# mageky/time-series-spark

Hardware: AMD Instinct MI355X
Metric: series_fitted_per_sec (higher is better)
Workload: dtype f64

## Files before the change

### include/tsf_dev.h

```cpp
#ifndef TSF_DEV_H
#define TSF_DEV_H

#include "tsf.h"

#ifdef __cplusplus
extern "C" {
#endif

enum {
    TSF_OPT_HARM = 0,
    TSF_OPT_LATTICE,
    TSF_OPT_SPARSE_EXTRA,
    TSF_OPT_FIT_GROUPED,
    TSF_OPT_GRAM_SHARE,
    TSF_OPT_GRID_ORDER,
    TSF_OPT_GRID_SHARE,
    TSF_OPT_RAGGED_SPLIT,
    TSF_OPT_QUAD_REG,
    TSF_OPT_QUAD_M2_LDS,
    TSF_OPT_QUAD_W4,
    TSF_OPT_QUAD_RREG,
    TSF_OPT_NEWTON_BATCH,
    TSF_OPT_NEWTON_FLAGS, TSF_OPT_NEWTON_NS, TSF_OPT_NEWTON_LCAP, TSF_OPT_NEWTON_FILL,
    TSF_OPT_QUAD_RAW_Y,
    TSF_OPT_DEBUG_ASYNC_SCRATCH,
    TSF_OPT_COOP_TAIL,
    TSF_OPT_MAP_DIRECT,
    TSF_OPT_COUNT
};
int tsf_set_option(tsf_ctx *ctx, int option, int value);
int tsf_get_option(const tsf_ctx *ctx, int option);

int tsf_eval(tsf_ctx *ctx, const tsf_spec *spec, int64_t N, int32_t T, const int64_t *ds,
             const void *y, int32_t y_dtype, const double *floor, const double *cap,
             const double *extra, const double *theta, double *f_out, double *grad_out);
int tsf_eval_quadratic(tsf_ctx *ctx, const tsf_spec *spec, int64_t N, int32_t T, const int64_t *ds,
                       const void *y, int32_t y_dtype, const double *extra, const double *theta_ref,
                       const double *theta, double *f_out, double *grad_out);
int tsf_design(tsf_ctx *ctx, const tsf_spec *spec, int32_t T, const int64_t *ds,
               const double *extra, double *X_out, double *t_out, tsf_grid_info *grid_out);
int tsf_selftest_math(tsf_ctx *ctx, int32_t op, int64_t n, const double *a, const double *b,
                      double *out);

#define TSF_PROFILE_RING 64
int tsf_set_profiling(tsf_ctx *ctx, int32_t enable);
int tsf_profile_read(tsf_ctx *ctx, float *ms_out, int32_t max_n, int32_t *n_out);
int tsf_last_fit_kernel_ms(tsf_ctx *ctx, float *ms_out);
int tsf_last_fit_route(tsf_ctx *ctx, int32_t *sparse_columns);
int tsf_last_cv_grids(const tsf_ctx *ctx, int64_t *n_grids, int32_t *n_launches);
int tsf_last_tune_counts(const tsf_ctx *ctx, int32_t *expand_launches, int32_t *fit_launches);

#ifdef __cplusplus
}
#endif
#endif
```

### time_series_spark_amd/_lib.py

```python
import contextlib
import ctypes
import os

import numpy as np

_HERE = os.path.dirname(os.path.abspath(__file__))
LIB_PATH = os.environ.get('TSF_LIB_PATH') or os.path.join(_HERE, 'libtsf_amd.so')

MAX_SEAS = 8
MAX_EXTRA = 64
MAX_S = 60
MAX_K = 64
MAX_P = 128
MAX_COMP = 128

GROWTH_LINEAR, GROWTH_LOGISTIC = 0, 1
MODE_ADDITIVE, MODE_MULTIPLICATIVE = 0, 1
Y_F64, Y_F32, Y_I32 = 0, 1, 2
EVAL_AUTO, EVAL_RESIDUAL, EVAL_QUADRATIC = 0, 1, 2
ALGO_LBFGS, ALGO_NEWTON, ALGO_AUTO = 0, 1, 2
RK_AUTO, RK_WAVE, RK_MFMA, RK_COOP = 0, 1, 2, 3
CONVERGE_STAN, CONVERGE_MAP = 0, 1

ST_ABSX, ST_ABSF, ST_RELF, ST_ABSGRAD, ST_RELGRAD, ST_MAXIT = 10, 20, 21, 30, 31, 40
ST_CONSTANT, ST_LSFAIL, ST_INIT_NONFINITE, ST_TOO_FEW, ST_CAP = 50, -1, -2, -10, -11
ST_EVAL_LIMIT = -3
ST_CHANGEPOINT = -12
ST_NEWTON_CONVERGED, ST_NEWTON_FAIL = 60, -4
ST_MAP_KKT, ST_MAP_FTOL, ST_MAP_MAXIT, ST_MAP_LS = 70, 71, 72, 73
STATUS_NAMES = {10: 'ABSX', 20: 'ABSF', 21: 'RELF', 30: 'ABSGRAD', 31: 'RELGRAD', 40: 'MAXIT',
                50: 'CONSTANT', -1: 'LSFAIL', -2: 'INIT_NONFINITE', -3: 'EVAL_LIMIT', -10: 'TOO_FEW',
                -11: 'CAP', -12: 'CHANGEPOINT', 60: 'NEWTON_CONVERGED', -4: 'NEWTON_FAIL', 70: 'MAP_KKT', 71: 'MAP_FTOL', 72: 'MAP_MAXIT',
                73: 'MAP_LS'}


class TsfSpec(ctypes.Structure):
    _fields_ = [('growth', ctypes.c_int32), ('n_changepoints', ctypes.c_int32),
                ('changepoint_range', ctypes.c_double),
                ('changepoint_prior_scale', ctypes.c_double),
                ('n_seas', ctypes.c_int32), ('n_extra', ctypes.c_int32),
                ('seas_period', ctypes.c_double * MAX_SEAS),
                ('seas_prior_scale', ctypes.c_double * MAX_SEAS),
                ('seas_order', ctypes.c_int32 * MAX_SEAS),
                ('seas_mode', ctypes.c_int32 * MAX_SEAS),
                ('extra_prior_scale', ctypes.c_double * MAX_EXTRA),
                ('extra_mode', ctypes.c_int32 * MAX_EXTRA),
                ('max_iter', ctypes.c_int32), ('history', ctypes.c_int32),
                ('init_alpha', ctypes.c_double), ('tol_obj', ctypes.c_double),
                ('tol_rel_obj', ctypes.c_double), ('tol_grad', ctypes.c_double),
                ('tol_rel_grad', ctypes.c_double), ('tol_param', ctypes.c_double),
                ('eval_form', ctypes.c_int32), ('recenter_every', ctypes.c_int32),
                ('recenter_ratio', ctypes.c_double),
                ('algorithm', ctypes.c_int32), ('residual_kernel', ctypes.c_int32),
                ('coop_after', ctypes.c_int32), ('converge', ctypes.c_int32), ('map_max_iter', ctypes.c_int32),
                ('map_tol', ctypes.c_double),
                ('changepoints_specified', ctypes.c_int32), ('changepoint_ns', ctypes.c_int64 * MAX_S)]


class TsfCvArgs(ctypes.Structure):
    _fields_ = [('horizon_ns', ctypes.c_int64), ('period_ns', ctypes.c_int64), ('initial_ns', ctypes.c_int64),
                ('rolling_window', ctypes.c_double)]


class TsfGridInfo(ctypes.Structure):
    _fields_ = [('start_ns', ctypes.c_int64), ('t_scale_ns', ctypes.c_int64),
                ('T', ctypes.c_int32), ('S', ctypes.c_int32), ('i1', ctypes.c_int32),
                ('NT', ctypes.c_int32), ('t_change', ctypes.c_double * (MAX_S + 4))]


GRID_DTYPE = np.dtype([('start_ns', '<i8'), ('t_scale_ns', '<i8'), ('T', '<i4'), ('S', '<i4'),
                       ('i1', '<i4'), ('NT', '<i4'), ('t_change', '<f8', (MAX_S + 4,))])


class TsfFitOut(ctypes.Structure):
    _fields_ = [('theta', ctypes.c_void_p), ('y_scale', ctypes.c_void_p),
                ('fval', ctypes.c_void_p), ('status', ctypes.c_void_p),
                ('n_iter', ctypes.c_void_p), ('n_eval', ctypes.c_void_p),
                ('grid', ctypes.c_void_p)]


class TsfCvOut(ctypes.Structure):
    _fields_ = [('fit', TsfFitOut), ('yhat', ctypes.c_void_p), ('yhat_lower', ctypes.c_void_p),
                ('yhat_upper', ctypes.c_void_p), ('horizon_ns', ctypes.c_void_p), ('mse', ctypes.c_void_p),
                ('rmse', ctypes.c_void_p), ('mae', ctypes.c_void_p), ('mape', ctypes.c_void_p),
                ('coverage', ctypes.c_void_p), ('series_status', ctypes.c_void_p)]


class TsfTuneOut(ctypes.Structure):
    _fields_ = [('score', ctypes.c_void_p), ('cand_status', ctypes.c_void_p), ('best', ctypes.c_void_p),
                ('series_status', ctypes.c_void_p), ('fit', TsfFitOut)]


EXPORTS = ['tsf_create', 'tsf_destroy', 'tsf_last_error', 'tsf_device_count', 'tsf_spec_default',
           'tsf_spec_size', 'tsf_grid_info_size', 'tsf_spec_K', 'tsf_theta_stride',
           'tsf_fit_aligned', 'tsf_fit_aligned_dev', 'tsf_fit_ragged', 'tsf_fit_ragged_dev',
           'tsf_predict', 'tsf_predict_dev', 'tsf_predict_intervals', 'tsf_predict_intervals_dev', 'tsf_predict_components', 'tsf_predict_components_dev', 'tsf_eval', 'tsf_eval_quadratic', 'tsf_design', 'tsf_selftest_math',
           'tsf_set_option', 'tsf_get_option', 'tsf_set_cost_hints', 'tsf_set_profiling', 'tsf_profile_read', 'tsf_last_fit_kernel_ms', 'tsf_last_fit_route',
           'tsf_cv_plan', 'tsf_cross_validate', 'tsf_last_cv_grids', 'tsf_tune', 'tsf_last_tune_counts',
           'tsf_pack_rows', 'tsf_pack_rows_typed', 'tsf_pack_fetch', 'tsf_pack_flags', 'tsf_pack_free', 'tsf_model_blobs',
           'tsf_csv_read', 'tsf_csv_fetch', 'tsf_csv_columns', 'tsf_csv_malformed', 'tsf_csv_free', 'tsf_csv_write_forecasts', 'tsf_csv_write_forecasts_i32',
           'tsf_csv_discover', 'tsf_csv_discover_load', 'tsf_csv_root_open', 'tsf_csv_root_load', 'tsf_csv_root_free', 'tsf_csv_read_loaded', 'tsf_csv_dir_paths', 'tsf_csv_dir_series_id', 'tsf_csv_dir_error_path', 'tsf_csv_dir_free']

CSV_E_OPEN, CSV_E_PARSE, CSV_E_CODEC = -10, -11, -12
CV_OK, CV_LESS_THAN_HORIZON, CV_NO_CUTOFF, CV_TOO_FEW, CV_FIT_FAILED = 0, -20, -21, -22, -23
TUNE_MSE, TUNE_RMSE, TUNE_MAE, TUNE_MAPE = 0, 1, 2, 3
TUNE_METRICS = {'mse': TUNE_MSE, 'rmse': TUNE_RMSE, 'mae': TUNE_MAE, 'mape': TUNE_MAPE}
TUNE_NO_SCORE = -24
TUNE_MAX_CAND = 256

OPTIONS = ['harm', 'lattice', 'sparse_extra', 'fit_grouped', 'gram_share', 'grid_order', 'grid_share', 'ragged_split',
           'quad_reg', 'quad_m2_lds', 'quad_w4', 'quad_rreg', 'newton_batch', 'newton_flags', 'newton_ns', 'newton_lcap',
           'newton_fill', 'quad_raw_y', 'debug_async_scratch', 'coop_tail', 'map_direct']

_lib = None


class TsfError(RuntimeError):
    pass


def load():
    global _lib
    if _lib is not None:
        return _lib
    if not os.path.exists(LIB_PATH):
        raise TsfError('libtsf_amd.so not built: run `python -m time_series_spark_amd.build` '
                       '(or __graft_entry__.build()).  There is no CPU fallback.')
    L = ctypes.CDLL(LIB_PATH)
    vp, i32, i64 = ctypes.c_void_p, ctypes.c_int32, ctypes.c_int64
    psp = ctypes.POINTER(TsfSpec)
    L.tsf_create.argtypes = [ctypes.c_int, ctypes.POINTER(vp)]
    L.tsf_destroy.argtypes = [vp]
    L.tsf_destroy.restype = None
    L.tsf_last_error.argtypes = [vp]
    L.tsf_last_error.restype = ctypes.c_char_p
    L.tsf_device_count.argtypes = []
    L.tsf_spec_default.argtypes = [psp]
    L.tsf_spec_default.restype = None
    L.tsf_spec_K.argtypes = [psp]
    L.tsf_theta_stride.argtypes = [psp]
    L.tsf_fit_aligned.argtypes = [vp, psp, i64, i32, vp, vp, i32, vp, vp, vp,
                                  ctypes.POINTER(TsfFitOut)]
    L.tsf_fit_aligned_dev.argtypes = [vp, psp, i64, i32, vp, vp, i32, vp, vp, vp,
                                      ctypes.POINTER(TsfFitOut), vp]
    L.tsf_fit_ragged.argtypes = [vp, psp, i64, vp, vp, vp, i32, vp, vp, vp,
                                 ctypes.POINTER(TsfFitOut)]
    L.tsf_fit_ragged_dev.argtypes = [vp, psp, i64, vp, i64, i32, vp, vp, i32, vp, vp, vp,
                                     ctypes.POINTER(TsfFitOut), vp]
    L.tsf_predict.argtypes = [vp, psp, i64, i32, vp, vp, vp, i32, vp, i32, vp, vp, vp, vp, vp]
    L.tsf_predict_dev.argtypes = [vp, psp, i64, i32, vp, vp, vp, i32, vp, i32, vp, vp, vp, vp, vp,
                                  vp]
    f64, u64 = ctypes.c_double, ctypes.c_uint64
    L.tsf_predict_intervals.argtypes = [vp, psp, i64, i32, vp, vp, vp, i32, vp, i32, vp, vp, vp, vp, i32, f64,
                                        u64, vp, vp, vp]
    L.tsf_predict_intervals_dev.argtypes = L.tsf_predict_intervals.argtypes + [vp]
    L.tsf_predict_components.argtypes = [vp, psp, i64, i32, vp, vp, vp, i32, vp, i32, vp, vp, vp, i32, vp, vp, vp, i32,
                                         f64, u64, vp, vp, vp, vp, vp, vp, vp]
    L.tsf_predict_components_dev.argtypes = L.tsf_predict_components.argtypes + [vp]
    L.tsf_eval.argtypes = [vp, psp, i64, i32, vp, vp, i32, vp, vp, vp, vp, vp, vp]
    L.tsf_eval_quadratic.argtypes = [vp, psp, i64, i32, vp, vp, i32, vp, vp, vp, vp, vp]
    L.tsf_design.argtypes = [vp, psp, i32, vp, vp, vp, vp, vp]
    L.tsf_selftest_math.argtypes = [vp, i32, i64, vp, vp, vp]
    L.tsf_set_cost_hints.argtypes = [vp, vp, i64]
    L.tsf_set_option.argtypes = [vp, i32, i32]
    L.tsf_get_option.argtypes = [vp, i32]
    L.tsf_set_profiling.argtypes = [vp, i32]
    L.tsf_profile_read.argtypes = [vp, ctypes.POINTER(ctypes.c_float), i32, ctypes.POINTER(i32)]
    L.tsf_last_fit_kernel_ms.argtypes = [vp, ctypes.POINTER(ctypes.c_float)]
    L.tsf_last_fit_route.argtypes = [vp, ctypes.POINTER(ctypes.c_int32)]
    L.tsf_cv_plan.argtypes = [i64, i32, vp, vp, ctypes.POINTER(TsfCvArgs), vp, vp, vp, vp, vp, vp, vp]
    L.tsf_cross_validate.argtypes = [vp, psp, i64, i32, vp, vp, vp, i32, vp, vp, vp, ctypes.POINTER(TsfCvArgs), vp, i32,
                                     ctypes.c_double, ctypes.c_uint64, ctypes.POINTER(TsfCvOut)]
    L.tsf_last_cv_grids.argtypes = [vp, ctypes.POINTER(i64), ctypes.POINTER(i32)]
    L.tsf_tune.argtypes = [vp, psp, psp, i32, i64, i32, vp, vp, vp, i32, vp, vp, vp, ctypes.POINTER(TsfCvArgs), i32, i32,
                           ctypes.POINTER(TsfTuneOut)]
    L.tsf_last_tune_counts.argtypes = [vp, ctypes.POINTER(i32), ctypes.POINTER(i32)]
    L.tsf_pack_rows.argtypes = [i64, vp, vp, vp, vp, i32, ctypes.POINTER(vp), ctypes.POINTER(i64),
                                ctypes.POINTER(i64), ctypes.POINTER(i32)]
    L.tsf_pack_fetch.argtypes = [vp, vp, vp, vp, vp, vp, vp, vp, vp]
    L.tsf_pack_rows_typed.argtypes = [i64, vp, vp, i32, vp, vp, i32, i32, ctypes.POINTER(vp), ctypes.POINTER(i64),
                                      ctypes.POINTER(i64), ctypes.POINTER(i32)]
    L.tsf_pack_flags.argtypes = [vp, ctypes.POINTER(i32), ctypes.POINTER(i32), ctypes.POINTER(i32), ctypes.POINTER(i32)]
    L.tsf_pack_free.argtypes = [vp]
    L.tsf_pack_free.restype = None
    L.tsf_model_blobs.argtypes = [i64, vp, i32, i32, vp, vp, vp, i32, vp, vp, vp, i32, vp, i32]
    L.tsf_csv_read.argtypes = [i32, vp, vp, ctypes.c_char_p, i32,
                               ctypes.POINTER(vp), ctypes.POINTER(i64), ctypes.POINTER(i32),
                               ctypes.POINTER(i64)]
    L.tsf_csv_fetch.argtypes = [vp, vp, vp, vp, vp]
    L.tsf_csv_columns.argtypes = [vp, ctypes.POINTER(vp), ctypes.POINTER(vp), ctypes.POINTER(vp), ctypes.POINTER(vp)]
    L.tsf_csv_discover.argtypes = [ctypes.c_char_p, i32, ctypes.POINTER(vp), ctypes.POINTER(i32), ctypes.POINTER(i32)]
    L.tsf_csv_discover_load.argtypes = L.tsf_csv_discover.argtypes
    L.tsf_csv_read_loaded.argtypes = [vp, i32, i32, ctypes.c_char_p, i32, ctypes.POINTER(vp), ctypes.POINTER(i64),
                                      ctypes.POINTER(i32), ctypes.POINTER(i64)]
    L.tsf_csv_root_open.argtypes = [ctypes.c_char_p, ctypes.POINTER(vp), ctypes.POINTER(i32), ctypes.POINTER(i32)]
    L.tsf_csv_root_load.argtypes = [vp, i32, i32, i32, ctypes.POINTER(vp), ctypes.POINTER(i32), ctypes.POINTER(i32),
                                    ctypes.POINTER(i32)]
    L.tsf_csv_root_free.argtypes = [vp]
    L.tsf_csv_root_free.restype = None
    L.tsf_csv_dir_paths.argtypes = [vp]
    L.tsf_csv_dir_paths.restype = vp
    L.tsf_csv_dir_series_id.argtypes = [vp]
    L.tsf_csv_dir_series_id.restype = vp
    L.tsf_csv_dir_error_path.argtypes = [vp]
    L.tsf_csv_dir_error_path.restype = ctypes.c_char_p
    L.tsf_csv_dir_free.argtypes = [vp]
    L.tsf_csv_dir_free.restype = None
    L.tsf_csv_malformed.argtypes = [vp]
    L.tsf_csv_malformed.restype = ctypes.c_int64
    L.tsf_csv_free.argtypes = [vp]
    L.tsf_csv_free.restype = None
    L.tsf_csv_write_forecasts.argtypes = [ctypes.c_char_p, ctypes.c_char_p, i64, vp, vp, vp, vp, i32]
    L.tsf_csv_write_forecasts_i32.argtypes = [ctypes.c_char_p, ctypes.c_char_p, i64, vp, vp, vp, vp, i32]
    if L.tsf_spec_size() != ctypes.sizeof(TsfSpec):
        raise TsfError('tsf_spec layout mismatch between _lib.py and libtsf_amd.so')
    if L.tsf_grid_info_size() != ctypes.sizeof(TsfGridInfo) or GRID_DTYPE.itemsize != ctypes.sizeof(TsfGridInfo):
        raise TsfError('tsf_grid_info layout mismatch between _lib.py and libtsf_amd.so')
    _lib = L
    return L


class Context(object):

    def __init__(self, device=0):
        L = load()
        h = ctypes.c_void_p()
        rc = L.tsf_create(int(device), ctypes.byref(h))
        if rc != 0:
            raise TsfError('tsf_create(device=%d) failed (rc=%d): no usable MI355X visible. '
                           'This library has no CPU fallback.' % (device, rc))
        self._h = h
        self.device = int(device)
        for item in filter(None, os.environ.get('TSF_OPTIONS', '').split(',')):
            k, v = item.split('=')
            self.set_option(k.strip(), int(v))

    def close(self):
        if getattr(self, '_h', None):
            load().tsf_destroy(self._h)
            self._h = None

    def __del__(self):
        try:
            self.close()
        except Exception:
            pass

    def check(self, rc):
        if rc != 0:
            msg = load().tsf_last_error(self._h)
            raise TsfError('libtsf_amd: rc=%d: %s' % (rc, msg.decode() if msg else '?'))

    @property
    def handle(self):
        return self._h

    def set_option(self, name, value=-1):
        self.check(load().tsf_set_option(self._h, OPTIONS.index(name), -1 if value is None else int(value)))

    def get_option(self, name):
        return int(load().tsf_get_option(self._h, OPTIONS.index(name)))

    @contextlib.contextmanager
    def options(self, **kw):
        old = {k: self.get_option(k) for k in kw}
        try:
            for k, v in kw.items():
                self.set_option(k, v)
            yield self
        finally:
            for k, v in old.items():
                self.set_option(k, v)


def default_spec():
    s = TsfSpec()
    load().tsf_spec_default(ctypes.byref(s))
    return s


def _ptr(a):
    return None if a is None else a.ctypes.data


def y_dtype_code(y):
    if y.dtype == np.float64:
        return Y_F64
    if y.dtype == np.float32:
        return Y_F32
    if y.dtype == np.int32:
        return Y_I32
    raise TypeError('y must be float64, float32 or int32')
```

### time_series_spark_amd/csrc/tsf_api.hip

```cpp
#include <hip/hip_runtime.h>

#include <cmath>
#include <cstdio>
#include <algorithm>
#include <chrono>
#include <cstdlib>
#include <cstring>
#include <map>
#include <mutex>
#include <string>
#include <thread>
#include <utility>
#include <atomic>
#include <vector>

#include "tsf_aux_kernels.h"
#include "tsf_interval_kernels.h"
#include "tsf_component_kernels.h"
#include "tsf_fit_kernels.h"
#include "tsf_quad_kernels.h"
#include "tsf_mfma_tabs.h"
#include "tsf_launch.h"
#include "tsf_cv_kernels.h"
#include "tsf_tune_kernels.h"
#include "tsf_cv_plan.h"

using namespace tsf;

struct tsf_ctx {
    int device;
    std::string err;
    void *ws;
    size_t ws_bytes;
    DevSpec *d_spec;
    void *nb_ws;
    size_t nb_ws_bytes;
    double *fut_tab;
    size_t fut_tab_bytes;
    void *iv_ws;
    size_t iv_ws_bytes;
    void *comp_tab;
    int32_t *order_dev[2];
    size_t order_cap[2];
    int order_next;
    int64_t order_n;
    std::vector<int32_t> cost_host;
    hipEvent_t order_ev[2];
    int order_busy[2];
    int n_cu;
    const int *last_sp_flag;
    int opt[TSF_OPT_COUNT];
    int profiling;
    hipEvent_t ev0[TSF_PROFILE_RING], ev1[TSF_PROFILE_RING];
    int ev_created;
    long ev_count;
    int64_t last_n_grids;
    int64_t cv_grids;
    int32_t cv_launches;
    int32_t tune_expand;
    int32_t tune_fits;
};

#define HIP_TRY(ctx, expr)                                                                   \
    do {                                                                                     \
        hipError_t e_ = (expr);                                                              \
        if (e_ != hipSuccess) {                                                              \
            (ctx)->err = std::string(#expr) + ": " + hipGetErrorString(e_);                  \
            return -2;                                                                       \
        }                                                                                    \
    } while (0)

static int fail(tsf_ctx *ctx, const char *msg)
{
    if (ctx) ctx->err = msg;
    return -1;
}

extern "C" int tsf_device_count(void)
{
    int n = 0;
    if (hipGetDeviceCount(&n) != hipSuccess) return 0;
    return n;
}

extern "C" int tsf_create(int device_id, tsf_ctx **out)
{
    if (!out) return -1;
    *out = nullptr;
    int n = 0;
    if (hipGetDeviceCount(&n) != hipSuccess || device_id < 0 || device_id >= n) return -2;
    if (hipSetDevice(device_id) != hipSuccess) return -2;
    tsf_ctx *c = new tsf_ctx();
    c->device = device_id; c->ws = nullptr; c->ws_bytes = 0; c->d_spec = nullptr;
    c->fut_tab = nullptr; c->fut_tab_bytes = 0;
    c->nb_ws = nullptr; c->nb_ws_bytes = 0;
    c->iv_ws = nullptr; c->iv_ws_bytes = 0;
    c->comp_tab = nullptr;
    c->order_dev[0] = c->order_dev[1] = nullptr; c->order_cap[0] = c->order_cap[1] = 0; c->order_next = 0; c->order_n = 0;
    c->order_ev[0] = c->order_ev[1] = nullptr; c->order_busy[0] = c->order_busy[1] = 0;
    c->profiling = 0; c->ev_created = 0; c->ev_count = 0;
    c->last_sp_flag = nullptr;
    c->last_n_grids = 0; c->cv_grids = 0; c->cv_launches = 0; c->tune_expand = 0; c->tune_fits = 0;
    for (int i = 0; i < TSF_OPT_COUNT; ++i) c->opt[i] = -1;
    if (hipMalloc((void **)&c->d_spec, sizeof(DevSpec)) != hipSuccess) { delete c; return -2; }
    {
        hipDeviceProp_t prop;
        c->n_cu = (hipGetDeviceProperties(&prop, device_id) == hipSuccess) ? prop.multiProcessorCount : 256;
    }
    *out = c;
    return 0;
}

namespace { void pool_trim(int device); }

extern "C" void tsf_destroy(tsf_ctx *ctx)
{
    if (!ctx) return;
    hipSetDevice(ctx->device);
    pool_trim(ctx->device);
    if (ctx->ws) hipFree(ctx->ws);
    if (ctx->d_spec) hipFree(ctx->d_spec);
    if (ctx->fut_tab) hipFree(ctx->fut_tab);
    if (ctx->nb_ws) hipFree(ctx->nb_ws);
    if (ctx->iv_ws) hipFree(ctx->iv_ws);
    if (ctx->comp_tab) hipFree(ctx->comp_tab);
    for (int b = 0; b < 2; ++b) { if (ctx->order_dev[b]) hipFree(ctx->order_dev[b]); if (ctx->order_ev[b]) hipEventDestroy(ctx->order_ev[b]); }
    if (ctx->ev_created)
        for (int i = 0; i < TSF_PROFILE_RING; ++i) { hipEventDestroy(ctx->ev0[i]); hipEventDestroy(ctx->ev1[i]); }
    delete ctx;
}

extern "C" const char *tsf_last_error(const tsf_ctx *ctx) { return ctx ? ctx->err.c_str() : "null context"; }

extern "C" int tsf_set_option(tsf_ctx *ctx, int option, int value)
{
    if (!ctx) return -1;
    if (option < 0 || option >= TSF_OPT_COUNT) return fail(ctx, "unknown option");
    ctx->opt[option] = value;
    return 0;
}

extern "C" int tsf_get_option(const tsf_ctx *ctx, int option)
{
    if (!ctx || option < 0 || option >= TSF_OPT_COUNT) return -1;
    return ctx->opt[option];
}

extern "C" void tsf_spec_default(tsf_spec *s)
{
    memset(s, 0, sizeof(*s));
    s->growth = TSF_GROWTH_LINEAR; s->n_changepoints = 25; s->changepoint_range = 0.8;
    s->changepoint_prior_scale = 0.05;
    s->max_iter = 10000; s->history = 5; s->init_alpha = 1e-3; s->tol_obj = 1e-12;
    s->tol_rel_obj = 1e4; s->tol_grad = 1e-8; s->tol_rel_grad = 1e7; s->tol_param = 1e-8;
    s->eval_form = TSF_EVAL_AUTO;
    s->algorithm = TSF_ALGO_LBFGS;
    s->residual_kernel = TSF_RK_AUTO; s->recenter_every = 128; s->recenter_ratio = 1.0;
    s->coop_after = -1;
    s->converge = TSF_CONVERGE_STAN; s->map_max_iter = 10000; s->map_tol = 1e-7;
}

extern "C" int tsf_spec_size(void) { return (int)sizeof(tsf_spec); }
extern "C" int tsf_grid_info_size(void) { return (int)sizeof(tsf_grid_info); }

extern "C" int tsf_spec_K(const tsf_spec *s)
{
    int K = s->n_extra;
    for (int i = 0; i < s->n_seas; ++i) K += 2 * s->seas_order[i];
    return K;
}

extern "C" int tsf_theta_stride(const tsf_spec *s) { return 3 + s->n_changepoints + tsf_spec_K(s); }


static int fit_P(int n_cp, int K) { return 3 + (n_cp > 0 ? n_cp : 1) + K; }

static int pick_KP(int K, int n_cp, int mixed)
{
    const int P = fit_P(n_cp, K);
    if (mixed || P > 64) return 64;
    if (K <= 8) return 8;
    if (K <= 16) return 16;
    if (K <= 28) return 28;
    return 64;
}

static int build_devspec(tsf_ctx *ctx, const tsf_spec *s, DevSpec *d, int *mode_out)
{
    if (!s) return fail(ctx, "spec is NULL");
    if (s->growth != TSF_GROWTH_LINEAR && s->growth != TSF_GROWTH_LOGISTIC) return fail(ctx, "bad growth");
    if (s->n_seas < 0 || s->n_seas > TSF_MAX_SEAS || s->n_extra < 0 || s->n_extra > TSF_MAX_EXTRA)
        return fail(ctx, "too many seasonalities / extra columns");
    if (s->n_changepoints < 0 || s->n_changepoints > TSF_MAX_S) return fail(ctx, "n_changepoints out of range");
    if (s->changepoints_specified != 0 && s->changepoints_specified != 1) return fail(ctx, "changepoints_specified must be 0 or 1");
    if (!s->changepoints_specified && !(s->changepoint_range >= 0.0 && s->changepoint_range <= 1.0)) return fail(ctx, "changepoint_range must be in [0,1]");
    if (s->changepoints_specified)
        for (int j = 1; j < s->n_changepoints; ++j)
            if (s->changepoint_ns[j] <= s->changepoint_ns[j - 1]) return fail(ctx, "changepoint_ns must be strictly ascending");
    if (!(s->changepoint_prior_scale > 0.0)) return fail(ctx, "changepoint_prior_scale must be > 0");
    if (s->history < 1 || s->history > MAXH) return fail(ctx, "history must be in [1,8]");
    if (s->eval_form < TSF_EVAL_AUTO || s->eval_form > TSF_EVAL_QUADRATIC) return fail(ctx, "bad eval_form");
    if (s->algorithm < TSF_ALGO_LBFGS || s->algorithm > TSF_ALGO_AUTO) return fail(ctx, "bad algorithm");
    if (s->residual_kernel < TSF_RK_AUTO || s->residual_kernel > TSF_RK_COOP) return fail(ctx, "bad residual_kernel");
    if (s->converge != TSF_CONVERGE_STAN && s->converge != TSF_CONVERGE_MAP) return fail(ctx, "bad converge");
    if (s->converge == TSF_CONVERGE_MAP && (s->map_max_iter < 1 || !(s->map_tol > 0.0))) return fail(ctx, "map_max_iter must be >= 1 and map_tol > 0");
    if (s->eval_form != TSF_EVAL_RESIDUAL && (s->recenter_every < 1 || !(s->recenter_ratio > 0.0)))
        return fail(ctx, "recenter_every must be >= 1 and recenter_ratio > 0");
    const int K = tsf_spec_K(s);
    if (K < 1) return fail(ctx, "model needs at least one design column (fbprophet adds a zero column; pass one extra column of zeros)");
    if (K > TSF_MAX_K || fit_P(s->n_changepoints, K) > TSF_MAX_P) return fail(ctx, "too many parameters (3+S+K must be <= 128, K <= 64)");
    memset(d, 0, sizeof(*d));
    int mode[TSF_MAX_P];
    double pr[TSF_MAX_P];
    int col = 0, np = 0;
    for (int i = 0; i < s->n_seas; ++i) {
        if (s->seas_order[i] < 1) return fail(ctx, "fourier order must be >= 1");
        if (!(s->seas_prior_scale[i] > 0.0) || !(s->seas_period[i] > 0.0)) return fail(ctx, "bad seasonality prior scale / period");
        d->seas_period[i] = s->seas_period[i]; d->seas_order[i] = s->seas_order[i]; d->seas_col[i] = col;
        for (int h = 0; h < s->seas_order[i]; ++h) {
            np++;
            mode[col] = s->seas_mode[i]; pr[col] = s->seas_prior_scale[i]; col++;
            mode[col] = s->seas_mode[i]; pr[col] = s->seas_prior_scale[i]; col++;
        }
    }
    for (int e = 0; e < s->n_extra; ++e) {
        if (!(s->extra_prior_scale[e] > 0.0)) return fail(ctx, "bad extra prior scale");
        mode[col] = s->extra_mode[e]; pr[col] = s->extra_prior_scale[e]; col++;
    }
    int n = 0;
    for (int j = 0; j < K; ++j) if (mode[j] == TSF_MODE_ADDITIVE) { d->perm[n] = j; d->inv_perm[j] = n; d->prior[n] = pr[j]; n++; }
    const int Ka = n;
    for (int j = 0; j < K; ++j) if (mode[j] != TSF_MODE_ADDITIVE) { d->perm[n] = j; d->inv_perm[j] = n; d->prior[n] = pr[j]; n++; }
    for (int j = K; j < TSF_MAX_P; ++j) d->prior[j] = 1.0;
    const int m = (Ka == K) ? 0 : (Ka == 0 ? 1 : 2);
    d->growth = s->growth; d->n_cp = s->n_changepoints; d->K = K; d->Ka = Ka;
    d->KP = pick_KP(K, s->n_changepoints, m == 2);
    d->n_seas = s->n_seas; d->n_extra = s->n_extra; d->n_pairs = np;
    d->max_iter = s->max_iter; d->history = s->history;
    d->harm = 0;
    if (m != 2 && s->n_seas >= 1 && s->n_seas <= 3) {
        bool ok = true;
        for (int i = 0; i < s->n_seas; ++i) ok = ok && s->seas_order[i] <= 255;
        if (ok) d->harm = harm_code(s->seas_order[0], s->n_seas > 1 ? s->seas_order[1] : 0, s->n_seas > 2 ? s->seas_order[2] : 0);
    }
    d->cp_range = s->changepoint_range; d->tau = s->changepoint_prior_scale;
    d->cp_spec = s->changepoints_specified;
    if (d->cp_spec) {
        d->cp_range = 0.0;
        for (int j = 0; j < s->n_changepoints; ++j) d->cp_ns[j] = s->changepoint_ns[j];
    }
    d->init_alpha = s->init_alpha; d->tol_obj = s->tol_obj; d->tol_rel_obj = s->tol_rel_obj;
    d->tol_grad = s->tol_grad; d->tol_rel_grad = s->tol_rel_grad; d->tol_param = s->tol_param;
    *mode_out = m;
    return 0;
}


struct WsLayout {
    size_t gtab, stab, tw, cw, Xw, yw, Mg, Mslot, rbuf, counter, uw, Xu, spm, spp, Bw;
    size_t mXF, mXB, mXT, mtq, mcq, mcpof, myq, mhist;
    size_t clist, cslots;
    size_t total;
};

constexpr size_t TSF_NB_KEEP = (size_t)1 << 30;

static int coop_slots_for(int64_t N, int after, int n_cu)
{
    if (after == COOP_DIRECT) return 0;
    const int64_t cap = after >= 0 ? 8192 : 8 * (int64_t)n_cu;
    return (int)(N < cap ? N : cap);
}

struct MfmaPlan { int on, NG, KF, NCB, rr0, blocks; };

static size_t align_up(size_t x) { return (x + 255) & ~(size_t)255; }

static WsLayout ws_layout(int64_t N, int64_t n_grids, int NTmax, int KP, int quad_P4 = 0,
                          int quad_slots = 0, int quad_ragged = 0, int64_t lat_U = 0,
                          const MfmaPlan *mp = nullptr, int coop_slots = 0, int coop_stride = 0, int64_t quad_pre = 0,
                          bool sparse = false, int bw_ns = 0, bool no_yw = false)
{
    WsLayout l;
    size_t off = 0;
    l.gtab = off; off = align_up(off + sizeof(GridTab) * (size_t)n_grids);
    l.stab = off; off = align_up(off + sizeof(SeriesTab) * (size_t)N);
    l.tw = off; off = align_up(off + sizeof(double) * (size_t)n_grids * NTmax * W);
    l.cw = off; off = align_up(off + sizeof(uint16_t) * (size_t)n_grids * NTmax * W);
    l.Xw = off; off = align_up(off + (lat_U > 0 ? 0 : sizeof(double) * (size_t)n_grids * NTmax * KP * W));
    l.yw = off; off = align_up(off + (no_yw ? 0 : sizeof(double) * (size_t)N * NTmax * W));
    l.Mg = off; off = align_up(off + sizeof(double) * (size_t)quad_P4 * 2 * W * (size_t)(quad_pre > 0 ? quad_pre : 1));
    l.Mslot = off; off = align_up(off + (quad_ragged ? sizeof(double) * (size_t)quad_slots * quad_P4 * 2 * W : 0));
    l.rbuf = off; off = align_up(off + sizeof(double) * (size_t)quad_slots * NTmax * W);
    l.counter = off; off = align_up(off + 256);
    l.spm = off; off = align_up(off + (sparse ? sizeof(uint32_t) * (size_t)n_grids * SP_M * W : 0));
    l.spp = off; off = align_up(off + (sparse ? sizeof(unsigned long long) * (size_t)n_grids * SP_MAXC : 0));
    l.Bw = off; off = align_up(off + sizeof(double) * (lat_U > 0 ? (size_t)lat_U * bw_ns * 2 : (size_t)n_grids * NTmax * bw_ns * 2 * W));
    l.uw = off; off = align_up(off + (lat_U > 0 ? sizeof(int32_t) * (size_t)n_grids * NTmax * W : 0));
    l.Xu = off; off = align_up(off + (lat_U > 0 ? sizeof(double) * (size_t)lat_U * KP : 0));
    const bool mf = mp && mp->on;
    const size_t tiles = mf ? (size_t)W * mp->NG : 0;
    l.mXF = off; off = align_up(off + (mf ? sizeof(double) * tiles * mp->KF * W : 0));
    l.mXB = off; off = align_up(off + (mf ? sizeof(double) * tiles * 4 * mp->NCB * W : 0));
    l.mXT = off; off = align_up(off + (mf ? sizeof(double) * tiles * 4 * W : 0));
    l.mtq = off; off = align_up(off + (mf ? sizeof(double) * tiles * 16 : 0));
    l.mcq = off; off = align_up(off + (mf ? sizeof(uint16_t) * tiles * 16 : 0));
    l.mcpof = off; off = align_up(off + (mf ? (size_t)W * 8 : 0));
    l.myq = off; off = align_up(off + (mf ? sizeof(double) * (size_t)N * tiles * 16 : 0));
    l.mhist = off; off = align_up(off + (mf ? sizeof(double) * (size_t)mp->blocks * MT_NS * 2 * MAXH * W : 0));
    l.clist = off; off = align_up(off + sizeof(int32_t) * (size_t)coop_slots);
    l.cslots = off; off = align_up(off + sizeof(double) * (size_t)coop_slots * coop_stride);
    l.total = off;
    return l;
}

static int ensure_ws(tsf_ctx *ctx, size_t bytes, int64_t N = 0, int NTmax = 0, int ragged = 0)
{
    if (ctx->ws_bytes >= bytes) return 0;
    {
        size_t free_b = 0, total_b = 0;
        if (hipMemGetInfo(&free_b, &total_b) == hipSuccess && bytes > free_b + ctx->ws_bytes && (ctx->nb_ws || ctx->iv_ws)) {
            if (ctx->nb_ws) { (void)hipFree(ctx->nb_ws); ctx->nb_ws = nullptr; ctx->nb_ws_bytes = 0; }
            if (ctx->iv_ws) { (void)hipFree(ctx->iv_ws); ctx->iv_ws = nullptr; ctx->iv_ws_bytes = 0; }
            (void)hipMemGetInfo(&free_b, &total_b);
        }
        if (free_b + total_b > 0 && bytes > free_b + ctx->ws_bytes) {
            char msg[384];
            snprintf(msg, sizeof(msg), "workspace of %.1f GB does not fit the device (%.1f GB free): %lld series, the longest has "
                     "%d rows%s", bytes / 1e9, (free_b + ctx->ws_bytes) / 1e9, (long long)N, NTmax * W,
                     ragged ? " and every series of a ragged call is padded to it -- split the call by series length" : "");
            ctx->err = msg;
            return -2;
        }
        (void)hipGetLastError();
    }
    ctx->last_sp_flag = nullptr;
    if (ctx->ws) { HIP_TRY(ctx, hipFree(ctx->ws)); ctx->ws = nullptr; ctx->ws_bytes = 0; }
    HIP_TRY(ctx, hipMalloc(&ctx->ws, bytes));
    ctx->ws_bytes = bytes;
    return 0;
}

static int quad_plan(tsf_ctx *ctx, const DevSpec &hs, int64_t N, QuadPlan *qp)
{
    const int P = fit_P(hs.n_cp, hs.K);
    qp->PPL = (hs.KP == 64) ? 2 : 1;
    qp->P4 = (qp->PPL == 2) ? ((P + 3) & ~3) : (P <= 40 ? 40 : (P <= 56 ? 56 : 64));
    qp->NW = quad_waves_per_block(qp->PPL);
    qp->n_cu = ctx->n_cu;
    qp->opt = ctx->opt;
    int64_t blocks = ctx->n_cu;
    const int64_t need = (N + qp->NW - 1) / qp->NW;
    if (blocks > need) blocks = need;
    if (blocks < 1) blocks = 1;
    qp->blocks = (int)blocks;
    int64_t slots = (int64_t)ctx->n_cu * qp->NW;
    if (slots > N + qp->NW) slots = N + qp->NW;
    qp->slots = (int)slots;
    if (qp->slots < qp->P4) qp->slots = qp->P4;
    return 0;
}

typedef int (*launch_t)(int, const FitArgs &, int, hipStream_t);
typedef int (*launch_newton_t)(int, const FitArgs &, int, hipStream_t);
static launch_newton_t pick_newton_launch(int growth, int mode)
{
    static const launch_newton_t tab[2][3] = {{launch_newton_g0m0, launch_newton_g0m1, launch_newton_g0m2},
                                              {launch_newton_g1m0, launch_newton_g1m1, launch_newton_g1m2}};
    return tab[growth][mode];
}

typedef int (*launch_map_t)(int, const FitArgs &, hipStream_t);
static launch_map_t pick_map_launch(int growth, int mode)
{
    static const launch_map_t tab[2][3] = {{launch_map_g0m0, launch_map_g0m1, launch_map_g0m2},
                                           {launch_map_g1m0, launch_map_g1m1, launch_map_g1m2}};
    return tab[growth][mode];
}

static launch_t pick_launch(int growth, int mode)
{
    static const launch_t tab[2][3] = {{launch_g0m0, launch_g0m1, launch_g0m2},
                                       {launch_g1m0, launch_g1m1, launch_g1m2}};
    return tab[growth][mode];
}

static int run_fit(tsf_ctx *ctx, const tsf_spec *spec, int64_t N, int aligned, int32_t T,
                   const int64_t *offsets, int64_t total_rows, int32_t max_T, const int64_t *ds,
                   const void *y, int32_t y_dtype, const double *floor_, const double *cap,
                   const double *extra, tsf_fit_out *out, const double *theta_in,
                   double *grad_out, hipStream_t st, int64_t lat_base = 0, int64_t lat_step = 0,
                   int64_t lat_U = 0, const double *theta_ref = nullptr,
                   const int32_t *grid_of = nullptr, const int64_t *grid_rows = nullptr, int64_t n_distinct = 0,
                   const int32_t *grid_order = nullptr, const int32_t *grid_keep = nullptr)
{
    if (!ctx) return -1;
    HIP_TRY(ctx, hipSetDevice(ctx->device));
    if (N <= 0) return fail(ctx, "N must be > 0");
    if (!ds || !y || !out) return fail(ctx, "NULL input");
    if (y_dtype < TSF_Y_F64 || y_dtype > TSF_Y_I32) return fail(ctx, "bad y_dtype");
    DevSpec hs;
    int mode = 0;
    int rc = build_devspec(ctx, spec, &hs, &mode);
    if (rc) return rc;
    if (hs.n_extra > 0 && !extra) return fail(ctx, "extra columns declared but extra is NULL");
    if (hs.growth == TSF_GROWTH_LOGISTIC && !cap) return fail(ctx, "logistic growth needs cap");
    const int Tm = aligned ? T : max_T;
    if (Tm < 1) return fail(ctx, "no rows");
    if (Tm > TSF_MAX_T) return fail(ctx, "series too long (TSF_MAX_T rows per series)");
    const int NTmax = (Tm + W - 1) / W;
    if (aligned || !grid_of || !grid_rows || n_distinct <= 0 || n_distinct >= N) { grid_of = nullptr; grid_rows = nullptr; n_distinct = 0; }
    const int64_t n_grids = aligned ? 1 : (grid_of ? n_distinct : N);
    ctx->last_n_grids = n_grids;
    const bool newton = theta_in == nullptr &&
                        (spec->algorithm == TSF_ALGO_NEWTON ||
                         (spec->algorithm == TSF_ALGO_AUTO && Tm < TSF_NEWTON_BELOW_T));
    if (newton && fit_P(hs.n_cp, hs.K) > 2 * W)
        return fail(ctx, "Newton needs 3 + n_changepoints + K <= 128");
    const bool quad_ok = hs.growth == TSF_GROWTH_LINEAR && mode == 0 && hs.history == QH &&
                         theta_in == nullptr && !newton;
    if (spec->eval_form == TSF_EVAL_QUADRATIC && !quad_ok && theta_in == nullptr)
        return fail(ctx, "eval_form QUADRATIC needs linear growth, additive columns only and history == 5");
    const bool quad = quad_ok && spec->eval_form != TSF_EVAL_RESIDUAL;
    const bool newton_quad = newton && hs.growth == TSF_GROWTH_LINEAR && mode == 0 && hs.KP <= 28 &&
                             spec->eval_form != TSF_EVAL_RESIDUAL && NTmax <= 16;
    const bool quad_eval = theta_in != nullptr && theta_ref != nullptr;
    if (quad_eval && !(aligned && hs.growth == TSF_GROWTH_LINEAR && mode == 0 && hs.KP != 64))
        return fail(ctx, "the quadratic form needs an aligned panel, linear growth, additive columns only and 3 + n_changepoints + K <= 64");
    if (!(newton_quad && aligned) && ctx->nb_ws_bytes > TSF_NB_KEEP) {
        HIP_TRY(ctx, hipFree(ctx->nb_ws));
        ctx->nb_ws = nullptr; ctx->nb_ws_bytes = 0;
    }
    QuadPlan qp;
    memset(&qp, 0, sizeof(qp));
    if (quad || newton_quad || quad_eval) {
        rc = quad_plan(ctx, hs, N, &qp);
        if (rc) return rc;
        if (newton_quad) {
            qp.slots = ctx->n_cu * 16;
            if (qp.slots < qp.P4) qp.slots = qp.P4;
        }
    }
    if (aligned || quad || newton || theta_in != nullptr || hs.n_extra > 0 || lat_step <= 0) lat_U = 0;
    {
        const int el = ctx->opt[TSF_OPT_LATTICE];
        const size_t tab = sizeof(double) * (size_t)n_grids * (size_t)NTmax * hs.KP * W;
        const bool harm_model = ctx->opt[TSF_OPT_HARM] != 0 && mode != 2 &&
                                ((hs.harm == HARM_Y10_W3 && hs.KP == 28) || (hs.harm == HARM_W3_D4 && hs.KP == 16) || (hs.harm == HARM_W3 && hs.KP == 8));
        const bool lat_harm = harm_model && hs.K == harm_kf(hs.harm);
        size_t harm_cap = (size_t)32 << 30;
        if (lat_U > 0 && el < 0 && harm_model && !lat_harm && tab > ((size_t)256 << 20)) {
            size_t free_b = 0, total_b = 0;
            if (hipMemGetInfo(&free_b, &total_b) == hipSuccess) {
                const size_t mine = (free_b + ctx->ws_bytes) / 5 * 2;
                if (mine < harm_cap) harm_cap = mine;
            } else {
                (void)hipGetLastError();
            }
        }
        if (el >= 0 ? el == 0 : ((grid_of != nullptr && tab <= ((size_t)64 << 20)) || (harm_model && !lat_harm && tab <= harm_cap))) lat_U = 0;
    }
    MfmaPlan mp;
    memset(&mp, 0, sizeof(mp));
    if (spec->residual_kernel == TSF_RK_MFMA && hs.cp_spec && theta_in == nullptr)
        return fail(ctx, "residual_kernel MFMA does not take specified changepoints (changepoints_specified = 1)");
    const bool want_mfma = spec->residual_kernel == TSF_RK_MFMA;
    if (aligned && !quad && !newton && theta_in == nullptr && hs.KP <= 28 && want_mfma) {
        const int hist_rows = (int)floor((double)Tm * hs.cp_range);
        int S = hs.n_cp;
        if (S + 1 > hist_rows) S = hist_rows - 1;
        if (S < 1) S = 1;
        const double step = (hs.n_cp > 0 && S > 0) ? (double)(hist_rows - 1) / (double)S : 1e30;
        const int per_chunk = (int)ceil((double)NTmax / (step > 1.0 ? step : 1.0)) + 2;
        if (S <= MT_SP && per_chunk <= MT_MAXCP && mfma_lds_bytes(hs.KP) <= 160 * 1024) {
            mp.on = 1;
            mp.NG = (NTmax + 15) / 16;
            mp.KF = hs.KP / 4;
            mp.NCB = (hs.KP + 15) / 16;
            mp.rr0 = (16 * mp.NG - NTmax) / 4;
            int64_t blocks = (N + MT_NS - 1) / MT_NS;
            if (blocks > ctx->n_cu) blocks = ctx->n_cu;
            mp.blocks = (int)blocks;
        }
    }
    if (spec->residual_kernel == TSF_RK_MFMA && !mp.on && theta_in == nullptr && !quad && !newton)
        return fail(ctx, "residual_kernel MFMA needs an aligned panel, K <= 28 columns of one mode, 3+S+K <= 64 and S <= 28");
    const bool coop_ok = !quad && !newton && theta_in == nullptr && !mp.on && NTmax <= COOP_MAX_NT;
    if (spec->residual_kernel == TSF_RK_COOP && !coop_ok && theta_in == nullptr)
        return fail(ctx, "residual_kernel COOP needs a residual-form L-BFGS fit of series of at most 4096 rows");
    const bool coop = coop_ok && spec->residual_kernel != TSF_RK_WAVE;
    const bool sparse_try = !quad && !newton && !mp.on && theta_in == nullptr && lat_U == 0 && hs.KP == 64 && mode != 2 &&
                            spec->residual_kernel == TSF_RK_AUTO && hs.K > SP_DENSE && hs.K <= SP_DENSE + SP_MAXC &&
                            hs.K - hs.n_extra <= SP_DENSE && NTmax <= SP_MAX_NT && ctx->opt[TSF_OPT_SPARSE_EXTRA] != 0;
    int coop_after = spec->residual_kernel == TSF_RK_COOP ? COOP_DIRECT : spec->coop_after;
    if (coop) {
        const bool grouped = NTmax <= 12 && ctx->opt[TSF_OPT_FIT_GROUPED] != 0 && lat_U == 0;
        if (spec->residual_kernel == TSF_RK_AUTO && spec->coop_after < 0 && hs.KP == 64 && !grouped && !sparse_try) coop_after = COOP_DIRECT;
    }
    const int coop_slots = coop ? coop_slots_for(N, coop_after, ctx->n_cu) : 0;
    const int coop_stride = coop ? coop_slot_doubles(hs.KP == 64 ? 2 : 1) : 0;
    const int64_t quad_pre = (quad && !aligned && grid_of && n_grids * 2 <= N && ctx->opt[TSF_OPT_GRAM_SHARE] != 0) ? n_grids : 0;
    int harm = 0;
    if (!quad && !newton && !mp.on && theta_in == nullptr && lat_U == 0 && ctx->opt[TSF_OPT_HARM] != 0) {
        if ((hs.harm == HARM_Y10_W3 && (hs.KP == 28 || sparse_try)) || (hs.harm == HARM_W3_D4 && hs.KP == 16) ||
            (hs.harm == HARM_W3 && hs.KP == 8))
            harm = hs.harm;
    } else if (!quad && !newton && !mp.on && theta_in == nullptr && lat_U > 0 && ctx->opt[TSF_OPT_HARM] != 0 && mode != 2 &&
               hs.K == harm_kf(hs.harm) &&
               ((hs.harm == HARM_Y10_W3 && hs.KP == 28) || (hs.harm == HARM_W3_D4 && hs.KP == 16) || (hs.harm == HARM_W3 && hs.KP == 8))) {
        harm = hs.harm;
    }
    int gram_harm = 0;
    if (quad && !aligned && !quad_pre && lat_U == 0 && hs.harm == HARM_Y10_W3 && hs.KP == 28 && ctx->opt[TSF_OPT_HARM] != 0)
        gram_harm = hs.harm;
    int map_harm = 0;
    if (spec->converge == TSF_CONVERGE_MAP && theta_in == nullptr && mode != 2 && ctx->opt[TSF_OPT_HARM] != 0 &&
        hs.K == harm_kf(hs.harm) &&
        ((hs.harm == HARM_Y10_W3 && hs.KP == 28) || (hs.harm == HARM_W3_D4 && hs.KP == 16) || (hs.harm == HARM_W3 && hs.KP == 8)))
        map_harm = hs.harm;
    const int bw_ns = (harm || gram_harm || map_harm) ? hs.n_seas : 0;
    const bool raw_y = quad && spec->converge != TSF_CONVERGE_MAP && ctx->opt[TSF_OPT_QUAD_RAW_Y] != 0;
    const WsLayout l = ws_layout(N, n_grids, NTmax, hs.KP, qp.P4, qp.slots, (quad || newton_quad) && !aligned, lat_U, &mp,
                                 coop_slots, coop_stride, quad_pre, sparse_try, bw_ns, raw_y);
    rc = ensure_ws(ctx, l.total, N, NTmax, !aligned);
    if (rc) return rc;
    char *ws = (char *)ctx->ws;
    GridTab *gtab = (GridTab *)(ws + l.gtab);
    SeriesTab *stab = (SeriesTab *)(ws + l.stab);
    double *tw = (double *)(ws + l.tw);
    uint16_t *cw = (uint16_t *)(ws + l.cw);
    double *Xw = (double *)(ws + l.Xw);
    double *yw = raw_y ? (double *)nullptr : (double *)(ws + l.yw);
    HIP_TRY(ctx, hipMemcpyAsync(ctx->d_spec, &hs, sizeof(hs), hipMemcpyHostToDevice, st));
    if (lat_U > 0) {
        double *Xu = (double *)(ws + l.Xu);
        HIP_TRY(ctx, hipMemsetAsync(Xu, 0, sizeof(double) * (size_t)lat_U * hs.KP, st));
        HIP_TRY(ctx, hipMemsetAsync(ws + l.uw, 0, sizeof(int32_t) * (size_t)n_grids * NTmax * W, st));
        const int64_t work = lat_U * (hs.n_seas > 0 ? hs.n_seas : 1);
        hipLaunchKernelGGL(setup_lattice_kernel, dim3((unsigned)((work + 255) / 256 > 65535 ? 65535 : (work + 255) / 256)),
                           dim3(256), 0, st, ctx->d_spec, lat_U, lat_base, lat_step, Xu, bw_ns ? (double *)(ws + l.Bw) : (double *)nullptr);
        HIP_TRY(ctx, hipGetLastError());
    } else {
        HIP_TRY(ctx, hipMemsetAsync(Xw, 0, sizeof(double) * (size_t)n_grids * NTmax * hs.KP * W, st));
        if (bw_ns) HIP_TRY(ctx, hipMemsetAsync(ws + l.Bw, 0, sizeof(double) * (size_t)n_grids * NTmax * bw_ns * 2 * W, st));
    }
    HIP_TRY(ctx, hipMemsetAsync(gtab, 0, sizeof(GridTab) * (size_t)n_grids, st));
    hipLaunchKernelGGL(setup_grid_kernel, dim3((unsigned)n_grids), dim3(256), 0, st, ctx->d_spec,
                       (int)n_grids, aligned ? nullptr : offsets, T, ds, extra,
                       aligned ? (int64_t)T : total_rows, NTmax, gtab, tw, cw, Xw,
                       (int32_t *)(ws + l.uw), lat_base, lat_U > 0 ? lat_step : (int64_t)0, grid_rows,
                       (bw_ns && lat_U == 0) ? (double *)(ws + l.Bw) : (double *)nullptr, grid_keep);
    HIP_TRY(ctx, hipGetLastError());
    if (sparse_try) {
        int *sp_bad = (int *)(ws + l.counter) + 8;
        HIP_TRY(ctx, hipMemsetAsync(sp_bad, 0, sizeof(int), st));
        hipLaunchKernelGGL(sparse_extra_kernel, dim3((unsigned)n_grids), dim3(64), 0, st, ctx->d_spec, gtab, Xw, NTmax,
                           (uint32_t *)(ws + l.spm), (unsigned long long *)(ws + l.spp), sp_bad);
        HIP_TRY(ctx, hipGetLastError());
    }
    if (!raw_y) {
        hipLaunchKernelGGL(setup_series_kernel, dim3((unsigned)N), dim3(64), 0, st, ctx->d_spec, N,
                           aligned ? nullptr : offsets, T, ds, y, y_dtype, floor_, cap, NTmax, gtab,
                           aligned, stab, yw, grid_of);
        HIP_TRY(ctx, hipGetLastError());
    }
    FitArgs a;
    memset(&a, 0, sizeof(a));
    a.sp = ctx->d_spec; a.N = N; a.aligned = aligned; a.NTmax = NTmax;
    a.theta_stride = tsf_theta_stride(spec);
    {
        const double eps = 2.220446049250313e-16;
        a.opt.init_alpha = hs.init_alpha; a.opt.tol_obj = hs.tol_obj;
        a.opt.tol_rel_obj_eps = hs.tol_rel_obj * eps; a.opt.tol_grad = hs.tol_grad;
        a.opt.tol_rel_grad_eps = hs.tol_rel_grad * eps; a.opt.tol_param = hs.tol_param;
        a.opt.max_iter = hs.max_iter; a.opt.history = hs.history;
    }
    a.gtab = gtab; a.stab = stab; a.tw = tw; a.yw = yw; a.Xw = Xw; a.cw = cw;
    a.theta = out->theta; a.y_scale = out->y_scale; a.fval = out->fval; a.status = out->status;
    a.n_iter = out->n_iter; a.n_eval = out->n_eval; a.grid_out = out->grid;
    a.theta_in = theta_in; a.grad_out = grad_out;
    if (raw_y) { a.y_raw = y; a.y_raw_dtype = y_dtype; a.y_offsets = aligned ? nullptr : offsets; a.y_T = T; }
    a.uw = (const int32_t *)(ws + l.uw); a.Xu = (const double *)(ws + l.Xu); a.xidx = lat_U > 0 ? 1 : 0;
    a.grid_of = grid_of;
    a.Bw = (bw_ns && lat_U == 0) ? (const double *)(ws + l.Bw) : nullptr; a.bw_ns = bw_ns; a.harm = harm;
    a.Bu = (bw_ns && lat_U > 0) ? (const double *)(ws + l.Bw) : nullptr;
    a.coop_harm = (harm != 0 && hs.K == harm_kf(harm) && mode != 2) ? 1 : 0;
    {
        const size_t row_tabs = (size_t)n_grids * NTmax * W * (sizeof(double) + sizeof(uint16_t) + sizeof(double) * 2 * (size_t)bw_ns) +
                                (size_t)N * NTmax * W * sizeof(double);
        const int oh = ctx->opt[TSF_OPT_HARM];
        a.harm_pf = (harm != 0 && (oh == 2 || (oh != 1 && !aligned && row_tabs > ((size_t)256 << 20)))) ? 1 : 0;
        if (harm != 0 && lat_U > 0) a.harm_pf = 1;
    }
    a.opt_coop_sparse = ctx->opt[TSF_OPT_SPARSE_EXTRA] != 2 ? 1 : 0;
    ctx->last_sp_flag = nullptr;
    if (sparse_try) {
        a.sp_meta = (const uint32_t *)(ws + l.spm); a.sp_prog = (const unsigned long long *)(ws + l.spp);
        a.sp_flag = (int *)(ws + l.counter) + 8;
        ctx->last_sp_flag = a.sp_flag;
    }
    const int order_buf = (ctx->order_n == N && !theta_in) ? (ctx->order_next ^ 1) : -1;
    if (order_buf >= 0) a.order = ctx->order_dev[order_buf];
    else if (grid_order && ctx->opt[TSF_OPT_GRID_ORDER] != 0) a.order = grid_order;
    ctx->order_n = 0;
    const int slot = (int)(ctx->ev_count % TSF_PROFILE_RING);
    if (ctx->profiling) HIP_TRY(ctx, hipEventRecord(ctx->ev0[slot], st));
    int lrc;
    bool map_done = false;
    if (newton_quad) {
        QuadArgs qa;
        memset(&qa, 0, sizeof(qa));
        qa.f = a; qa.Mg = (const double *)(ws + l.Mg); qa.Mslot = (double *)(ws + l.Mslot);
        qa.rbuf = (double *)(ws + l.rbuf);
        qa.counter = (int *)(ws + l.counter); qa.P4 = qp.P4;
        if (aligned && !(ctx->opt[TSF_OPT_DEBUG_ASYNC_SCRATCH] > 0 && (ctx->opt[TSF_OPT_DEBUG_ASYNC_SCRATCH] & 1))) {
            const size_t need = newton_batch_scratch_bytes(hs.KP, fit_P(hs.n_cp, hs.K) | 1, N, NTmax, ctx->n_cu, ctx->opt);
            if (need > ctx->nb_ws_bytes) {
                if (ctx->nb_ws) { HIP_TRY(ctx, hipFree(ctx->nb_ws)); ctx->nb_ws = nullptr; ctx->nb_ws_bytes = 0; }
                if (hipMalloc(&ctx->nb_ws, need) == hipSuccess) ctx->nb_ws_bytes = need;
                else { ctx->nb_ws = nullptr; (void)hipGetLastError(); }
            }
            qa.nb_buf = ctx->nb_ws; qa.nb_bytes = ctx->nb_ws_bytes;
        }
        HIP_TRY(ctx, hipMemsetAsync(qa.counter, 0, sizeof(int), st));
        lrc = launch_newton_quad(hs.KP, qp, qa, (double *)(ws + l.Mg), fit_P(hs.n_cp, hs.K) | 1, ctx->n_cu, st);
        if (lrc == -1) lrc = pick_newton_launch(hs.growth, mode)(hs.KP, a, fit_P(hs.n_cp, hs.K), st);
    } else if (newton) {
        lrc = pick_newton_launch(hs.growth, mode)(hs.KP, a, fit_P(hs.n_cp, hs.K), st);
    } else if (quad_eval) {
        QuadArgs qa;
        memset(&qa, 0, sizeof(qa));
        qa.f = a; qa.Mg = (const double *)(ws + l.Mg); qa.rbuf = (double *)(ws + l.rbuf);
        qa.counter = (int *)(ws + l.counter); qa.P4 = qp.P4;
        lrc = launch_eval_quad(hs.KP, qp, qa, (double *)(ws + l.Mg), theta_ref, st);
    } else if (quad) {
        QuadArgs qa;
        memset(&qa, 0, sizeof(qa));
        qa.f = a; qa.Mg = (const double *)(ws + l.Mg); qa.Mslot = (double *)(ws + l.Mslot);
        qa.rbuf = (double *)(ws + l.rbuf);
        qa.counter = (int *)(ws + l.counter); qa.P4 = qp.P4;
        qa.recenter_every = spec->recenter_every; qa.recenter_ratio = spec->recenter_ratio;
        qa.dbg = nullptr; qa.nb_buf = nullptr; qa.nb_bytes = 0;
        qa.Mpre = quad_pre ? qa.Mg : nullptr; qa.n_pre = quad_pre;
        qa.gram_harm = gram_harm;
        HIP_TRY(ctx, hipMemsetAsync(qa.counter, 0, sizeof(int), st));
        lrc = -1;
        if (spec->converge == TSF_CONVERGE_MAP && qp.PPL == 1 && ctx->opt[TSF_OPT_MAP_DIRECT] != 0) {
            qa.f.map_max_iter = spec->map_max_iter; qa.f.map_tol = spec->map_tol;
            lrc = launch_map_quad(hs.KP, qp, qa, (double *)(ws + l.Mg), fit_P(hs.n_cp, hs.K) | 1, st);
            if (lrc == 0) map_done = true;
        }
        if (lrc == -1) lrc = launch_quad(hs.KP, qp, qa, (double *)(ws + l.Mg), st);
    } else if (mp.on) {
        MfmaTabs mt;
        memset(&mt, 0, sizeof(mt));
        int *flags = (int *)(ws + l.counter);
        HIP_TRY(ctx, hipMemsetAsync(flags, 0, 2 * sizeof(int), st));
        mt.XF = (const double *)(ws + l.mXF); mt.XB = (const double *)(ws + l.mXB);
        mt.XT = (const double *)(ws + l.mXT); mt.tq = (const double *)(ws + l.mtq);
        mt.cq = (const uint16_t *)(ws + l.mcq); mt.cpof = (const int8_t *)(ws + l.mcpof);
        mt.yq = (const double *)(ws + l.myq); mt.hist = (double *)(ws + l.mhist);
        mt.counter = flags; mt.overflow = flags + 1;
        mt.NG = mp.NG; mt.KF = mp.KF; mt.NCB = mp.NCB; mt.rr0 = mp.rr0; mt.run_if_overflow = 0;
        lrc = launch_mfma_layout(a, hs.KP, mt, (double *)(ws + l.mXF), (double *)(ws + l.mXB),
                                 (double *)(ws + l.mXT), (double *)(ws + l.mtq), (uint16_t *)(ws + l.mcq),
                                 (int8_t *)(ws + l.mcpof), (double *)(ws + l.myq), flags + 1, st);
        if (lrc == 0) {
            if (ctx->profiling) HIP_TRY(ctx, hipEventRecord(ctx->ev0[slot], st));
            lrc = launch_mfma(hs.KP, hs.growth, mode, a, mt, mp.blocks, st);
        }
        if (lrc == 0) {
            FitArgs fb = a;
            fb.run_flag = flags + 1; fb.run_if = 1;
            lrc = pick_launch(hs.growth, mode)(hs.KP, fb, 0, st);
        }
    } else {
        if (coop) {
            a.coop_ctl = (int *)(ws + l.counter);
            a.coop_list = (int32_t *)(ws + l.clist);
            a.coop_slots = (double *)(ws + l.cslots);
            a.coop_max = coop_slots; a.coop_stride = coop_stride;
            a.coop_after = coop_after;
            a.coop_blocks = ctx->n_cu;
            {
                const int pct = ctx->opt[TSF_OPT_COOP_TAIL] > 0 ? ctx->opt[TSF_OPT_COOP_TAIL] : 200;
                a.coop_tail_at = (int)((int64_t)ctx->n_cu * (pct > 400 ? 400 : pct) / 100);
                if (a.coop_tail_at < 1) a.coop_tail_at = 1;
            }
            HIP_TRY(ctx, hipMemsetAsync(a.coop_ctl, 0, 4 * sizeof(int), st));
        }
        lrc = pick_launch(hs.growth, mode)(hs.KP, a, theta_in != nullptr, st);
    }
    if (lrc == 0 && spec->converge == TSF_CONVERGE_MAP && theta_in == nullptr && !map_done) {
        a.map_max_iter = spec->map_max_iter; a.map_tol = spec->map_tol; a.map_harm = map_harm;
        if (map_harm && lat_U == 0) a.Bw = (const double *)(ws + l.Bw);
        if (map_harm && lat_U > 0) a.Bu = (const double *)(ws + l.Bw);
        a.order = nullptr; a.run_flag = nullptr;
        lrc = pick_map_launch(hs.growth, mode)(hs.KP, a, st);
    }
    if (ctx->profiling) { HIP_TRY(ctx, hipEventRecord(ctx->ev1[slot], st)); ctx->ev_count++; }
    if (order_buf >= 0) {
        if (!ctx->order_ev[order_buf]) HIP_TRY(ctx, hipEventCreateWithFlags(&ctx->order_ev[order_buf], hipEventDisableTiming));
        HIP_TRY(ctx, hipEventRecord(ctx->order_ev[order_buf], st));
        ctx->order_busy[order_buf] = 1;
    }
    if (lrc != 0) {
        ctx->err = std::string("kernel launch failed: ") + (lrc > 0 ? hipGetErrorString((hipError_t)lrc) : "no kernel for this shape");
        return -2;
    }
    return 0;
}

extern "C" int tsf_fit_aligned_dev(tsf_ctx *ctx, const tsf_spec *spec, int64_t N, int32_t T,
                                   const int64_t *ds, const void *y, int32_t y_dtype,
                                   const double *floor_, const double *cap, const double *extra,
                                   tsf_fit_out *out, void *stream)
{
    if (!ctx) return -1;
    if (!out || !out->theta || !out->y_scale || !out->fval || !out->status || !out->n_iter ||
        !out->n_eval || !out->grid)
        return fail(ctx, "tsf_fit_out has NULL members");
    return run_fit(ctx, spec, N, 1, T, nullptr, 0, T, ds, y, y_dtype, floor_, cap, extra, out,
                   nullptr, nullptr, (hipStream_t)stream);
}

extern "C" int tsf_fit_ragged_dev(tsf_ctx *ctx, const tsf_spec *spec, int64_t N,
                                  const int64_t *offsets, int64_t total_rows, int32_t max_T,
                                  const int64_t *ds, const void *y, int32_t y_dtype,
                                  const double *floor_, const double *cap, const double *extra,
                                  tsf_fit_out *out, void *stream)
{
    if (!ctx) return -1;
    if (!offsets) return fail(ctx, "offsets is NULL");
    if (!out || !out->theta || !out->y_scale || !out->fval || !out->status || !out->n_iter ||
        !out->n_eval || !out->grid)
        return fail(ctx, "tsf_fit_out has NULL members");
    return run_fit(ctx, spec, N, 0, 0, offsets, total_rows, max_T, ds, y, y_dtype, floor_, cap,
                   extra, out, nullptr, nullptr, (hipStream_t)stream);
}


namespace {
struct PoolEntry { void *p; size_t bytes; int device; };
std::mutex g_pool_mu;
std::vector<PoolEntry> g_pool;
size_t g_pool_bytes = 0;
constexpr size_t POOL_LIMIT = (size_t)2 << 30;

size_t pool_class(size_t n)
{
    size_t c = 256;
    while (c < n) c <<= 1;
    return c;
}

void pool_trim(int device)
{
    std::lock_guard<std::mutex> lk(g_pool_mu);
    for (size_t i = 0; i < g_pool.size();) {
        if (g_pool[i].device == device) {
            hipFree(g_pool[i].p);
            g_pool_bytes -= g_pool[i].bytes;
            g_pool[i] = g_pool.back();
            g_pool.pop_back();
        } else {
            ++i;
        }
    }
}

struct DevBuf {
    void *p = nullptr;
    size_t bytes = 0;
    int device = 0;
    ~DevBuf()
    {
        if (!p) return;
        std::lock_guard<std::mutex> lk(g_pool_mu);
        if (g_pool_bytes + bytes <= POOL_LIMIT) { g_pool.push_back({p, bytes, device}); g_pool_bytes += bytes; }
        else hipFree(p);
    }
    hipError_t alloc(size_t n)
    {
        bytes = pool_class(n ? n : 8);
        hipGetDevice(&device);
        {
            std::lock_guard<std::mutex> lk(g_pool_mu);
            for (size_t i = 0; i < g_pool.size(); ++i) {
                if (g_pool[i].device == device && g_pool[i].bytes == bytes) {
                    p = g_pool[i].p;
                    g_pool_bytes -= bytes;
                    g_pool[i] = g_pool.back();
                    g_pool.pop_back();
                    return hipSuccess;
                }
            }
        }
        return hipMalloc(&p, bytes);
// ... 803 lines not shown
    HIP_TRY(ctx, hipDeviceSynchronize());
    HIP_TRY(ctx, hipMemcpy(yhat, d_yh.p, nh, hipMemcpyDeviceToHost));
    HIP_TRY(ctx, hipMemcpy(trend, d_tr.p, nh, hipMemcpyDeviceToHost));
    if (n_comp > 0) HIP_TRY(ctx, hipMemcpy(comp, d_co.p, nh * n_comp, hipMemcpyDeviceToHost));
    if (iv) {
        HIP_TRY(ctx, hipMemcpy(yhat_lower, d_lo.p, nh, hipMemcpyDeviceToHost));
        HIP_TRY(ctx, hipMemcpy(yhat_upper, d_hi.p, nh, hipMemcpyDeviceToHost));
        HIP_TRY(ctx, hipMemcpy(trend_lower, d_tlo.p, nh, hipMemcpyDeviceToHost));
        HIP_TRY(ctx, hipMemcpy(trend_upper, d_thi.p, nh, hipMemcpyDeviceToHost));
    }
    return 0;
}


extern "C" int tsf_design(tsf_ctx *ctx, const tsf_spec *spec, int32_t T, const int64_t *ds,
                          const double *extra, double *X_out, double *t_out,
                          tsf_grid_info *grid_out)
{
    if (!ctx) return -1;
    HIP_TRY(ctx, hipSetDevice(ctx->device));
    if (!spec || !ds || T < 2) return fail(ctx, "bad input");
    DevSpec hs;
    int mode = 0;
    int rc = build_devspec(ctx, spec, &hs, &mode);
    if (rc) return rc;
    if (hs.n_extra > 0 && !extra) return fail(ctx, "extra is NULL");
    const int NT = (T + W - 1) / W;
    const WsLayout l = ws_layout(1, 1, NT, hs.KP);
    rc = ensure_ws(ctx, l.total);
    if (rc) return rc;
    char *ws = (char *)ctx->ws;
    DevBuf d_ds, d_ex;
    HIP_TRY(ctx, d_ds.alloc(8 * (size_t)T));
    HIP_TRY(ctx, hipMemcpy(d_ds.p, ds, 8 * (size_t)T, hipMemcpyHostToDevice));
    if (hs.n_extra > 0) {
        HIP_TRY(ctx, d_ex.alloc(8 * (size_t)hs.n_extra * T));
        HIP_TRY(ctx, hipMemcpy(d_ex.p, extra, 8 * (size_t)hs.n_extra * T, hipMemcpyHostToDevice));
    }
    HIP_TRY(ctx, hipMemcpy(ctx->d_spec, &hs, sizeof(hs), hipMemcpyHostToDevice));
    HIP_TRY(ctx, hipMemset(ws + l.Xw, 0, sizeof(double) * (size_t)NT * hs.KP * W));
    HIP_TRY(ctx, hipMemset(ws + l.gtab, 0, sizeof(GridTab)));
    hipLaunchKernelGGL(setup_grid_kernel, dim3(1), dim3(256), 0, nullptr, ctx->d_spec, 1, nullptr, T,
                       d_ds.as<int64_t>(), d_ex.as<double>(), (int64_t)T, NT, (GridTab *)(ws + l.gtab),
                       (double *)(ws + l.tw), (uint16_t *)(ws + l.cw), (double *)(ws + l.Xw), nullptr,
                       (int64_t)0, (int64_t)0);
    HIP_TRY(ctx, hipGetLastError());
    HIP_TRY(ctx, hipDeviceSynchronize());
    std::vector<double> Xw((size_t)NT * hs.KP * W), tw((size_t)NT * W);
    GridTab gt;
    HIP_TRY(ctx, hipMemcpy(Xw.data(), ws + l.Xw, Xw.size() * 8, hipMemcpyDeviceToHost));
    HIP_TRY(ctx, hipMemcpy(tw.data(), ws + l.tw, tw.size() * 8, hipMemcpyDeviceToHost));
    HIP_TRY(ctx, hipMemcpy(&gt, ws + l.gtab, sizeof(gt), hipMemcpyDeviceToHost));
    for (int i = 0; i < T; ++i) {
        const int L = i / NT, q = i - L * NT;
        if (t_out) t_out[i] = tw[(size_t)q * W + L];
        if (X_out)
            for (int j = 0; j < hs.K; ++j)
                X_out[(size_t)i * hs.K + hs.perm[j]] = Xw[((size_t)q * hs.KP + j) * W + L];
    }
    if (grid_out) *grid_out = gt.info;
    return 0;
}

extern "C" int tsf_selftest_math(tsf_ctx *ctx, int32_t op, int64_t n, const double *a,
                                 const double *b, double *out)
{
    if (!ctx) return -1;
    HIP_TRY(ctx, hipSetDevice(ctx->device));
    if (n <= 0 || !a || !out) return fail(ctx, "bad input");
    DevBuf da, db, dout;
    HIP_TRY(ctx, da.alloc(8 * n)); HIP_TRY(ctx, dout.alloc(8 * n));
    HIP_TRY(ctx, hipMemcpy(da.p, a, 8 * n, hipMemcpyHostToDevice));
    if (b) { HIP_TRY(ctx, db.alloc(8 * n)); HIP_TRY(ctx, hipMemcpy(db.p, b, 8 * n, hipMemcpyHostToDevice)); }
    hipLaunchKernelGGL(selftest_kernel, dim3((unsigned)((n + 255) / 256)), dim3(256), 0, nullptr, op, n,
                       da.as<double>(), b ? db.as<double>() : nullptr, dout.as<double>());
    HIP_TRY(ctx, hipGetLastError());
    HIP_TRY(ctx, hipDeviceSynchronize());
    HIP_TRY(ctx, hipMemcpy(out, dout.p, 8 * n, hipMemcpyDeviceToHost));
    return 0;
}


extern "C" int tsf_set_cost_hints(tsf_ctx *ctx, const int32_t *cost, int64_t n)
{
    if (!ctx) return -1;
    ctx->order_n = 0;
    if (!cost || n <= 0) return 0;
    if (n > (int64_t)INT32_MAX) return fail(ctx, "tsf_set_cost_hints: too many series");
    HIP_TRY(ctx, hipSetDevice(ctx->device));
    std::vector<int32_t> order((size_t)n);
    for (int64_t i = 0; i < n; ++i) order[(size_t)i] = (int32_t)i;
    std::stable_sort(order.begin(), order.end(), [cost](int32_t x, int32_t y) { return cost[x] > cost[y]; });
    const int b = ctx->order_next;
    if (ctx->order_busy[b]) {
        HIP_TRY(ctx, hipEventSynchronize(ctx->order_ev[b]));
        ctx->order_busy[b] = 0;
    }
    const size_t need = sizeof(int32_t) * (size_t)n;
    if (ctx->order_cap[b] < need) {
        if (ctx->order_dev[b]) { HIP_TRY(ctx, hipFree(ctx->order_dev[b])); ctx->order_dev[b] = nullptr; ctx->order_cap[b] = 0; }
        HIP_TRY(ctx, hipMalloc((void **)&ctx->order_dev[b], need));
        ctx->order_cap[b] = need;
    }
    HIP_TRY(ctx, hipMemcpy(ctx->order_dev[b], order.data(), need, hipMemcpyHostToDevice));
    ctx->order_next = b ^ 1;
    ctx->order_n = n;
    if (cost != ctx->cost_host.data()) ctx->cost_host.assign(cost, cost + n);
    return 0;
}

extern "C" int tsf_set_profiling(tsf_ctx *ctx, int32_t enable)
{
    if (!ctx) return -1;
    HIP_TRY(ctx, hipSetDevice(ctx->device));
    if (enable && !ctx->ev_created) {
        for (int i = 0; i < TSF_PROFILE_RING; ++i) {
            HIP_TRY(ctx, hipEventCreate(&ctx->ev0[i]));
            HIP_TRY(ctx, hipEventCreate(&ctx->ev1[i]));
        }
        ctx->ev_created = 1;
    }
    ctx->profiling = enable ? 1 : 0;
    ctx->ev_count = 0;
    return 0;
}

extern "C" int tsf_profile_read(tsf_ctx *ctx, float *ms_out, int32_t max_n, int32_t *n_out)
{
    if (!ctx) return -1;
    if (!ms_out || !n_out) return fail(ctx, "NULL output");
    HIP_TRY(ctx, hipSetDevice(ctx->device));
    long n = ctx->ev_count < TSF_PROFILE_RING ? ctx->ev_count : TSF_PROFILE_RING;
    if (n > max_n) n = max_n;
    const long first = ctx->ev_count - n;
    for (long i = 0; i < n; ++i) {
        const int slot = (int)((first + i) % TSF_PROFILE_RING);
        HIP_TRY(ctx, hipEventSynchronize(ctx->ev1[slot]));
        HIP_TRY(ctx, hipEventElapsedTime(&ms_out[i], ctx->ev0[slot], ctx->ev1[slot]));
    }
    *n_out = (int32_t)n;
    return 0;
}

extern "C" int tsf_last_fit_route(tsf_ctx *ctx, int32_t *sparse_columns)
{
    if (!ctx || !sparse_columns) return -1;
    *sparse_columns = 0;
    if (!ctx->last_sp_flag) return 0;
    int bad = 1;
    HIP_TRY(ctx, hipSetDevice(ctx->device));
    HIP_TRY(ctx, hipDeviceSynchronize());
    HIP_TRY(ctx, hipMemcpy(&bad, ctx->last_sp_flag, sizeof(int), hipMemcpyDeviceToHost));
    *sparse_columns = bad ? 0 : 1;
    return 0;
}

extern "C" int tsf_last_fit_kernel_ms(tsf_ctx *ctx, float *ms_out)
{
    if (!ctx) return -1;
    if (!ms_out || ctx->ev_count == 0) return fail(ctx, "no profiled fit call recorded");
    int32_t n = 0;
    float tmp[TSF_PROFILE_RING];
    int rc = tsf_profile_read(ctx, tmp, TSF_PROFILE_RING, &n);
    if (rc) return rc;
    *ms_out = tmp[n - 1];
    return 0;
}


extern "C" int tsf_last_cv_grids(const tsf_ctx *ctx, int64_t *n_grids, int32_t *n_launches)
{
    if (!ctx || !n_grids || !n_launches) return -1;
    *n_grids = ctx->cv_grids;
    *n_launches = ctx->cv_launches;
    return 0;
}

namespace {
struct CvCall {
    bool aligned = false;
    int64_t N = 0;
    int32_t T = 0;
    const int64_t *offsets = nullptr, *ds = nullptr;
    int32_t y_dtype = 0;
    size_t ysz = 8;
    int n_extra = 0, stride = 0;
    bool has_floor = false, has_cap = false;
    std::vector<std::vector<tsf_cv::Fold>> plan;
    std::vector<int32_t> pst;
    std::vector<int64_t> pnh, pnm, fold_off, rows_off, m_off;
    int64_t F = 0, R = 0, M = 0;
    std::vector<int32_t> f_series, f_c;
    std::vector<int64_t> f_cut, f_hist, f_hold, f_row0;
    std::vector<double> f_floor, f_cap;
    std::vector<int32_t> f_keep;
    int32_t Hmax = 1, C = 0;
    DevBuf d_ds, d_y, d_off, d_ex, d_fl, d_cap, d_key, d_fser, d_fc, d_fhist, d_fhold;
    CvPanel pn;
    DevBuf d_th, d_ys, d_fv, d_st, d_it, d_ev, d_gr;
    tsf_fit_out dfo;
};

struct CvViews {
    const int32_t *d_series;
    const int32_t *series;
    const int64_t *hist;
    const int32_t *cls;
    int32_t n_cls;
    const int32_t *keep;
};

struct CvGroup {
    std::vector<int32_t> gf;
    int64_t G = 0, rows = 0, n_distinct = 0;
    int32_t maxT = 0;
    DevBuf d_gf, d_goff, d_gds, d_gy, d_gex, d_gfl, d_gcap, d_gof, d_grows, d_gord;
    DevBuf d_gkeep;
};

struct CvHoldout {
    DevBuf d_fds, d_fex, d_fkey, d_ffl, d_fcap;
};

struct CvMetrics {
    DevBuf d_foff, d_roff, d_moff, d_fcut, d_frow0, d_hs, d_ts, d_pre, d_yo, d_loo, d_hio, d_mh, d_mm, d_sst;
    CvMetricArgs ma;
};
}

static void cv_plan_call(int64_t N, int32_t T, const int64_t *offsets, const int64_t *ds, const tsf_cv_args &a,
                         const tsf_spec *spec, int32_t y_dtype, const double *floor_, const double *cap, CvCall *S)
{
    S->aligned = offsets == nullptr;
    S->N = N; S->T = T; S->offsets = offsets; S->ds = ds; S->y_dtype = y_dtype; S->ysz = ysize(y_dtype);
    S->n_extra = spec->n_extra; S->stride = tsf_theta_stride(spec);
    S->has_floor = floor_ != nullptr; S->has_cap = cap != nullptr;
    tsf_cv::panel_plan(N, T, offsets, ds, a, &S->plan, &S->pst, &S->pnh, &S->pnm);
    S->fold_off.assign((size_t)N + 1, 0); S->rows_off.assign((size_t)N + 1, 0); S->m_off.assign((size_t)N + 1, 0);
    for (int64_t n = 0; n < N; ++n) {
        S->fold_off[(size_t)n + 1] = S->fold_off[(size_t)n] + (int64_t)S->plan[(size_t)n].size();
        S->rows_off[(size_t)n + 1] = S->rows_off[(size_t)n] + S->pnh[(size_t)n];
        S->m_off[(size_t)n + 1] = S->m_off[(size_t)n] + S->pnm[(size_t)n];
    }
    const int64_t F = S->F = S->fold_off[(size_t)N];
    S->R = S->rows_off[(size_t)N]; S->M = S->m_off[(size_t)N];
    S->f_series.resize((size_t)F); S->f_c.resize((size_t)F);
    S->f_cut.resize((size_t)F); S->f_hist.resize((size_t)F); S->f_hold.resize((size_t)F); S->f_row0.resize((size_t)F);
    S->f_floor.resize(floor_ ? (size_t)F : 0); S->f_cap.resize(cap ? (size_t)F : 0);
    const bool cp_spec = spec->changepoints_specified == 1 && spec->n_changepoints >= 0 && spec->n_changepoints <= TSF_MAX_S;
    S->f_keep.resize(cp_spec ? (size_t)F : 0);
    for (int64_t n = 0; n < N; ++n) {
        int64_t r = S->rows_off[(size_t)n];
        for (size_t c = 0; c < S->plan[(size_t)n].size(); ++c) {
            const int64_t f = S->fold_off[(size_t)n] + (int64_t)c;
            const tsf_cv::Fold &x = S->plan[(size_t)n][c];
            S->f_series[(size_t)f] = (int32_t)n; S->f_c[(size_t)f] = (int32_t)c;
            S->f_cut[(size_t)f] = x.cutoff; S->f_hist[(size_t)f] = x.hist; S->f_hold[(size_t)f] = x.hold; S->f_row0[(size_t)f] = r;
            if (floor_) S->f_floor[(size_t)f] = floor_[n];
            if (cap) S->f_cap[(size_t)f] = cap[n];
            if (cp_spec) {
                int32_t k = 0;
                while (k < spec->n_changepoints && spec->changepoint_ns[k] <= x.cutoff) ++k;
                S->f_keep[(size_t)f] = k;
            }
            r += x.hold;
            if (x.hold > S->Hmax) S->Hmax = (int32_t)x.hold;
        }
        if ((int32_t)S->plan[(size_t)n].size() > S->C) S->C = (int32_t)S->plan[(size_t)n].size();
    }
}

static int cv_upload(tsf_ctx *ctx, const void *y, const double *floor_, const double *cap, const double *extra,
                     const int64_t *series_key, CvCall *S)
{
    const int64_t N = S->N, F = S->F, T = S->T;
    const int64_t n_ds = S->aligned ? T : S->offsets[N];
    const int64_t n_y = S->aligned ? N * T : S->offsets[N];
    HIP_TRY(ctx, S->d_ds.alloc(8 * (size_t)n_ds));
    HIP_TRY(ctx, hipMemcpy(S->d_ds.p, S->ds, 8 * (size_t)n_ds, hipMemcpyHostToDevice));
    HIP_TRY(ctx, S->d_y.alloc(S->ysz * (size_t)n_y));
    HIP_TRY(ctx, hipMemcpy(S->d_y.p, y, S->ysz * (size_t)n_y, hipMemcpyHostToDevice));
    if (!S->aligned) {
        HIP_TRY(ctx, S->d_off.alloc(8 * ((size_t)N + 1)));
        HIP_TRY(ctx, hipMemcpy(S->d_off.p, S->offsets, 8 * ((size_t)N + 1), hipMemcpyHostToDevice));
    }
    if (S->n_extra > 0) {
        HIP_TRY(ctx, S->d_ex.alloc(8 * (size_t)S->n_extra * n_ds));
        HIP_TRY(ctx, hipMemcpy(S->d_ex.p, extra, 8 * (size_t)S->n_extra * n_ds, hipMemcpyHostToDevice));
    }
    if (floor_) { HIP_TRY(ctx, S->d_fl.alloc(8 * (size_t)N)); HIP_TRY(ctx, hipMemcpy(S->d_fl.p, floor_, 8 * (size_t)N, hipMemcpyHostToDevice)); }
    if (cap) { HIP_TRY(ctx, S->d_cap.alloc(8 * (size_t)N)); HIP_TRY(ctx, hipMemcpy(S->d_cap.p, cap, 8 * (size_t)N, hipMemcpyHostToDevice)); }
    if (series_key) { HIP_TRY(ctx, S->d_key.alloc(8 * (size_t)N)); HIP_TRY(ctx, hipMemcpy(S->d_key.p, series_key, 8 * (size_t)N, hipMemcpyHostToDevice)); }
    if (F > 0) {
        HIP_TRY(ctx, S->d_fser.alloc(4 * (size_t)F)); HIP_TRY(ctx, hipMemcpy(S->d_fser.p, S->f_series.data(), 4 * (size_t)F, hipMemcpyHostToDevice));
        HIP_TRY(ctx, S->d_fc.alloc(4 * (size_t)F)); HIP_TRY(ctx, hipMemcpy(S->d_fc.p, S->f_c.data(), 4 * (size_t)F, hipMemcpyHostToDevice));
        HIP_TRY(ctx, S->d_fhist.alloc(8 * (size_t)F)); HIP_TRY(ctx, hipMemcpy(S->d_fhist.p, S->f_hist.data(), 8 * (size_t)F, hipMemcpyHostToDevice));
        HIP_TRY(ctx, S->d_fhold.alloc(8 * (size_t)F)); HIP_TRY(ctx, hipMemcpy(S->d_fhold.p, S->f_hold.data(), 8 * (size_t)F, hipMemcpyHostToDevice));
    }
    CvPanel &pn = S->pn;
    pn.ds = S->d_ds.as<int64_t>(); pn.y = S->d_y.p; pn.extra = S->n_extra > 0 ? S->d_ex.as<double>() : nullptr;
    pn.src_off = S->aligned ? nullptr : S->d_off.as<int64_t>(); pn.T = S->aligned ? T : 0;
    pn.src_total = S->aligned ? 0 : S->offsets[N];
    pn.ysz = (int)S->ysz; pn.n_extra = S->n_extra;
    const int stride = S->stride;
    HIP_TRY(ctx, S->d_th.alloc(8 * (size_t)F * stride)); HIP_TRY(ctx, S->d_ys.alloc(8 * (size_t)F));
    HIP_TRY(ctx, S->d_fv.alloc(8 * (size_t)F)); HIP_TRY(ctx, S->d_st.alloc(4 * (size_t)F));
// ... 539 lines not shown
```

### time_series_spark_amd/csrc/tsf_inst_quad4.hip

```cpp
#include "tsf_quad_launch.h"

namespace tsf {

int launch_quad_aligned_reg(int KP, const QuadPlan &qp, const QuadArgs &qa, double *Mg, hipStream_t st)
{
    switch (KP * 100 + qp.P4) {
    case 840: return launch_quad_mm<8, 1, QM_GLOBAL_REG, 40>(qp, qa, Mg, st);
    case 856: return launch_quad_mm<8, 1, QM_GLOBAL_REG, 56>(qp, qa, Mg, st);
    case 1640: return launch_quad_mm<16, 1, QM_GLOBAL_REG, 40>(qp, qa, Mg, st);
    case 1656: return launch_quad_mm<16, 1, QM_GLOBAL_REG, 56>(qp, qa, Mg, st);
    case 2840: return launch_quad_mm<28, 1, QM_GLOBAL_REG, 40>(qp, qa, Mg, st);
    case 2856: return launch_quad_mm<28, 1, QM_GLOBAL_REG, 56>(qp, qa, Mg, st);
    default: return -2;
    }
}

}
```

### time_series_spark_amd/csrc/tsf_launch.h

```cpp
#pragma once
#include <hip/hip_runtime.h>
#include <stddef.h>
#include <stdint.h>
namespace tsf {
struct FitArgs;
struct QuadArgs;
struct MfmaTabs;
struct QuadPlan { int P4, PPL, NW, blocks, slots, n_cu; const int *opt; };
int quad_waves_per_block(int PPL);
int launch_quad(int KP, const QuadPlan &qp, const QuadArgs &qa, double *Mg, hipStream_t st);
int launch_quad_aligned1(int KP, const QuadPlan &qp, const QuadArgs &qa, double *Mg, hipStream_t st);
int launch_eval_quad(int KP, const QuadPlan &qp, const QuadArgs &qa, double *Mg, const double *theta_ref, hipStream_t st);
int launch_map_quad(int KP, const QuadPlan &qp, const QuadArgs &qa, double *Mg, int PM, hipStream_t st);
int launch_quad_aligned_reg(int KP, const QuadPlan &qp, const QuadArgs &qa, double *Mg, hipStream_t st);
int launch_newton_quad(int KP, const QuadPlan &qp, const QuadArgs &qa, double *Mg, int PM, int n_cu, hipStream_t st);
size_t newton_batch_scratch_bytes(int KP, int PM, int64_t N, int NTmax, int n_cu, const int *opt);
int launch_g0m0(int KP, const FitArgs &a, int eval_only, hipStream_t st);
int launch_g0m1(int KP, const FitArgs &a, int eval_only, hipStream_t st);
int launch_g0m2(int KP, const FitArgs &a, int eval_only, hipStream_t st);
int launch_g1m0(int KP, const FitArgs &a, int eval_only, hipStream_t st);
int launch_g1m1(int KP, const FitArgs &a, int eval_only, hipStream_t st);
int launch_g1m2(int KP, const FitArgs &a, int eval_only, hipStream_t st);
int launch_map_g0m0(int KP, const FitArgs &a, hipStream_t st);
int launch_map_g0m1(int KP, const FitArgs &a, hipStream_t st);
int launch_map_g0m2(int KP, const FitArgs &a, hipStream_t st);
int launch_map_g1m0(int KP, const FitArgs &a, hipStream_t st);
int launch_map_g1m1(int KP, const FitArgs &a, hipStream_t st);
int launch_map_g1m2(int KP, const FitArgs &a, hipStream_t st);
size_t mfma_lds_bytes(int KP);
int launch_mfma_layout(const FitArgs &a, int KP, const MfmaTabs &mt, double *XF, double *XB, double *XT,
                       double *tq, uint16_t *cq, int8_t *cpof, double *yq, int *overflow, hipStream_t st);
int launch_mfma(int KP, int growth, int mode, const FitArgs &a, const MfmaTabs &mt, int blocks, hipStream_t st);
int launch_newton_g0m0(int KP, const FitArgs &a, int P, hipStream_t st);
int launch_newton_g0m1(int KP, const FitArgs &a, int P, hipStream_t st);
int launch_newton_g0m2(int KP, const FitArgs &a, int P, hipStream_t st);
int launch_newton_g1m0(int KP, const FitArgs &a, int P, hipStream_t st);
int launch_newton_g1m1(int KP, const FitArgs &a, int P, hipStream_t st);
int launch_newton_g1m2(int KP, const FitArgs &a, int P, hipStream_t st);
}
```

### time_series_spark_amd/csrc/tsf_quad_kernels.h

```cpp
#pragma once
#include "tsf_fit_kernels.h"

namespace tsf {

#define UQ(x) uniform_f64(x)
#ifndef TSF_QUAD_EXPSC
#define TSF_QUAD_EXPSC 0
#endif

constexpr int QH = 5;
constexpr int quad_waves_per_simd(bool w3, int nw = 0) { return nw == 16 ? 4 : (w3 ? 3 : 2); }
constexpr bool quad_three_waves(int mmode, int ppl, bool hlds) { return hlds && mmode == 0 && ppl == 1; }

struct QuadArgs {
    FitArgs f;
    const double *Mg;
    double *Mslot;
    const double *Mpre;
    int64_t n_pre;
    double *rbuf;
    int *counter;
    int P4;
    int recenter_every;
    double recenter_ratio;
    long long *dbg;
    void *nb_buf;
    size_t nb_bytes;
    int gram_harm;
};

template <int KP, int PPL>
struct QuadLds {
    double th[PPL * W + W];
    double ks[NTAB + 1], mc[NTAB + 1];
    double tp1[NTAB], tp2[NTAB];
    double tot1[W + 1], tot2[W + 1];
    double accR[KP];
    double ref[PPL * W], cvec[PPL * W];
};

constexpr int QC_N = 32;
enum { QC_LOG2E = 0, QC_LN2HI = 1, QC_LN2LO = 2, QC_EXP_P = 3 , QC_EXP_HI = 14, QC_EXP_LO = 15,
       QC_TOL_OBJ = 16, QC_TOL_REL_OBJ = 17, QC_TOL_GRAD = 18, QC_TOL_REL_GRAD = 19, QC_TOL_PARAM = 20,
       QC_INIT_ALPHA = 21, QC_RC_RATIO = 22,
       QC_GRAD2_LO = 23, QC_GRAD2_HI = 24, QC_PARAM2_LO = 25, QC_PARAM2_HI = 26, QC_RELGRAD_LO = 27, QC_RELGRAD_HI = 28 };
template <int PPL>
constexpr size_t quad_lanec_bytes() { return sizeof(double) * (3 * PPL * W + QC_N); }

typedef const volatile __attribute__((address_space(3))) double *qc_lds_ptr;
__device__ __forceinline__ double qc(const double *ct, int k) { return *((qc_lds_ptr)ct + k); }

template <int PPL>
struct QuadWave { double dl[PPL * W], ref[PPL * W], cvec[PPL * W]; };

struct QuadPool {
    int *locks;
    unsigned char *slots;
    int ns, first;
    unsigned slot_bytes;
};
constexpr size_t QUAD_POOL_LOCK_BYTES = 64;

__device__ __forceinline__ int pool_acquire(const QuadPool &pl)
{
    int i = pl.first;
    for (;;) {
        const int old = atomicCAS(pl.locks + i, 0, 1);
        if (__any(old == 0)) break;
        i = (i + 1 == pl.ns) ? 0 : i + 1;
        if (i == pl.first) __builtin_amdgcn_s_sleep(8);
    }
    __builtin_amdgcn_fence(__ATOMIC_ACQUIRE, "workgroup");
    return __builtin_amdgcn_readfirstlane(i);
}

__device__ __forceinline__ void pool_release(const QuadPool &pl, int i)
{
    __builtin_amdgcn_fence(__ATOMIC_RELEASE, "workgroup");
    __hip_atomic_store(pl.locks + i, 0, __ATOMIC_RELAXED, __HIP_MEMORY_SCOPE_WORKGROUP);
}


template <int KP, int G, int NTR = 0>
__device__ __forceinline__ void column_group(const SeriesView &sv, const double *rb, int g0,
                                             double *accR, const double (&rr)[NTR > 0 ? NTR : 1])
{
    const int lane = lane_id();
    double acc[G];
#pragma unroll
    for (int j = 0; j < G; ++j) acc[j] = 0.0;
    auto step = [&](int q, double r) {
        const double *xp = sv.Xw + ((size_t)q * KP + g0) * W + lane;
        double x[G];
#pragma unroll
        for (int j = 0; j < G; ++j) x[j] = xp[j * W];
#pragma unroll
        for (int j = 0; j < G; ++j) acc[j] = __builtin_fma(x[j], r, acc[j]);
    };
    if (NTR > 0) {
#pragma unroll 2
        for (int q = sv.NT - 1; q >= NTR; --q) step(q, rb[q * W + lane]);
        const int q1 = sv.NT < NTR ? sv.NT : NTR;
#pragma unroll 4
        for (int q = q1 - 1; q >= 0; --q) step(q, rr[NTR > 0 ? q : 0]);
    } else {
#pragma unroll 4
        for (int q = sv.NT - 1; q >= 0; --q) step(q, rb[q * W + lane]);
    }
    column_sums_g<G>(acc, accR + g0);
}

template <int KP, int HARM, int G0, int G>
__device__ __forceinline__ void column_group_harm(const SeriesView &sv, const double *rb, double *accR, bool has_xd)
{
    constexpr int KF = harm_kf(HARM), NS = harm_ns(HARM);
    const int lane = lane_id();
    double acc[G];
#pragma unroll
    for (int j = 0; j < G; ++j) acc[j] = 0.0;
#pragma unroll 2
    for (int q = sv.NT - 1; q >= 0; --q) {
        const double r = rb[q * W + lane];
        const bool valid = q < sv.cnt;
        const double2 *bq = reinterpret_cast<const double2 *>(sv.Bw) + (size_t)q * NS * W + lane;
        double2 bp[NS];
#pragma unroll
        for (int se = 0; se < NS; ++se) {
            const double2 b = bq[se * W];
            bp[se].x = valid ? b.x : 0.0; bp[se].y = valid ? b.y : 0.0;
        }
        harm_row<HARM>(bp, [&](int j, double v) {
            if (j >= G0 && j < G0 + G) acc[j - G0 < 0 ? 0 : (j - G0 < G ? j - G0 : 0)] = __builtin_fma(v, r, acc[j - G0 < 0 ? 0 : (j - G0 < G ? j - G0 : 0)]);
        });
        if (G0 + G > KF && has_xd) {
#pragma unroll
            for (int j = (G0 > KF ? G0 : KF); j < G0 + G; ++j)
                acc[j - G0] = __builtin_fma(sv.Xw[((size_t)q * KP + j) * W + lane], r, acc[j - G0]);
        }
    }
    column_sums_g<G>(acc, accR + G0);
}

template <int KP, int PPL, int NTR = 0, int HARM = 0, class RGen>
__device__ __forceinline__ void ztr_pass(const SeriesView &sv, QuadLds<KP, PPL> &wl, double *rb,
                                         RGen gen, double &sse_out, double (&ztr)[PPL])
{
    const int lane = lane_id();
    const int S = sv.S;
    double sse = 0.0, rt1 = 0.0, rt2 = 0.0;
    double rr[NTR > 0 ? NTR : 1];
    if (NTR > 0) {
#pragma unroll
        for (int q = 0; q < (NTR > 0 ? NTR : 1); ++q) rr[q] = 0.0;
    }
    auto row_step = [&](int q) -> double {
        const bool valid = q < sv.cnt;
        const int idx = q * W + lane;
        const unsigned cwv = valid ? (unsigned)sv.cw[idx] : 0u;
        const int c = (int)(cwv & 0xffu), cprev = (int)(cwv >> 8);
        const double ti = valid ? sv.tw[idx] : 0.0;
        double r = gen(q, idx, c, ti);
        if (!valid) r = 0.0;
        sse = __builtin_fma(r, r, sse);
        rt1 = __builtin_fma(r, ti, rt1);
        rt2 = rt2 + r;
        for (int j = cprev; j < c; ++j) { wl.tp1[j] = rt1; wl.tp2[j] = rt2; }
        return r;
    };
    if (NTR > 0) {
#pragma unroll 1
        for (int q = sv.NT - 1; q >= NTR; --q) rb[q * W + lane] = row_step(q);
        const int q1 = sv.NT < NTR ? sv.NT : NTR;
#pragma unroll 1
        for (int q = q1 - 1; q >= 0; --q) rr[NTR > 0 ? q : 0] = row_step(q);
    } else {
#pragma unroll 1
        for (int q = sv.NT - 1; q >= 0; --q) rb[q * W + lane] = row_step(q);
    }
    sse_out = bfly_sum(sse);
    const double s1 = suffix_scan(rt1), s2v = suffix_scan(rt2);
    wl.tot1[lane] = s1; wl.tot2[lane] = s2v;
    if (lane == 0) { wl.tot1[W] = 0.0; wl.tot2[W] = 0.0; }
// ... 560 lines not shown
            else rv = cur.w[c];
            r[c] = (valid && qq >= 0) ? rv : 0.0;
            rt1[c] = __builtin_fma(r[c], ti, rt1[c]); rt2[c] = rt2[c] + r[c];
        }
        for (int j = cprev; j < cseg; ++j) {
#pragma unroll
            for (int c = 0; c < NC; ++c) { tp1[c][j] = rt1[c]; tp2[c][j] = rt2[c]; }
        }
        harm_row<HARM>(bp, [&](int j, double v) {
#pragma unroll
            for (int c = 0; c < NC; ++c) acc[c][j] = __builtin_fma(v, r[c], acc[c][j]);
        });
        if (has_xd) {
            const double *xp = sv.Xw + (size_t)q * KP * W + lane;
#pragma unroll
            for (int j = KF; j < KP; ++j) {
                const double xv = xp[j * W];
#pragma unroll
                for (int c = 0; c < NC; ++c) acc[c][j] = __builtin_fma(xv, r[c], acc[c][j]);
            }
        }
        cur = nxt;
    }
#pragma unroll
    for (int c = 0; c < NC; ++c) {
        const double s1 = suffix_scan(rt1[c]), s2v = suffix_scan(rt2[c]);
        tot1[c][lane] = s1; tot2[c][lane] = s2v;
        if (lane == 0) { tot1[c][W] = 0.0; tot2[c][W] = 0.0; }
    }
    constexpr int G8 = (KP / 8) * 8;
#pragma unroll
    for (int c = 0; c < NC; ++c) {
#pragma unroll
        for (int g0 = 0; g0 < G8; g0 += 8) {
            double ta[8];
#pragma unroll
            for (int u = 0; u < 8; ++u) ta[u] = acc[c][g0 + u];
            column_sums_g<8>(ta, accR[c] + g0);
        }
        if (KP % 8 != 0) {
            double ta[4];
#pragma unroll
            for (int u = 0; u < 4; ++u) ta[u] = acc[c][(G8 + u) < KP ? G8 + u : 0];
            column_sums_g<4>(ta, accR[c] + G8);
        }
    }
    wave_sync();
    {
        const int p = lane;
#pragma unroll
        for (int c = 0; c < NC; ++c) {
            double v = 0.0;
            if (p == 0) v = tot1[c][0];
            else if (p == 1) v = tot2[c][0];
            else if (p >= 3 && p < 3 + S) {
                const int j = p - 3, Lj = sv.Ljp_l[0];
                v = (tp1[c][j] + tot1[c][Lj + 1]) - sv.tcp_l[0] * (tp2[c][j] + tot2[c][Lj + 1]);
            } else if (p >= 3 + S && p < sv.P) {
                v = accR[c][p - 3 - S];
            }
            z[c] = v;
        }
    }
    wave_sync();
}

template <int KP, int PPL>
__global__ __launch_bounds__(64) void gram_build_kernel(QuadArgs qa, double *Mout)
{
    __shared__ QuadLds<KP, PPL> wl;
    const int q = blockIdx.x, lane = threadIdx.x;
    SeriesView sv;
    make_view_q<KP, PPL>(qa.f, 0, sv);
    double *out = Mout + (size_t)q * PPL * W;
    if (q == 2 || q >= sv.P) {
#pragma unroll
        for (int s = 0; s < PPL; ++s) out[s * W + lane] = 0.0;
        return;
    }
    double *rb = qa.rbuf + (size_t)q * qa.f.NTmax * W;
    double ztr[PPL];
    gram_column<KP, PPL>(sv, wl, rb, q, ztr);
#pragma unroll
    for (int s = 0; s < PPL; ++s) out[s * W + lane] = ztr[s];
}

template <int KP, int PPL>
__global__ __launch_bounds__(64) void gram_grids_kernel(QuadArgs qa, double *Mpre, int64_t g0)
{
    __shared__ QuadLds<KP, PPL> wl;
    const int q = blockIdx.x, lane = threadIdx.x;
    const int64_t g = g0 + blockIdx.y;
    SeriesView sv;
    make_view_grid<KP, PPL>(qa.f, g, 0, sv);
    double *out = Mpre + ((size_t)g * qa.P4 + q) * PPL * W;
    if (q == 2 || q >= sv.P) {
#pragma unroll
        for (int s = 0; s < PPL; ++s) out[s * W + lane] = 0.0;
        return;
    }
    double *rb = qa.rbuf + ((size_t)blockIdx.y * qa.P4 + q) * qa.f.NTmax * W;
    double ztr[PPL];
    gram_column<KP, PPL>(sv, wl, rb, q, ztr);
#pragma unroll
    for (int s = 0; s < PPL; ++s) out[s * W + lane] = ztr[s];
}

#ifdef TSF_QUAD_TIMING
#define QT_DECL long long qt_acc[8] = {0, 0, 0, 0, 0, 0, 0, 0}; long long qt_t0 = __builtin_readcyclecounter(), qt_start = qt_t0
#define QT_LAP(k) do { const long long t_ = __builtin_readcyclecounter(); qt_acc[k] += t_ - qt_t0; qt_t0 = t_; } while (0)
#define QT_FLUSH() do { if (qa.dbg && lane == 0) { qt_acc[7] = __builtin_readcyclecounter() - qt_start; for (int k_ = 0; k_ < 8; ++k_) qa.dbg[(size_t)n * 8 + k_] = qt_acc[k_]; } } while (0)
#else
#define QT_DECL do { } while (0)
#define QT_LAP(k) do { } while (0)
#define QT_FLUSH() do { } while (0)
#endif

__device__ __forceinline__ SeriesTab series_tab_wave(const SeriesView &sv, const GridTab &gt)
{
    SeriesTab st;
    st.cap = 0.0; st.floor_ = 0.0; st.k0 = 0.0; st.m0 = 0.0; st.y_scale = 1.0; st.status0 = 0; st.pad_ = 0;
    const int T = sv.T, NT = sv.NT;
    if (T < 2) { st.status0 = TSF_ST_TOO_FEW; return st; }
    const int lane = lane_id();
    double amax = 0.0, ymin = __builtin_huge_val(), ymax = -__builtin_huge_val();
    for (int i = lane; i < T; i += W) {
        const double v = load_y(sv.y_raw, sv.y_dtype, sv.y_base + i);
        amax = __builtin_fmax(amax, __builtin_fabs(v - 0.0));
        ymin = __builtin_fmin(ymin, v);
        ymax = __builtin_fmax(ymax, v);
    }
#pragma unroll
    for (int off = 1; off < W; off <<= 1) {
        amax = __builtin_fmax(amax, __shfl_xor(amax, off, W));
        ymin = __builtin_fmin(ymin, __shfl_xor(ymin, off, W));
        ymax = __builtin_fmax(ymax, __shfl_xor(ymax, off, W));
    }
    const double ys = (amax == 0.0) ? 1.0 : amax;
    const int i1 = gt.info.i1;
    const double t0 = sv.tw[0];
    const double t1 = sv.tw[(i1 - (i1 / NT) * NT) * W + i1 / NT];
    const double y0 = (load_y(sv.y_raw, sv.y_dtype, sv.y_base) - 0.0) / ys;
    const double y1 = (load_y(sv.y_raw, sv.y_dtype, sv.y_base + i1) - 0.0) / ys;
    const double Td = t1 - t0;
    st.k0 = (y1 - y0) / Td;
    st.m0 = y0 - st.k0 * t0;
    if (ymin == ymax) st.status0 = TSF_ST_CONSTANT;
    if (gt.cp_bad) st.status0 = TSF_ST_CHANGEPOINT;
    st.y_scale = ys;
    return st;
}

template <int KP, int PPL, int PQ, bool RAGGED, int MRS = W, bool HLDS = false, int MBATCH = 16, bool MREG = false, int NTR = 0, bool POOL = false,
          bool MPIPE = (TSF_QUAD_MPIPE != 0) && !POOL>
__device__ __forceinline__ bool fit_one_quad(const QuadArgs &qa, QuadLds<KP, PPL> *wlp, double *rb,
                                          const double *Mp, double *Mown, int64_t n, double *lanec,
                                          double *hist = nullptr, GramX *gx = nullptr,
                                          QuadWave<PPL> *qw = nullptr, const QuadPool *pool = nullptr)
{
    static_assert(!POOL || (!RAGGED && PQ > 0 && PPL == 1), "pooled trend tables: the shared-M one-slot kernel");
    double *const dl_w = POOL ? qw->dl : wlp->th;
    double *const ref_w = POOL ? qw->ref : wlp->ref;
    double *const cvec_w = POOL ? qw->cvec : wlp->cvec;
    const FitArgs &a = qa.f;
    const DevSpec *sp = a.sp;
    const int lane = lane_id();
    const int P4 = qa.P4;
    const double eps = 2.220446049250313e-16;
    const double c1 = 1e-4, c2 = 0.9, minAlpha = 1e-12, min_range = 1e-16;
    const int maxLSIts = 20, maxLSRestarts = 10;
    SeriesView sv;
    make_view_q<KP, PPL>(a, n, sv);
    const SeriesTab st = a.y_raw ? series_tab_wave(sv, a.gtab[grid_index(a, n)]) : a.stab[n];
    sv.y_scl = st.y_scale;
    if (lane == 0) {
        a.y_scale[n] = st.y_scale;
        if (!a.aligned || n == 0) a.grid_out[a.aligned ? 0 : n] = a.gtab[grid_index(a, n)].info;
    }
    double xk[PPL], gk[PPL], pk[PPL], xk1[PPL], gk1[PPL];
#pragma unroll
    for (int s = 0; s < PPL; ++s) {
        const int p = lane + s * W;
        xk[s] = (p == 0) ? st.k0 : (p == 1 ? st.m0 : 0.0);
        gk[s] = 0.0; pk[s] = 0.0; xk1[s] = xk[s]; gk1[s] = 0.0;
    }
    if (st.status0 != 0) {
        if (st.status0 == TSF_ST_CONSTANT) {
#pragma unroll
            for (int s = 0; s < PPL; ++s) if (lane + s * W == 2) xk[s] = -20.72326583694641;
        }
        store_theta<PPL>(a, sv, n, xk, a.theta);
        if (lane == 0) { a.status[n] = st.status0; a.n_iter[n] = 0; a.n_eval[n] = 0; a.fval[n] = 0.0; }
        return false;
    }
    LaneConst<PPL> lk;
    quad_const_table(lanec + 3 * PPL * W, a.opt, qa.recenter_ratio);
    lane_consts<PPL>(sp, sv, lanec, lk);
    lk.ct = lanec + 3 * PPL * W;
    constexpr bool CT = HLDS && !RAGGED && !MREG && PQ > 0 && PPL == 1;
    const double *const ct = lk.ct;
    QT_DECL;
    if (RAGGED && MRS == W && qa.Mpre) {
        Mp = qa.Mpre + (size_t)grid_index(a, n) * P4 * PPL * W;
    } else if (RAGGED) {
        bool built = false;
        if constexpr (MREG && PPL == 1 && KP == 28) {
            if (qa.gram_harm == HARM_Y10_W3) {
                int qs[3] = {-1, -1, -1}, nq = 0;
#pragma unroll 1
                for (int q = 0; q <= P4; ++q) {
                    if (q < P4) {
                        const bool real = q != 2 && q < sv.P;
                        if (!real) { Mown[(size_t)q * W + lane] = 0.0; continue; }
                        qs[nq++] = q;
                        if (nq < 3) continue;
                    } else if (nq == 0) break;
                    double z[3];
                    gram_columns_harm<KP, HARM_Y10_W3, 3>(sv, *wlp, gx, qs, z);
#pragma unroll
                    for (int c = 0; c < 3; ++c) if (qs[c] >= 0) Mown[(size_t)qs[c] * W + lane] = z[c];
                    qs[0] = -1; qs[1] = -1; qs[2] = -1; nq = 0;
                }
                built = true;
            }
        }
        if (built) {
        } else if constexpr (MREG && PPL == 1) {
            int qprev = -1;
#pragma unroll 1
            for (int q = 0; q < P4; ++q) {
                const bool real = q != 2 && q < sv.P;
                if (!real) { Mown[(size_t)q * W + lane] = 0.0; continue; }
                if (qprev < 0) { qprev = q; continue; }
                double za, zb;
                gram_columns2<KP>(sv, *wlp, *gx, qprev, q, za, zb);
                Mown[(size_t)qprev * W + lane] = za;
                Mown[(size_t)q * W + lane] = zb;
                qprev = -1;
            }
            if (qprev >= 0) {
                double za, zb;
                gram_columns2<KP>(sv, *wlp, *gx, qprev, qprev, za, zb);
                Mown[(size_t)qprev * W + lane] = za;
            }
        } else {
#pragma unroll 1
        for (int q = 0; q < P4; ++q) {
            double col[PPL];
#pragma unroll
            for (int s = 0; s < PPL; ++s) col[s] = 0.0;
            if (q != 2 && q < sv.P) gram_column<KP, PPL>(sv, *wlp, rb, q, col);
            if (MRS == W) {
#pragma unroll
                for (int s = 0; s < PPL; ++s) Mown[((size_t)q * PPL + s) * W + lane] = col[s];
            } else if (lane < MRS) {
                Mown[(size_t)q * MRS + lane] = col[0];
            }
        }
        }
        Mp = Mown;
        QT_LAP(5);
    }
    double mreg[(MREG && PQ > 0) ? PQ : 1];
    if constexpr (MREG && PQ > 0) {
        static_assert(!MREG || (MRS == W && PPL == 1), "register M: one-slot kernels");
        const double *Msrc = Mp;
#pragma unroll
        for (int q = 0; q < PQ; ++q) mreg[q] = Msrc[(size_t)q * W + lane];
    } else {
        mreg[0] = 0.0;
    }

    double s0 = 0.0, q2 = 0.0;
    constexpr int QHR = HLDS ? 1 : QH;
    double ShR[QHR][PPL], YhR[QHR][PPL], rh[QH];
#pragma unroll
    for (int h = 0; h < QH; ++h) rh[h] = 0.0;
#pragma unroll
    for (int h = 0; h < QHR; ++h) {
#pragma unroll
        for (int s = 0; s < PPL; ++s) { ShR[h][s] = 0.0; YhR[h][s] = 0.0; }
    }
    int h0 = 0;
    double *const histS = hist, *const histY = hist + QH * PPL * W;
    double *const histR = hist + 2 * QH * PPL * W;

    double fk = 0.0, fk1 = 0.0, alpha = a.opt.init_alpha, gammak = 1.0;
    int itNum = 0, ret = 0, resetB = 0, hist_len = 0, since_rc = 0;
    double dfp = 0, c1dfp = 0, c2dfp = 0, alpha0 = 0, prevF = 0, prevDFp = 0;
    double alo = 0, aloF = 0, aloDFp = 0, ahi = 0, ahiF = 0, ahiDFp = 0;
    int nits = 0, lsRestarts = 0, zoom = 0, zit = 0;
    double gp = 0.0;
    bool gp_valid = false, pk1_scaled = false;
    double gp1s = 0.0;

    const int eval_limit = 64 * a.opt.max_iter + 1024;
    auto recenter = [&](double &fe_out) -> bool {
        double xe[PPL], ge[PPL], fe, sse_e, ztr_e[PPL];
#pragma unroll
        for (int s = 0; s < PPL; ++s) xe[s] = xk[s];
        sv.n_eval++;
        QT_LAP(2);
        bool bad;
        if constexpr (POOL) {
            const int slot = pool_acquire(*pool);
            unsigned char *sl = pool->slots + (size_t)slot * pool->slot_bytes;
            double *rbs = pool->slot_bytes > sizeof(QuadLds<KP, PPL>) ? reinterpret_cast<double *>(sl + sizeof(QuadLds<KP, PPL>)) : rb;
            bad = resid_eval_q<KP, PPL, NTR>(sv, *reinterpret_cast<QuadLds<KP, PPL> *>(sl), lk, rbs, xe, fe, ge, sse_e, ztr_e);
            pool_release(*pool, slot);
        } else if constexpr (RAGGED && MREG && PPL == 1 && KP == 28 && NTR == 0) {
            if (qa.gram_harm == HARM_Y10_W3) bad = resid_eval_q<KP, PPL, NTR, HARM_Y10_W3>(sv, *wlp, lk, rb, xe, fe, ge, sse_e, ztr_e);
            else bad = resid_eval_q<KP, PPL, NTR>(sv, *wlp, lk, rb, xe, fe, ge, sse_e, ztr_e);
        } else {
            bad = resid_eval_q<KP, PPL, NTR>(sv, *wlp, lk, rb, xe, fe, ge, sse_e, ztr_e);
        }
        QT_LAP(3);
        if (!bad) {
#pragma unroll
            for (int s = 0; s < PPL; ++s) {
                const int p = lane + s * W;
                ref_w[p] = (p == 2) ? 0.0 : xe[s];
                cvec_w[p] = ztr_e[s];
                gk[s] = ge[s];
            }
            s0 = sse_e; since_rc = 0; fk = UQ(fe);
            wave_sync();
        }
        fe_out = fe;
        return bad;
    };
    bool first = true, do_resid = true;
    for (;;) {
        QT_LAP(0);
        if (do_resid) {
            double fe0;
            const bool bad0 = recenter(fe0);
            if (first && bad0) { ret = TSF_ST_INIT_NONFINITE; fk = UQ(fe0); break; }
        }
        if (first) {
            first = false;
#pragma unroll
            for (int s = 0; s < PPL; ++s) { pk[s] = -gk[s]; gk1[s] = 0.0; xk1[s] = 0.0; }
        } else {
            double sk[PPL], yk[PPL];
#pragma unroll
            for (int s = 0; s < PPL; ++s) { sk[s] = xk[s] - xk1[s]; yk[s] = gk[s] - gk1[s]; }
            const double dots = bfly_sum4_lanes(pdot_part<PPL>(gk, gk), pdot_part<PPL>(sk, sk),
                                                pdot_part<PPL>(yk, sk), pdot_part<PPL>(yk, yk));
            const double g2sum = readlane_f64(dots, 0), s2sum = readlane_f64(dots, 2);
            auto norm_below = [&](double x2, int k_lo, int k_tol) -> bool {
                if (x2 < qc(ct, k_lo)) return true;
                if (x2 >= qc(ct, k_lo + 1)) return false;
                return __builtin_sqrt(x2) < qc(ct, k_tol);
            };
            double qnum = dpp_mov<0x07>(dots);
            if ((lane & 3) >= 2) qnum = 1.0;
            const double qden = dpp_mov<0x5D>(dots);
            const double qv = qnum / qden;
            if (resetB) {
                const double B0fact = readlane_f64(qv, 0);
                hist_len = 0;
                double ps[PPL];
#pragma unroll
                for (int s = 0; s < PPL; ++s) ps[s] = pk[s] / B0fact;
                gp1s = pdot<PPL>(gk1, ps);
                alpha = UQ(alpha * B0fact);
                pk1_scaled = true;
            } else {
                pk1_scaled = false;
            }
            gammak = readlane_f64(qv, 1);
            const double rho_new = readlane_f64(qv, 2);
            double Sh[QH][PPL], Yh[QH][PPL];
            if (HLDS) {
                if (resetB) h0 = 0;
                int slot;
                if (hist_len < QH) {
                    slot = h0 + hist_len; if (slot >= QH) slot -= QH;
                    hist_len++;
                } else {
                    slot = h0; h0 = (h0 + 1 == QH) ? 0 : h0 + 1;
                }
#pragma unroll
                for (int s = 0; s < PPL; ++s) {
                    histS[(slot * PPL + s) * W + lane] = sk[s];
                    histY[(slot * PPL + s) * W + lane] = yk[s];
                }
                histR[slot] = rho_new;
                wave_sync();
#pragma unroll
                for (int h = 0; h < QH; ++h) {
                    int sl = h0 + h; if (sl >= QH) sl -= QH;
#pragma unroll
                    for (int s = 0; s < PPL; ++s) {
                        Sh[h][s] = histS[(sl * PPL + s) * W + lane];
                        Yh[h][s] = histY[(sl * PPL + s) * W + lane];
                    }
                    rh[h] = histR[sl];
                }
            } else {
            if (hist_len < QH) {
#pragma unroll
                for (int h = 0; h < QH; ++h) {
                    if (h == hist_len) {
                        rh[h] = rho_new;
#pragma unroll
                        for (int s = 0; s < PPL; ++s) { ShR[h][s] = sk[s]; YhR[h][s] = yk[s]; }
                    }
                }
                hist_len++;
            } else {
#pragma unroll
                for (int h = 0; h + 1 < QH; ++h) {
                    rh[h] = rh[h + 1];
#pragma unroll
                    for (int s = 0; s < PPL; ++s) { ShR[h][s] = ShR[h + 1][s]; YhR[h][s] = YhR[h + 1][s]; }
                }
                rh[QH - 1] = rho_new;
#pragma unroll
                for (int s = 0; s < PPL; ++s) { ShR[QH - 1][s] = sk[s]; YhR[QH - 1][s] = yk[s]; }
            }
#pragma unroll
            for (int h = 0; h < QH; ++h) {
#pragma unroll
                for (int s = 0; s < PPL; ++s) { Sh[h][s] = ShR[HLDS ? 0 : h][s]; Yh[h][s] = YhR[HLDS ? 0 : h][s]; }
            }
            }
            double alphas[QH];
            QT_LAP(1);
#pragma unroll
            for (int s = 0; s < PPL; ++s) pk[s] = -gk[s];
#pragma unroll
            for (int h = QH - 1; h >= 0; --h) {
                if (h < hist_len) {
                    const double aa = lane63(rh[h] * pdot_l63<PPL>(Sh[h], pk));
#pragma unroll
                    for (int s = 0; s < PPL; ++s) pk[s] = __builtin_fma(-aa, Yh[h][s], pk[s]);
                    alphas[h] = aa;
                }
            }
#pragma unroll
            for (int s = 0; s < PPL; ++s) pk[s] = pk[s] * gammak;
#pragma unroll
            for (int h = 0; h < QH; ++h) {
                if (h < hist_len) {
                    const double cc = lane63(alphas[h] - rh[h] * pdot_l63<PPL>(Yh[h], pk));
#pragma unroll
                    for (int s = 0; s < PPL; ++s) pk[s] = __builtin_fma(cc, Sh[h][s], pk[s]);
                }
            }
            QT_LAP(6);
            const double dF = __builtin_fabs(fk1 - fk);
            const double fmaxv = __builtin_fmax(__builtin_fabs(fk1),
                                                __builtin_fmax(__builtin_fabs(fk), 1.0));
            gp = pdot<PPL>(gk, pk);
            gp_valid = true;
            auto relgrad_below = [&]() -> bool {
                const double m = __builtin_fmax(__builtin_fabs(fk), 1.0), ngp = -gp;
                if (ngp < qc(ct, QC_RELGRAD_LO) * m) return true;
                if (ngp > qc(ct, QC_RELGRAD_HI) * m) return false;
                return ngp / m < qc(ct, QC_TOL_REL_GRAD);
            };
            if constexpr (CT) {
                if (dF < qc(ct, QC_TOL_OBJ)) ret = TSF_ST_ABSF;
                else if (dF < qc(ct, QC_TOL_REL_OBJ) * fmaxv) ret = TSF_ST_RELF;
                else if (norm_below(g2sum, QC_GRAD2_LO, QC_TOL_GRAD)) ret = TSF_ST_ABSGRAD;
                else if (relgrad_below()) ret = TSF_ST_RELGRAD;
                else if (norm_below(s2sum, QC_PARAM2_LO, QC_TOL_PARAM)) ret = TSF_ST_ABSX;
                else if (itNum >= a.opt.max_iter) ret = TSF_ST_MAXIT;
                else ret = 0;
            } else {
                if (dF < a.opt.tol_obj) ret = TSF_ST_ABSF;
                else if (dF < a.opt.tol_rel_obj_eps * fmaxv) ret = TSF_ST_RELF;
                else if (__builtin_sqrt(g2sum) < a.opt.tol_grad) ret = TSF_ST_ABSGRAD;
                else if (-gp / __builtin_fmax(__builtin_fabs(fk), 1.0) < a.opt.tol_rel_grad_eps) ret = TSF_ST_RELGRAD;
                else if (__builtin_sqrt(s2sum) < a.opt.tol_param) ret = TSF_ST_ABSX;
                else if (itNum >= a.opt.max_iter) ret = TSF_ST_MAXIT;
                else ret = 0;
            }

            QT_LAP(1);
            if (ret != 0) break;
        }
        itNum++;
        resetB = (itNum == 1) ? 1 : 0;
        bool accepted = false;
        for (;;) {
            if (resetB) {
#pragma unroll
                for (int s = 0; s < PPL; ++s) pk[s] = -gk[s];
                gp_valid = false;
            }
            if (!gp_valid) gp = pdot<PPL>(gk, pk);
            gp_valid = false;
            if (itNum > 1 && resetB != 2) {
                const double gp1 = pk1_scaled ? gp1s : dfp;
                const double ci = cubic_interp6(gp1, alpha, fk - fk1, gp, minAlpha, 1.0);
                alpha = UQ(__builtin_fmin(1.0, 1.01 * ci));
            } else {
                alpha = CT ? qc(ct, QC_INIT_ALPHA) : a.opt.init_alpha;
            }
            dfp = gp;
            c1dfp = UQ(c1 * dfp); c2dfp = UQ(c2 * dfp);
            alpha0 = minAlpha; prevF = fk; prevDFp = dfp;
            nits = 0; lsRestarts = 0; zoom = 0; zit = 0;

            bool ls_fail = false, pre = true;
            for (;;) {
                if (pre) {
                    if (!zoom) {
                        if (nits >= maxLSIts) ls_fail = true;
                    } else {
                        zit++;
                        if (__builtin_fabs(alo - ahi) < min_range) {
                            ls_fail = true;
                        } else if (zit % 5 == 0) {
                            alpha = UQ(0.5 * (alo + ahi));
                        } else {
                            const double d1 = aloDFp + ahiDFp - 3.0 * (aloF - ahiF) / (alo - ahi);
                            double d2 = __builtin_sqrt(d1 * d1 - aloDFp * ahiDFp);
                            if (ahi < alo) d2 = -d2;
                            alpha = ahi - (ahi - alo) * (ahiDFp + d2 - d1) / (ahiDFp - aloDFp + 2.0 * d2);
                            const double lo = __builtin_fmin(alo, ahi), hi = __builtin_fmax(alo, ahi),
                                         w = __builtin_fabs(alo - ahi);
                            if (!finite_f64(alpha) || alpha < lo + 0.01 * w || alpha > hi - 0.01 * w)
                                alpha = 0.5 * (alo + ahi);
                            alpha = UQ(alpha);
                        }
                    }

                    if (ls_fail) break;
                }
                pre = true;
                if (sv.n_eval >= eval_limit) { ret = TSF_ST_EVAL_LIMIT; break; }
                double xe[PPL], ge[PPL], fe;
#pragma unroll
                for (int s = 0; s < PPL; ++s) { xk1[s] = __builtin_fma(alpha, pk[s], xk[s]); xe[s] = xk1[s]; }
                sv.n_eval++;
                QT_LAP(2);
                const bool bad = gram_eval_q<PPL, PQ, MRS, MBATCH, MREG, MPIPE, (TSF_QUAD_EXPTAB != 0)>(sv, lk, Mp, P4, xe, ref_w, cvec_w, s0, fe, ge, q2, dl_w, mreg);
                QT_LAP(4);
#pragma unroll
                for (int s = 0; s < PPL; ++s) gk1[s] = ge[s];
                const double f1 = UQ(fe);
                if (bad) {
                    if (!zoom) {
                        if (lsRestarts >= maxLSRestarts) ls_fail = true;
                        else { alpha = UQ(0.5 * (alpha0 + alpha)); lsRestarts++; }
                    } else {
                        alpha = UQ(0.5 * (alpha + __builtin_fmin(alo, ahi)));
                        if (__builtin_fabs(__builtin_fmin(alo, ahi) - alpha) < min_range) ls_fail = true;
                    }
                    if (ls_fail) break;
                    pre = false;
                    continue;
                }
                const double newDFp = pdot<PPL>(gk1, pk);
                QT_LAP(5);
                bool ls_ok = false;
                if (!zoom) {
                    lsRestarts = 0;
                    if (f1 > fk + alpha * c1dfp || (f1 >= prevF && nits > 0)) {
                        zoom = 1; alo = alpha0; aloF = prevF; aloDFp = prevDFp;
                        ahi = alpha; ahiF = f1; ahiDFp = newDFp;
                    } else if (__builtin_fabs(newDFp) <= -c2dfp) {
                        ls_ok = true;
                    } else if (newDFp >= 0) {
                        zoom = 1; alo = alpha; aloF = f1; aloDFp = newDFp;
                        ahi = alpha0; ahiF = prevF; ahiDFp = prevDFp;
                    } else {
                        alpha0 = alpha; prevF = f1; prevDFp = newDFp;
                        alpha = UQ(alpha * 10.0);
                        nits++;
                    }
                } else {
                    if (f1 > (fk + alpha * c1dfp) || f1 >= aloF) {
                        ahi = alpha; ahiF = f1; ahiDFp = newDFp;
                    } else if (__builtin_fabs(newDFp) <= -c2dfp) {
                        ls_ok = true;
                    } else {
                        if (newDFp * (ahi - alo) >= 0) { ahi = alo; ahiF = aloF; ahiDFp = aloDFp; }
                        alo = alpha; aloF = f1; aloDFp = newDFp;
                    }
                }
                if (ls_ok) { fk1 = f1; accepted = true; break; }
            }
            if (accepted || ret != 0) break;
            if (resetB) { ret = TSF_ST_LSFAIL; break; }
            resetB = 2;
        }
        if (!accepted) break;
        { const double tf = fk; fk = fk1; fk1 = tf; }
#pragma unroll
        for (int s = 0; s < PPL; ++s) {
            const double tx = xk[s]; xk[s] = xk1[s]; xk1[s] = tx;
            const double tg = gk[s]; gk[s] = gk1[s]; gk1[s] = tg;
        }
        since_rc++;
        do_resid = q2 > (CT ? qc(ct, QC_RC_RATIO) : qa.recenter_ratio) * s0 || since_rc >= qa.recenter_every;
    }
    store_theta<PPL>(a, sv, n, xk, a.theta);
    if (lane == 0) { a.status[n] = ret; a.n_iter[n] = itNum; a.n_eval[n] = sv.n_eval; a.fval[n] = fk; }
    QT_FLUSH();
    return false;
}

enum { QM_LDS = 0, QM_GLOBAL = 1, QM_RAGGED = 2, QM_RAGGED_LDS = 3, QM_RAGGED_REG = 4, QM_GLOBAL_REG = 5 };

template <int PPL>
constexpr size_t quad_hist_bytes(bool hlds) { return hlds ? sizeof(double) * (2 * QH * PPL * W + 8) : 0; }

template <int KP, int PPL, int NW, int MMODE, int PQ, bool RLDS, bool HLDS = false, int NTR = 0, bool RPOOL = false>
__global__ __launch_bounds__(NW * 64, quad_waves_per_simd(quad_three_waves(MMODE, PPL, HLDS), NW)) void fit_quad_kernel(QuadArgs qa, int pool_slots, int pool_slot_bytes)
{
    static_assert(NTR == 0 || (!RLDS && MMODE == QM_LDS), "register-resident weights: the shared-M kernel without LDS staging");
    static_assert(!RPOOL || (MMODE == QM_LDS && !RLDS && PPL == 1 && PQ > 0 && HLDS), "pooled trend tables: the shared-M one-slot kernel");
    extern __shared__ __align__(16) unsigned char smem[];
    const FitArgs &a = qa.f;
    const int lane = lane_id(), wid = (int)threadIdx.x >> 6;
    const int P4 = qa.P4;
    constexpr bool MLDS = MMODE == QM_LDS;
    double *Ml = reinterpret_cast<double *>(smem);
    const size_t m_bytes = MLDS ? sizeof(double) * (size_t)P4 * PPL * W : 0;
    constexpr bool RAGGED_K = MMODE == QM_RAGGED || MMODE == QM_RAGGED_LDS || MMODE == QM_RAGGED_REG;
    constexpr size_t LCB = quad_lanec_bytes<PPL>();
    double *lanec = reinterpret_cast<double *>(smem + m_bytes + (RAGGED_K ? LCB * wid : 0));
    const size_t off_wl = m_bytes + LCB * (RAGGED_K ? NW : 1);
    constexpr size_t WLB = RPOOL ? sizeof(QuadWave<PPL>) : sizeof(QuadLds<KP, PPL>);
    QuadLds<KP, PPL> *wlp = RPOOL ? nullptr : reinterpret_cast<QuadLds<KP, PPL> *>(smem + off_wl + WLB * wid);
    QuadWave<PPL> *qw = RPOOL ? reinterpret_cast<QuadWave<PPL> *>(smem + off_wl + WLB * wid) : nullptr;
    constexpr size_t HB = quad_hist_bytes<PPL>(HLDS);
    const size_t off_hist = off_wl + WLB * NW;
    double *hist = HLDS ? reinterpret_cast<double *>(smem + off_hist + HB * wid) : nullptr;
    const size_t off_rb = off_hist + HB * NW;
    QuadPool pool;
    pool.locks = reinterpret_cast<int *>(smem + off_rb);
    pool.slots = smem + off_rb + QUAD_POOL_LOCK_BYTES;
    pool.ns = pool_slots;
    pool.first = __builtin_amdgcn_readfirstlane(wid % (pool_slots > 0 ? pool_slots : 1));
    pool.slot_bytes = (unsigned)pool_slot_bytes;
    if (RPOOL) {
        for (int i = threadIdx.x; i < (int)(QUAD_POOL_LOCK_BYTES / sizeof(int)); i += NW * 64) pool.locks[i] = 0;
        for (int i = threadIdx.x; i < pool_slots * (PPL * W + W); i += NW * 64) {
            const int sl = i / (PPL * W + W), k = i - sl * (PPL * W + W);
            reinterpret_cast<QuadLds<KP, PPL> *>(pool.slots + (size_t)sl * pool.slot_bytes)->th[k] = 0.0;
        }
    }
    if (MLDS) {
        for (int i = threadIdx.x; i < P4 * PPL * W; i += NW * 64) Ml[i] = qa.Mg[i];
        __syncthreads();
    }
    const double *Mp = MLDS ? Ml : qa.Mg;
    const size_t rb_bytes = RLDS ? sizeof(double) * (size_t)NW * a.NTmax * W : 0;
    double *Mown = (MMODE == QM_RAGGED || MMODE == QM_RAGGED_REG) ? qa.Mslot + ((size_t)blockIdx.x * NW + wid) * (size_t)P4 * PPL * W
                 : (MMODE == QM_RAGGED_LDS) ? reinterpret_cast<double *>(smem + off_rb + rb_bytes) +
                                               (size_t)wid * (PQ * PQ + W)
                                            : nullptr;
    constexpr int MRS = (MMODE == QM_RAGGED_LDS) ? PQ : W;
    if (MMODE == QM_RAGGED_LDS) {
        Mown[PQ * PQ + lane] = 0.0;
        wave_sync();
    }
    double *rb = RLDS ? reinterpret_cast<double *>(smem + off_rb) + (size_t)wid * a.NTmax * W
                      : qa.rbuf + ((size_t)blockIdx.x * NW + wid) * a.NTmax * W;
    GramX *gx = (MMODE == QM_RAGGED_REG && RLDS) ? reinterpret_cast<GramX *>(rb) : nullptr;
    if (RPOOL) {
        for (int i = lane; i < PPL * W; i += W) qw->dl[i] = 0.0;
    } else {
        for (int i = lane; i < PPL * W + W; i += W) wlp->th[i] = 0.0;
    }
    wave_sync();

    for (;;) {
        int n32 = atomicAdd(qa.counter, lane == 0 ? 1 : 0);
        n32 = __builtin_amdgcn_readfirstlane(n32);
        if (n32 >= a.N) break;
        const int64_t n = a.order ? (int64_t)a.order[n32] : (int64_t)n32;
        fit_one_quad<KP, PPL, PQ, RAGGED_K, MRS, HLDS,
                     ((quad_three_waves(MMODE, PPL, HLDS) || MMODE == QM_RAGGED_REG || MMODE == QM_GLOBAL_REG) ? 8 : 16),
                     MMODE == QM_RAGGED_REG || MMODE == QM_GLOBAL_REG, NTR, RPOOL>(qa, wlp, rb, Mp, Mown, n, lanec, hist, gx, qw, &pool);
    }
}


template <int KP, int PQ, int NTR>
__global__ __launch_bounds__(64) void eval_quad_kernel(QuadArgs qa, const double *theta_ref)
{
    extern __shared__ __align__(16) unsigned char smem[];
    const FitArgs &a = qa.f;
    const int lane = lane_id();
    double *Ml = reinterpret_cast<double *>(smem);
    const size_t m_bytes = sizeof(double) * (size_t)PQ * W;
    double *lanec = reinterpret_cast<double *>(smem + m_bytes);
    QuadLds<KP, 1> &wl = *reinterpret_cast<QuadLds<KP, 1> *>(smem + m_bytes + quad_lanec_bytes<1>());
    for (int i = lane; i < PQ * W; i += W) Ml[i] = qa.Mg[i];
    for (int i = lane; i < 2 * W; i += W) wl.th[i] = 0.0;
    wave_sync();
    double *rb = qa.rbuf + (size_t)blockIdx.x * a.NTmax * W;
    for (int64_t n = blockIdx.x; n < a.N; n += gridDim.x) {
        SeriesView sv;
        make_view_q<KP, 1>(a, n, sv);
        LaneConst<1> lk;
        quad_const_table(lanec + 3 * W, a.opt, qa.recenter_ratio);
        lane_consts<1>(a.sp, sv, lanec, lk);
        lk.ct = lanec + 3 * W;
        double xr[1], gr[1], fr, s0, ztr[1];
        load_theta<1>(a, sv, n, theta_ref, xr);
        const bool bad_ref = resid_eval_q<KP, 1, NTR>(sv, wl, lk, rb, xr, fr, gr, s0, ztr);
        wl.ref[lane] = (lane == 2) ? 0.0 : xr[0];
        wl.cvec[lane] = ztr[0];
        wave_sync();
        double th[1], g[1], f, q2;
        load_theta<1>(a, sv, n, a.theta_in, th);
        const double mreg[1] = {0.0};
        const bool bad = gram_eval_q<1, PQ, W, 8, false, true, (TSF_QUAD_EXPTAB != 0)>(sv, lk, Ml, qa.P4, th, wl.ref, wl.cvec, s0, f, g, q2, wl.th, mreg);
        store_theta<1, false>(a, sv, n, g, a.grad_out);
        if (lane == 0) { a.fval[n] = f; a.status[n] = (bad || bad_ref) ? 1 : 0; }
        wave_sync();
    }
}

}
```

### time_series_spark_amd/csrc/tsf_quad_launch.h

```cpp
#pragma once
#include "tsf_quad_kernels.h"
#include "tsf_launch.h"
#include <cstdio>
#include <cstdlib>
#include <cstring>
#include <vector>

#ifndef TSF_QUAD_NW
#define TSF_QUAD_NW 8
#endif
#ifndef TSF_QUAD_NW3
#define TSF_QUAD_NW3 12
#endif
#ifndef TSF_QUAD_NTR
#define TSF_QUAD_NTR 12
#endif
#ifndef TSF_QUAD_NW4
#define TSF_QUAD_NW4 16
#endif
#ifndef TSF_QUAD_POOL_MIN
#define TSF_QUAD_POOL_MIN 3
#endif
#ifndef TSF_QUAD_POOL_RB_MIN
#define TSF_QUAD_POOL_RB_MIN 4
#endif
#ifndef TSF_QUAD_W4_MIN_PER_SLOT
#define TSF_QUAD_W4_MIN_PER_SLOT 8
#endif
#ifndef TSF_QUAD_W4_DEFAULT
#define TSF_QUAD_W4_DEFAULT -1
#endif
#ifndef TSF_QUAD_NW2G
#define TSF_QUAD_NW2G 8
#endif
#ifndef TSF_QUAD_NW2
#define TSF_QUAD_NW2 4
#endif

namespace tsf {

template <int PPL, int MMODE>
struct QuadShape {
    static constexpr bool HL = true;
    static constexpr int NW = (PPL == 2) ? (MMODE == QM_GLOBAL ? TSF_QUAD_NW2G : TSF_QUAD_NW2) : (quad_three_waves(MMODE, PPL, HL) ? TSF_QUAD_NW3 : TSF_QUAD_NW);
};

template <int PPL>
static size_t quad_pool_base_bytes(int P4, int nw)
{
    return sizeof(double) * (size_t)P4 * PPL * W + quad_lanec_bytes<PPL>() +
           (sizeof(QuadWave<PPL>) + quad_hist_bytes<PPL>(true)) * (size_t)nw + QUAD_POOL_LOCK_BYTES;
}

template <int KP, int PPL, int MMODE, int PQ, bool RLDS, int NTR = 0, bool RPOOL = false>
static int launch_quad_rl(const QuadPlan &qp, const QuadArgs &qa_in, double *Mg, hipStream_t st, int pool_slots = 0, int pool_slot_bytes = 0)
{
    constexpr int NW = RPOOL ? TSF_QUAD_NW4 : QuadShape<PPL, MMODE>::NW;
    constexpr bool MLDS = MMODE == QM_LDS;
    constexpr bool HL = QuadShape<PPL, MMODE>::HL;
    const QuadArgs &qa = qa_in;
    int64_t blocks = qp.n_cu;
    if (blocks > (qa.f.N + NW - 1) / NW) blocks = (qa.f.N + NW - 1) / NW;
    if (blocks < 1) blocks = 1;
    if (MMODE != QM_RAGGED && MMODE != QM_RAGGED_REG) {
        hipLaunchKernelGGL((gram_build_kernel<KP, PPL>), dim3((unsigned)qp.P4), dim3(64), 0, st, qa, Mg);
        hipError_t e = hipGetLastError();
        if (e != hipSuccess) return (int)e;
    }
    const size_t lds = RPOOL ? quad_pool_base_bytes<PPL>(qp.P4, NW) + (size_t)pool_slot_bytes * (size_t)pool_slots
                     : (MLDS ? sizeof(double) * (size_t)qp.P4 * PPL * W : 0) + quad_lanec_bytes<PPL>() * ((MMODE == QM_RAGGED || MMODE == QM_RAGGED_REG) ? NW : 1) +
                       (sizeof(QuadLds<KP, PPL>) + quad_hist_bytes<PPL>(HL)) * NW +
                       (RLDS ? sizeof(double) * (size_t)NW * qa.f.NTmax * W : 0);
    hipFuncSetAttribute((const void *)fit_quad_kernel<KP, PPL, NW, MMODE, PQ, RLDS, HL, NTR, RPOOL>,
                            hipFuncAttributeMaxDynamicSharedMemorySize, 160 * 1024);
#ifdef TSF_QUAD_TIMING
    {
        QuadArgs qb = qa;
        const size_t nb = sizeof(long long) * 8 * (size_t)qa.f.N;
        hipMalloc((void **)&qb.dbg, nb);
        hipMemsetAsync(qb.dbg, 0, nb, st);
        hipLaunchKernelGGL((fit_quad_kernel<KP, PPL, NW, MMODE, PQ, RLDS, HL, NTR, RPOOL>), dim3((unsigned)blocks), dim3(NW * 64), lds, st, qb, pool_slots, pool_slot_bytes);
        hipStreamSynchronize(st);
        std::vector<long long> h(8 * (size_t)qa.f.N);
        hipMemcpy(h.data(), qb.dbg, nb, hipMemcpyDeviceToHost);
        double sum[8] = {0};
        long long mx = 0;
        for (int64_t i = 0; i < qa.f.N; ++i) { for (int k = 0; k < 8; ++k) sum[k] += (double)h[i * 8 + k]; if (h[i * 8 + 7] > mx) mx = h[i * 8 + 7]; }
        fprintf(stderr, "[quad-timing] N %lld waves/CU %d pool %d mean cycles/series: misc %.0f post %.0f (+ two-loop %.0f) ls %.0f resid %.0f gram %.0f newDFp %.0f | total %.0f max %lld\n",
                (long long)qa.f.N, NW, pool_slots, sum[0] / qa.f.N, sum[1] / qa.f.N, sum[6] / qa.f.N, sum[2] / qa.f.N, sum[3] / qa.f.N, sum[4] / qa.f.N, sum[5] / qa.f.N, sum[7] / qa.f.N, mx);
        hipFree(qb.dbg);
        return (int)hipGetLastError();
    }
#endif
    hipLaunchKernelGGL((fit_quad_kernel<KP, PPL, NW, MMODE, PQ, RLDS, HL, NTR, RPOOL>), dim3((unsigned)blocks), dim3(NW * 64), lds, st, qa, pool_slots, pool_slot_bytes);
    return (int)hipGetLastError();
}

template <int KP, int PPL, int MMODE, int PQ>
static int launch_quad_mm(const QuadPlan &qp, const QuadArgs &qa, double *Mg, hipStream_t st)
{
    constexpr int NW = QuadShape<PPL, MMODE>::NW;
    constexpr bool HL = QuadShape<PPL, MMODE>::HL;
    if constexpr (MMODE == QM_LDS && PPL == 1 && PQ > 0) {
        const int e = qp.opt ? qp.opt[TSF_OPT_QUAD_W4] : -1;
        const int forced = e >= 0 ? e : TSF_QUAD_W4_DEFAULT;
        const size_t pbase = quad_pool_base_bytes<PPL>(qp.P4, TSF_QUAD_NW4);
        const size_t avail = pbase < 160 * 1024 ? 160 * 1024 - pbase : 0;
        size_t slot = sizeof(QuadLds<KP, PPL>) + sizeof(double) * (size_t)qa.f.NTmax * W;
        if (avail / slot < TSF_QUAD_POOL_RB_MIN) slot = sizeof(QuadLds<KP, PPL>);
        int ns = (int)(avail / slot);
        if (ns > TSF_QUAD_NW4) ns = TSF_QUAD_NW4;
        if (forced > 0 && forced < ns) ns = forced;
        if (forced != 0 && ns >= (forced > 0 ? 1 : TSF_QUAD_POOL_MIN) &&
            (forced > 0 || qa.f.N >= (int64_t)TSF_QUAD_W4_MIN_PER_SLOT * TSF_QUAD_NW4 * qp.n_cu))
            return launch_quad_rl<KP, PPL, MMODE, PQ, false, 0, true>(qp, qa, Mg, st, ns, (int)slot);
    }
    const size_t base = (MMODE == QM_LDS ? sizeof(double) * (size_t)qp.P4 * PPL * W : 0) + quad_lanec_bytes<PPL>() * ((MMODE == QM_RAGGED || MMODE == QM_RAGGED_REG) ? NW : 1) +
                        (sizeof(QuadLds<KP, PPL>) + quad_hist_bytes<PPL>(HL)) * NW;
    const size_t rbytes = sizeof(double) * (size_t)NW * qa.f.NTmax * W;
    if (base + rbytes <= 160 * 1024) return launch_quad_rl<KP, PPL, MMODE, PQ, true>(qp, qa, Mg, st);
    if constexpr (MMODE == QM_LDS && PPL == 1 && PQ > 0) {
        if (!(qp.opt && qp.opt[TSF_OPT_QUAD_RREG] == 0))
            return launch_quad_rl<KP, PPL, MMODE, PQ, false, TSF_QUAD_NTR>(qp, qa, Mg, st);
    }
    return launch_quad_rl<KP, PPL, MMODE, PQ, false>(qp, qa, Mg, st);
}

}
```

### time_series_spark_amd/forecaster.py

```python
import ctypes
import os

import numpy as np

from . import _lib, parallel

DAY_NS = 86400 * 10 ** 9


class ModelSpec(object):

    def __init__(self, growth='linear', seasonality_mode='additive', n_changepoints=25,
                 changepoint_range=0.8, changepoint_prior_scale=0.05,
                 seasonality_prior_scale=10.0, holidays_prior_scale=10.0,
                 seasonalities=None, extra=None, holidays=None, changepoints=None, **lbfgs):
        if growth not in ('linear', 'logistic'):
            raise ValueError("Parameter 'growth' should be 'linear' or 'logistic'.")
        if seasonality_mode not in ('additive', 'multiplicative'):
            raise ValueError("seasonality_mode must be 'additive' or 'multiplicative'")
        if changepoint_range < 0 or changepoint_range > 1:
            raise ValueError("Parameter 'changepoint_range' must be in [0, 1]")
        self.growth = growth
        self.seasonality_mode = seasonality_mode
        self.changepoints = None if changepoints is None else changepoints_ns(changepoints)
# ... 664 lines not shown
        return np.concatenate([[0], np.cumsum(self.n_holdout)]).astype(np.int64)

    @property
    def metric_offsets(self):
        return np.concatenate([[0], np.cumsum(self.n_metric)]).astype(np.int64)


def _cv_args(horizon, period, initial, rolling_window):
    a = _lib.TsfCvArgs()
    a.horizon_ns = int(horizon)
    a.period_ns = -1 if period is None else int(period)
    a.initial_ns = -1 if initial is None else int(initial)
    a.rolling_window = float(rolling_window)
    return a


def _cv_panel(ds_ns, y, offsets):
    ds_ns = np.ascontiguousarray(ds_ns, dtype=np.int64)
    y = np.ascontiguousarray(y)
    if offsets is None:
        if y.ndim != 2 or y.shape[1] != ds_ns.shape[0]:
            raise ValueError('aligned panel: y must be [N][T] with T == len(ds)')
        return ds_ns, y, None, y.shape[0], ds_ns.shape[0]
    offsets = np.ascontiguousarray(offsets, dtype=np.int64)
    if y.ndim != 1 or y.shape[0] != ds_ns.shape[0] or offsets[-1] != y.shape[0]:
        raise ValueError('ragged panel: ds / y must be 1-D with offsets[-1] rows')
    return ds_ns, y, offsets, len(offsets) - 1, 0


def cv_plan(ds_ns, horizon, period=None, initial=None, rolling_window=0.1, offsets=None, N=1):
    L = _lib.load()
    ds_ns = np.ascontiguousarray(ds_ns, dtype=np.int64)
    if offsets is not None:
        offsets = np.ascontiguousarray(offsets, dtype=np.int64)
        N, T = len(offsets) - 1, 0
    else:
        T = len(ds_ns)
    a = _cv_args(horizon, period, initial, rolling_window)
    nf, st = np.zeros(N, np.int32), np.zeros(N, np.int32)
    nh, nm = np.zeros(N, np.int64), np.zeros(N, np.int64)
    args = (N, T, _lib._ptr(offsets), ds_ns.ctypes.data, ctypes.byref(a), nf.ctypes.data, st.ctypes.data,
            nh.ctypes.data, nm.ctypes.data)
    if L.tsf_cv_plan(*args, None, None, None) != 0:
        raise ValueError('tsf_cv_plan: bad arguments (horizon > 0, rolling_window in [0, 1], sorted panel)')
    F = int(nf.sum())
    cut, hist, hold = np.zeros(F, np.int64), np.zeros(F, np.int32), np.zeros(F, np.int32)
    if L.tsf_cv_plan(*args, cut.ctypes.data, hist.ctypes.data, hold.ctypes.data) != 0:
        raise ValueError('tsf_cv_plan failed')
    return {'n_folds': nf, 'status': st, 'n_holdout': nh, 'n_metric': nm, 'cutoff': cut, 'hist_rows': hist,
            'hold_rows': hold}


def cross_validate(spec, ds_ns, y, horizon, period=None, initial=None, offsets=None, floor=None, cap=None, extra=None,
                   rolling_window=0.1, intervals=False, uncertainty_samples=1000, interval_width=0.8, seed=0,
                   series_key=None, ctx=None, devices=None):
    ds_ns, y, offsets, N, T = _cv_panel(ds_ns, y, offsets)
    fl = _opt_f64(floor, N, 'floor')
    cp = _opt_f64(cap, N, 'cap')
    key = None if series_key is None else np.ascontiguousarray(series_key, dtype=np.int64)
    if key is not None and key.shape != (N,):
        raise ValueError('series_key must be [N]')
    devs = None if ctx is not None else resolve_devices(devices)
    kw = dict(rolling_window=rolling_window, intervals=intervals, uncertainty_samples=uncertainty_samples,
              interval_width=interval_width, seed=seed)
    if devs and N >= 2 * MIN_SERIES_PER_DEVICE:
        parts = min(len(devs), N // MIN_SERIES_PER_DEVICE)
        lens = np.full(N, T, np.int64) if offsets is None else np.diff(offsets)
        cuts = _cuts(lens, parts)
        key = np.arange(N, dtype=np.int64) if key is None else key
        ex = None if extra is None else np.asarray(extra)

        def one(c, a, b):
            if offsets is None:
                return cross_validate(spec, ds_ns, y[a:b], horizon, period, initial, None,
                                      None if fl is None else fl[a:b], None if cp is None else cp[a:b], extra,
                                      series_key=key[a:b], ctx=c, **kw)
            r0, r1 = int(offsets[a]), int(offsets[b])
            return cross_validate(spec, ds_ns[r0:r1], y[r0:r1], horizon, period, initial, offsets[a:b + 1] - r0,
                                  None if fl is None else fl[a:b], None if cp is None else cp[a:b],
                                  None if ex is None else ex[:, r0:r1], series_key=key[a:b], ctx=c, **kw)
        blocks = [(c, int(a), int(b)) for c, a, b in zip(_contexts(devs[:parts]), cuts[:-1], cuts[1:]) if b > a]
        parts_res = _run_blocks(one, blocks)
        return _merge_cv(spec, parts_res, [a for _, a, _ in blocks], intervals)
    ctx = ctx or get_context()
    L = _lib.load()
    cs = spec.to_c()
    ex = None
    if spec.extra:
        ex = np.ascontiguousarray(extra, dtype=np.float64)
        if ex.shape != (len(spec.extra), len(ds_ns)):
            raise ValueError('extra must be [n_extra][len(ds)]')
    plan = cv_plan(ds_ns, horizon, period, initial, rolling_window, offsets=offsets, N=N)
    F, R, M = int(plan['n_folds'].sum()), int(plan['n_holdout'].sum()), int(plan['n_metric'].sum())
    fout, farrs = _alloc_out(F, spec.theta_stride, F)
    yhat = np.zeros(R)
    lo = np.zeros(R) if intervals else None
    hi = np.zeros(R) if intervals else None
    hz = np.zeros(M, np.int64)
    mse, rmse, mae, mape = np.zeros(M), np.zeros(M), np.zeros(M), np.zeros(M)
    cov = np.zeros(M) if intervals else None
    sst = np.zeros(N, np.int32)
    out = _lib.TsfCvOut(fout, yhat.ctypes.data, _lib._ptr(lo), _lib._ptr(hi), hz.ctypes.data, mse.ctypes.data,
                        rmse.ctypes.data, mae.ctypes.data, mape.ctypes.data, _lib._ptr(cov), sst.ctypes.data)
    a = _cv_args(horizon, period, initial, rolling_window)
    rc = L.tsf_cross_validate(ctx.handle, ctypes.byref(cs), N, T, _lib._ptr(offsets), ds_ns.ctypes.data, y.ctypes.data,
                              _lib.y_dtype_code(y), _lib._ptr(fl), _lib._ptr(cp), _lib._ptr(ex), ctypes.byref(a),
                              _lib._ptr(key), int(uncertainty_samples) if intervals else 0, float(interval_width),
                              int(seed), ctypes.byref(out))
    ctx.check(rc)
    fold_series = np.repeat(np.arange(N, dtype=np.int64), plan['n_folds'])
    start = (np.zeros(N, np.int64) if offsets is None else offsets[:-1])[fold_series] + plan['hist_rows']
    ridx = np.repeat(start - np.concatenate([[0], np.cumsum(plan['hold_rows'])[:-1]]), plan['hold_rows']) + np.arange(R)
    row_fold = np.repeat(np.arange(F, dtype=np.int64), plan['hold_rows'])
    if offsets is None:
        y_rows = y[fold_series[row_fold], ridx].astype(np.float64)
    else:
        y_rows = y[ridx].astype(np.float64)
    return CVResult(spec=spec, status=sst, n_folds=plan['n_folds'], n_holdout=plan['n_holdout'], n_metric=plan['n_metric'],
                    fold_series=fold_series, cutoff=plan['cutoff'], hist_rows=plan['hist_rows'], hold_rows=plan['hold_rows'],
                    fit=FitResult(spec, *farrs), row_fold=row_fold, ds=ds_ns[ridx], y=y_rows, yhat=yhat,
                    yhat_lower=lo, yhat_upper=hi,
                    metric_series=np.repeat(np.arange(N, dtype=np.int64), plan['n_metric']), horizon=hz, mse=mse,
                    rmse=rmse, mae=mae, mape=mape, coverage=cov)


def _merge_cv(spec, parts, firsts, intervals):
    cat = lambda k, p=parts: np.concatenate([getattr(x, k) for x in p])
    f_first = np.cumsum([0] + [len(p.cutoff) for p in parts])
    shifted = lambda k, base: np.concatenate([getattr(p, k) + b for p, b in zip(parts, base)])
    return CVResult(spec=spec, status=cat('status'), n_folds=cat('n_folds'), n_holdout=cat('n_holdout'),
                    n_metric=cat('n_metric'), fold_series=shifted('fold_series', firsts), cutoff=cat('cutoff'),
                    hist_rows=cat('hist_rows'), hold_rows=cat('hold_rows'),
                    fit=_merge_fits(spec, [p.fit for p in parts], shared_grid=False),
                    row_fold=shifted('row_fold', f_first[:-1]), ds=cat('ds'), y=cat('y'), yhat=cat('yhat'),
                    yhat_lower=cat('yhat_lower') if intervals else None, yhat_upper=cat('yhat_upper') if intervals else None,
                    metric_series=shifted('metric_series', firsts), horizon=cat('horizon'), mse=cat('mse'),
                    rmse=cat('rmse'), mae=cat('mae'), mape=cat('mape'), coverage=cat('coverage') if intervals else None)


def performance_metrics(cv):
    import pandas as pd
    d = {'series': cv.metric_series, 'horizon': cv.horizon, 'mse': cv.mse, 'rmse': cv.rmse, 'mae': cv.mae,
         'mape': cv.mape}
    if cv.coverage is not None:
        d['coverage'] = cv.coverage
    return pd.DataFrame(d)


def last_cv_grids(ctx=None):
    ctx = ctx or get_context()
    g, n = ctypes.c_int64(), ctypes.c_int32()
    ctx.check(_lib.load().tsf_last_cv_grids(ctx.handle, ctypes.byref(g), ctypes.byref(n)))
    return int(g.value), int(n.value)



TUNE_AXES = ('changepoint_prior_scale', 'seasonality_prior_scale', 'holidays_prior_scale')


def _n_holiday_columns(spec):
    from . import features
    return len(features.holiday_columns(spec.holidays)[0]) if spec.holidays else 0


def tune_candidates(spec, grid):
    import itertools
    if not isinstance(grid, dict) or not grid:
        raise ValueError('grid must be a non-empty dict over %s' % (TUNE_AXES,))
    unknown = sorted(set(grid) - set(TUNE_AXES))
    if unknown:
        raise ValueError('unknown grid axes %s (tunable: %s)' % (unknown, TUNE_AXES))
    n_hol = _n_holiday_columns(spec)
    if 'seasonality_prior_scale' in grid and not spec.seasonalities:
        raise ValueError('grid over seasonality_prior_scale, but the model has no seasonality')
    if 'holidays_prior_scale' in grid and n_hol == 0:
        raise ValueError('grid over holidays_prior_scale, but the model has no holidays')
    axes = [k for k in TUNE_AXES if k in grid]
    values = []
    for k in axes:
        v = np.asarray(grid[k], dtype=np.float64).ravel()
        if v.size == 0:
            raise ValueError('grid axis %s is empty' % k)
        if not (np.isfinite(v).all() and (v > 0).all()):
            raise ValueError('grid axis %s: prior scales must be finite and > 0' % k)
        values.append(v)
    cands, params = [], {k: [] for k in axes}
    for combo in itertools.product(*values):
        d = spec.to_dict()
        d['seasonalities'] = [dict(s) for s in spec.seasonalities]
        d['extra'] = [dict(e) for e in spec.extra]
        for e in d['extra'][n_hol:]:
            e.setdefault('prior_scale', spec.holidays_prior_scale)
        for k, v in zip(axes, combo):
            v = float(v)
            d[k] = v
            params[k].append(v)
            if k == 'seasonality_prior_scale':
                for s in d['seasonalities']:
                    s['prior_scale'] = v
            elif k == 'holidays_prior_scale':
                for e in d['extra'][:n_hol]:
                    e['prior_scale'] = v
        cands.append(ModelSpec.from_dict(d))
    return cands, {k: np.array(v) for k, v in params.items()}


def _effective_scales(spec, cands):
    n_hol = _n_holiday_columns(spec)
    cs = [c.to_c() for c in cands]
    return {'changepoint_prior_scale': np.array([c.changepoint_prior_scale for c in cs]),
            'seasonality_prior_scale': np.array([c.seas_prior_scale[0] if c.n_seas else np.nan for c in cs]),
            'holidays_prior_scale': np.array([c.extra_prior_scale[0] if n_hol else np.nan for c in cs])}


class TuneResult(object):

    def __init__(self, **kw):
        self.__dict__.update(kw)

    def spec_of(self, n):
        b = int(self.best[n])
        return self.candidates[b] if b >= 0 else self.spec

    def frame(self):
        import pandas as pd
        N = len(self.best)
        ok = self.best >= 0
        eff = _effective_scales(self.spec, list(self.candidates) + [self.spec])
        pick = np.where(ok, self.best, len(self.candidates))
        d = {'series': np.arange(N, dtype=np.int64), 'candidate': self.best.astype(np.int64),
             'status': self.status.astype(np.int64)}
        for k in TUNE_AXES:
            d[k] = eff[k][pick]
        d['metric'] = np.full(N, self.metric, dtype=object)
        d['score'] = np.where(ok, self.score[np.arange(N), np.maximum(self.best, 0)], np.nan)
        return pd.DataFrame(d)


def tune(spec, ds_ns, y, horizon, period=None, initial=None, offsets=None, floor=None, cap=None, extra=None,
         grid=None, candidates=None, metric='rmse', refit=True, ctx=None, devices=None):
    if (grid is None) == (candidates is None):
        raise ValueError('give exactly one of grid and candidates')
    if grid is not None:
        cands, params = tune_candidates(spec, grid)
    else:
        cands = list(candidates)
        if not cands:
            raise ValueError('candidates is empty')
        params = _effective_scales(spec, cands)
    if len(cands) > _lib.TUNE_MAX_CAND:
        raise ValueError('at most %d candidates' % _lib.TUNE_MAX_CAND)
    if metric not in _lib.TUNE_METRICS:
        raise ValueError('metric must be one of %s' % sorted(_lib.TUNE_METRICS))
    ds_ns, y, offsets, N, T = _cv_panel(ds_ns, y, offsets)
    fl = _opt_f64(floor, N, 'floor')
    cp = _opt_f64(cap, N, 'cap')
    C = len(cands)

    def result(score, cst, best, sst, fit):
        return TuneResult(spec=spec, candidates=cands, params=params, metric=metric, score=score, cand_status=cst,
                          best=best, status=sst, fit=fit)
    devs = None if ctx is not None else resolve_devices(devices)
    if devs and N >= 2 * MIN_SERIES_PER_DEVICE:
        parts = min(len(devs), N // MIN_SERIES_PER_DEVICE)
        lens = np.full(N, T, np.int64) if offsets is None else np.diff(offsets)
        cuts = _cuts(lens, parts)
        ex = None if extra is None else np.asarray(extra)

        def one(c, a, b):
            kw = dict(candidates=cands, metric=metric, refit=refit, ctx=c)
            if offsets is None:
                return tune(spec, ds_ns, y[a:b], horizon, period, initial, None, None if fl is None else fl[a:b],
                            None if cp is None else cp[a:b], extra, **kw)
            r0, r1 = int(offsets[a]), int(offsets[b])
            return tune(spec, ds_ns[r0:r1], y[r0:r1], horizon, period, initial, offsets[a:b + 1] - r0,
                        None if fl is None else fl[a:b], None if cp is None else cp[a:b],
                        None if ex is None else ex[:, r0:r1], **kw)
        blocks = [(c, int(a), int(b)) for c, a, b in zip(_contexts(devs[:parts]), cuts[:-1], cuts[1:]) if b > a]
        pr = _run_blocks(one, blocks)
        cat = lambda k: np.concatenate([getattr(p, k) for p in pr])
        fit = _merge_fits(spec, [p.fit for p in pr], shared_grid=offsets is None) if refit else None
        return result(cat('score'), cat('cand_status'), cat('best'), cat('status'), fit)
    ctx = ctx or get_context()
    L = _lib.load()
    ex = None
    if spec.extra:
        ex = np.ascontiguousarray(extra, dtype=np.float64)
        if ex.shape != (len(spec.extra), len(ds_ns)):
            raise ValueError('extra must be [n_extra][len(ds)]')
    base = spec.to_c()
    carr = (_lib.TsfSpec * C)(*[c.to_c() for c in cands])
    score = np.zeros((N, C))
    cst = np.zeros((N, C), np.int32)
    best = np.zeros(N, np.int32)
    sst = np.zeros(N, np.int32)
    fout, farrs = _alloc_out(N, spec.theta_stride, 1 if offsets is None else N) if refit else (_lib.TsfFitOut(), None)
    out = _lib.TsfTuneOut(score.ctypes.data, cst.ctypes.data, best.ctypes.data, sst.ctypes.data, fout)
    a = _cv_args(horizon, period, initial, 1.0)
    rc = L.tsf_tune(ctx.handle, ctypes.byref(base), carr, C, N, T, _lib._ptr(offsets), ds_ns.ctypes.data, y.ctypes.data,
                    _lib.y_dtype_code(y), _lib._ptr(fl), _lib._ptr(cp), _lib._ptr(ex), ctypes.byref(a),
                    _lib.TUNE_METRICS[metric], int(bool(refit)), ctypes.byref(out))
    ctx.check(rc)
    return result(score, cst, best, sst, FitResult(spec, *farrs) if refit else None)


def last_tune_counts(ctx=None):
# ... 5 lines not shown
```

Before: 1.126 million.

## Hand over straggler quad fits to a register-M resume kernel at tail

New measurement: 1.108 million. 1.6% lower.

```diff
diff --git a/include/tsf_dev.h b/include/tsf_dev.h
--- a/include/tsf_dev.h
+++ b/include/tsf_dev.h
@@ -26,6 +26,7 @@
     TSF_OPT_DEBUG_ASYNC_SCRATCH,
     TSF_OPT_COOP_TAIL,
     TSF_OPT_MAP_DIRECT,
+    TSF_OPT_QUAD_TAIL,
     TSF_OPT_COUNT
 };
 int tsf_set_option(tsf_ctx *ctx, int option, int value);
@@ -47,6 +48,7 @@
 int tsf_profile_read(tsf_ctx *ctx, float *ms_out, int32_t max_n, int32_t *n_out);
 int tsf_last_fit_kernel_ms(tsf_ctx *ctx, float *ms_out);
 int tsf_last_fit_route(tsf_ctx *ctx, int32_t *sparse_columns);
+int tsf_last_quad_tail(tsf_ctx *ctx, int32_t *handed_over, int32_t *resumed, int32_t *alive_at_flag);
 int tsf_last_cv_grids(const tsf_ctx *ctx, int64_t *n_grids, int32_t *n_launches);
 int tsf_last_tune_counts(const tsf_ctx *ctx, int32_t *expand_launches, int32_t *fit_launches);
 
diff --git a/time_series_spark_amd/_lib.py b/time_series_spark_amd/_lib.py
--- a/time_series_spark_amd/_lib.py
+++ b/time_series_spark_amd/_lib.py
@@ -95,7 +95,7 @@
            'tsf_spec_size', 'tsf_grid_info_size', 'tsf_spec_K', 'tsf_theta_stride',
            'tsf_fit_aligned', 'tsf_fit_aligned_dev', 'tsf_fit_ragged', 'tsf_fit_ragged_dev',
            'tsf_predict', 'tsf_predict_dev', 'tsf_predict_intervals', 'tsf_predict_intervals_dev', 'tsf_predict_components', 'tsf_predict_components_dev', 'tsf_eval', 'tsf_eval_quadratic', 'tsf_design', 'tsf_selftest_math',
-           'tsf_set_option', 'tsf_get_option', 'tsf_set_cost_hints', 'tsf_set_profiling', 'tsf_profile_read', 'tsf_last_fit_kernel_ms', 'tsf_last_fit_route',
+           'tsf_set_option', 'tsf_get_option', 'tsf_set_cost_hints', 'tsf_set_profiling', 'tsf_profile_read', 'tsf_last_fit_kernel_ms', 'tsf_last_fit_route', 'tsf_last_quad_tail',
            'tsf_cv_plan', 'tsf_cross_validate', 'tsf_last_cv_grids', 'tsf_tune', 'tsf_last_tune_counts',
            'tsf_pack_rows', 'tsf_pack_rows_typed', 'tsf_pack_fetch', 'tsf_pack_flags', 'tsf_pack_free', 'tsf_model_blobs',
            'tsf_csv_read', 'tsf_csv_fetch', 'tsf_csv_columns', 'tsf_csv_malformed', 'tsf_csv_free', 'tsf_csv_write_forecasts', 'tsf_csv_write_forecasts_i32',
@@ -110,7 +110,7 @@
 
 OPTIONS = ['harm', 'lattice', 'sparse_extra', 'fit_grouped', 'gram_share', 'grid_order', 'grid_share', 'ragged_split',
            'quad_reg', 'quad_m2_lds', 'quad_w4', 'quad_rreg', 'newton_batch', 'newton_flags', 'newton_ns', 'newton_lcap',
-           'newton_fill', 'quad_raw_y', 'debug_async_scratch', 'coop_tail', 'map_direct']
+           'newton_fill', 'quad_raw_y', 'debug_async_scratch', 'coop_tail', 'map_direct', 'quad_tail']
 
 _lib = None
 
@@ -168,6 +168,7 @@
     L.tsf_profile_read.argtypes = [vp, ctypes.POINTER(ctypes.c_float), i32, ctypes.POINTER(i32)]
     L.tsf_last_fit_kernel_ms.argtypes = [vp, ctypes.POINTER(ctypes.c_float)]
     L.tsf_last_fit_route.argtypes = [vp, ctypes.POINTER(ctypes.c_int32)]
+    L.tsf_last_quad_tail.argtypes = [vp] + [ctypes.POINTER(ctypes.c_int32)] * 3
     L.tsf_cv_plan.argtypes = [i64, i32, vp, vp, ctypes.POINTER(TsfCvArgs), vp, vp, vp, vp, vp, vp, vp]
     L.tsf_cross_validate.argtypes = [vp, psp, i64, i32, vp, vp, vp, i32, vp, vp, vp, ctypes.POINTER(TsfCvArgs), vp, i32,
                                      ctypes.c_double, ctypes.c_uint64, ctypes.POINTER(TsfCvOut)]
diff --git a/time_series_spark_amd/csrc/tsf_api.hip b/time_series_spark_amd/csrc/tsf_api.hip
--- a/time_series_spark_amd/csrc/tsf_api.hip
+++ b/time_series_spark_amd/csrc/tsf_api.hip
@@ -49,6 +49,7 @@
     int order_busy[2];
     int n_cu;
     const int *last_sp_flag;
+    const int *last_qtail;
     int opt[TSF_OPT_COUNT];
     int profiling;
     hipEvent_t ev0[TSF_PROFILE_RING], ev1[TSF_PROFILE_RING];
@@ -100,6 +101,7 @@
     c->order_ev[0] = c->order_ev[1] = nullptr; c->order_busy[0] = c->order_busy[1] = 0;
     c->profiling = 0; c->ev_created = 0; c->ev_count = 0;
     c->last_sp_flag = nullptr;
+    c->last_qtail = nullptr;
     c->last_n_grids = 0; c->cv_grids = 0; c->cv_launches = 0; c->tune_expand = 0; c->tune_fits = 0;
     for (int i = 0; i < TSF_OPT_COUNT; ++i) c->opt[i] = -1;
     if (hipMalloc((void **)&c->d_spec, sizeof(DevSpec)) != hipSuccess) { delete c; return -2; }
@@ -335,6 +337,7 @@
         (void)hipGetLastError();
     }
     ctx->last_sp_flag = nullptr;
+    ctx->last_qtail = nullptr;
     if (ctx->ws) { HIP_TRY(ctx, hipFree(ctx->ws)); ctx->ws = nullptr; ctx->ws_bytes = 0; }
     HIP_TRY(ctx, hipMalloc(&ctx->ws, bytes));
     ctx->ws_bytes = bytes;
@@ -520,8 +523,10 @@
         map_harm = hs.harm;
     const int bw_ns = (harm || gram_harm || map_harm) ? hs.n_seas : 0;
     const bool raw_y = quad && spec->converge != TSF_CONVERGE_MAP && ctx->opt[TSF_OPT_QUAD_RAW_Y] != 0;
+    const int qtail_slots = (quad && aligned && qp.PPL == 1 && qp.P4 != 64 && ctx->opt[TSF_OPT_QUAD_TAIL] != 0)
+                                ? (int)(N < (int64_t)QT_MAIN_WAVES * ctx->n_cu ? N : (int64_t)QT_MAIN_WAVES * ctx->n_cu) : 0;
     const WsLayout l = ws_layout(N, n_grids, NTmax, hs.KP, qp.P4, qp.slots, (quad || newton_quad) && !aligned, lat_U, &mp,
-                                 coop_slots, coop_stride, quad_pre, sparse_try, bw_ns, raw_y);
+                                 qtail_slots ? qtail_slots : coop_slots, qtail_slots ? QT_REC : coop_stride, quad_pre, sparse_try, bw_ns, raw_y);
     rc = ensure_ws(ctx, l.total, N, NTmax, !aligned);
     if (rc) return rc;
     char *ws = (char *)ctx->ws;
@@ -594,6 +599,7 @@
     }
     a.opt_coop_sparse = ctx->opt[TSF_OPT_SPARSE_EXTRA] != 2 ? 1 : 0;
     ctx->last_sp_flag = nullptr;
+    ctx->last_qtail = nullptr;
     if (sparse_try) {
         a.sp_meta = (const uint32_t *)(ws + l.spm); a.sp_prog = (const unsigned long long *)(ws + l.spp);
         a.sp_flag = (int *)(ws + l.counter) + 8;
@@ -643,7 +649,9 @@
         qa.dbg = nullptr; qa.nb_buf = nullptr; qa.nb_bytes = 0;
         qa.Mpre = quad_pre ? qa.Mg : nullptr; qa.n_pre = quad_pre;
         qa.gram_harm = gram_harm;
-        HIP_TRY(ctx, hipMemsetAsync(qa.counter, 0, sizeof(int), st));
+        if (qtail_slots) { qa.tail_list = (int *)(ws + l.clist); qa.tail_rec = (double *)(ws + l.cslots); qa.tail_cap = qtail_slots; }
+        ctx->last_qtail = qtail_slots ? qa.counter : nullptr;
+        HIP_TRY(ctx, hipMemsetAsync(qa.counter, 0, sizeof(int) * QTC_N, st));
         lrc = -1;
         if (spec->converge == TSF_CONVERGE_MAP && qp.PPL == 1 && ctx->opt[TSF_OPT_MAP_DIRECT] != 0) {
             qa.f.map_max_iter = spec->map_max_iter; qa.f.map_tol = spec->map_tol;
@@ -1753,6 +1761,19 @@
     HIP_TRY(ctx, hipDeviceSynchronize());
     HIP_TRY(ctx, hipMemcpy(&bad, ctx->last_sp_flag, sizeof(int), hipMemcpyDeviceToHost));
     *sparse_columns = bad ? 0 : 1;
+    return 0;
+}
+
+extern "C" int tsf_last_quad_tail(tsf_ctx *ctx, int32_t *handed_over, int32_t *resumed, int32_t *alive_at_flag)
+{
+    if (!ctx || !handed_over || !resumed || !alive_at_flag) return -1;
+    *handed_over = 0; *resumed = 0; *alive_at_flag = -1;
+    if (!ctx->last_qtail) return 0;
+    int w[QTC_N];
+    HIP_TRY(ctx, hipSetDevice(ctx->device));
+    HIP_TRY(ctx, hipDeviceSynchronize());
+    HIP_TRY(ctx, hipMemcpy(w, ctx->last_qtail, sizeof(w), hipMemcpyDeviceToHost));
+    *handed_over = w[QTC_LEN]; *resumed = w[QTC_RESUMED]; *alive_at_flag = w[QTC_ALIVE] - 1;
     return 0;
 }
 
diff --git a/time_series_spark_amd/csrc/tsf_inst_quad4.hip b/time_series_spark_amd/csrc/tsf_inst_quad4.hip
--- a/time_series_spark_amd/csrc/tsf_inst_quad4.hip
+++ b/time_series_spark_amd/csrc/tsf_inst_quad4.hip
@@ -15,4 +15,17 @@
     }
 }
 
+int launch_quad_tail(int KP, const QuadPlan &qp, const QuadArgs &qa, hipStream_t st)
+{
+    switch (KP * 100 + qp.P4) {
+    case 840: return launch_quad_resume<8, 40>(qp, qa, st);
+    case 856: return launch_quad_resume<8, 56>(qp, qa, st);
+    case 1640: return launch_quad_resume<16, 40>(qp, qa, st);
+    case 1656: return launch_quad_resume<16, 56>(qp, qa, st);
+    case 2840: return launch_quad_resume<28, 40>(qp, qa, st);
+    case 2856: return launch_quad_resume<28, 56>(qp, qa, st);
+    default: return -1;
+    }
 }
+
+}
diff --git a/time_series_spark_amd/csrc/tsf_launch.h b/time_series_spark_amd/csrc/tsf_launch.h
--- a/time_series_spark_amd/csrc/tsf_launch.h
+++ b/time_series_spark_amd/csrc/tsf_launch.h
@@ -13,6 +13,7 @@
 int launch_eval_quad(int KP, const QuadPlan &qp, const QuadArgs &qa, double *Mg, const double *theta_ref, hipStream_t st);
 int launch_map_quad(int KP, const QuadPlan &qp, const QuadArgs &qa, double *Mg, int PM, hipStream_t st);
 int launch_quad_aligned_reg(int KP, const QuadPlan &qp, const QuadArgs &qa, double *Mg, hipStream_t st);
+int launch_quad_tail(int KP, const QuadPlan &qp, const QuadArgs &qa, hipStream_t st);
 int launch_newton_quad(int KP, const QuadPlan &qp, const QuadArgs &qa, double *Mg, int PM, int n_cu, hipStream_t st);
 size_t newton_batch_scratch_bytes(int KP, int PM, int64_t N, int NTmax, int n_cu, const int *opt);
 int launch_g0m0(int KP, const FitArgs &a, int eval_only, hipStream_t st);
diff --git a/time_series_spark_amd/csrc/tsf_quad_kernels.h b/time_series_spark_amd/csrc/tsf_quad_kernels.h
--- a/time_series_spark_amd/csrc/tsf_quad_kernels.h
+++ b/time_series_spark_amd/csrc/tsf_quad_kernels.h
@@ -27,7 +27,22 @@
     void *nb_buf;
     size_t nb_bytes;
     int gram_harm;
+    int *tail_list;
+    double *tail_rec;
+    int tail_cap, tail_at;
 };
+
+enum { QT_XK = 0, QT_GK, QT_XK1, QT_GK1, QT_PK, QT_REF, QT_CVEC, QT_S , QT_Y = QT_S + QH ,
+       QT_SCAL = QT_Y + QH, QT_ROWS };
+enum { QTS_FK = 0, QTS_FK1, QTS_ALPHA, QTS_S0, QTS_DFP, QTS_RHO ,
+       QTS_ITNUM = QTS_RHO + QH, QTS_RESETB, QTS_HIST_LEN, QTS_SINCE_RC, QTS_DO_RESID, QTS_N_EVAL, QTS_N };
+#ifndef TSF_QUAD_TAIL_POLL_EVERY
+#define TSF_QUAD_TAIL_POLL_EVERY 4
+#endif
+constexpr int QT_REC = QT_ROWS * W;
+constexpr int QT_MAIN_WAVES = 12;
+enum { QTC_HEAD = 0, QTC_DONE, QTC_FLAG, QTC_LEN, QTC_TAIL_HEAD, QTC_RESUMED, QTC_ALIVE, QTC_N };
+enum { QTAIL_NONE = 0, QTAIL_MAIN = 1, QTAIL_RESUME = 2 };
 
 template <int KP, int PPL>
 struct QuadLds {
@@ -894,13 +909,16 @@
 }
 
 template <int KP, int PPL, int PQ, bool RAGGED, int MRS = W, bool HLDS = false, int MBATCH = 16, bool MREG = false, int NTR = 0, bool POOL = false,
+          int TAIL = QTAIL_NONE,
           bool MPIPE = (TSF_QUAD_MPIPE != 0) && !POOL>
 __device__ __forceinline__ bool fit_one_quad(const QuadArgs &qa, QuadLds<KP, PPL> *wlp, double *rb,
                                           const double *Mp, double *Mown, int64_t n, double *lanec,
                                           double *hist = nullptr, GramX *gx = nullptr,
-                                          QuadWave<PPL> *qw = nullptr, const QuadPool *pool = nullptr)
+                                          QuadWave<PPL> *qw = nullptr, const QuadPool *pool = nullptr,
+                                          const double *rec = nullptr)
 {
     static_assert(!POOL || (!RAGGED && PQ > 0 && PPL == 1), "pooled trend tables: the shared-M one-slot kernel");
+    static_assert(TAIL == QTAIL_NONE || (HLDS && !RAGGED && !POOL && PQ > 0 && PPL == 1), "hand-over: aligned one-slot kernels with the history ring in LDS");
     double *const dl_w = POOL ? qw->dl : wlp->th;
     double *const ref_w = POOL ? qw->ref : wlp->ref;
     double *const cvec_w = POOL ? qw->cvec : wlp->cvec;
@@ -913,9 +931,14 @@
     const int maxLSIts = 20, maxLSRestarts = 10;
     SeriesView sv;
     make_view_q<KP, PPL>(a, n, sv);
-    const SeriesTab st = a.y_raw ? series_tab_wave(sv, a.gtab[grid_index(a, n)]) : a.stab[n];
+    SeriesTab st;
+    if constexpr (TAIL == QTAIL_RESUME) {
+        st.cap = 0.0; st.floor_ = 0.0; st.k0 = 0.0; st.m0 = 0.0; st.y_scale = UQ(a.y_scale[n]); st.status0 = 0; st.pad_ = 0;
+    } else {
+        st = a.y_raw ? series_tab_wave(sv, a.gtab[grid_index(a, n)]) : a.stab[n];
+    }
     sv.y_scl = st.y_scale;
-    if (lane == 0) {
+    if (TAIL != QTAIL_RESUME && lane == 0) {
         a.y_scale[n] = st.y_scale;
         if (!a.aligned || n == 0) a.grid_out[a.aligned ? 0 : n] = a.gtab[grid_index(a, n)].info;
     }
@@ -926,7 +949,7 @@
         xk[s] = (p == 0) ? st.k0 : (p == 1 ? st.m0 : 0.0);
         gk[s] = 0.0; pk[s] = 0.0; xk1[s] = xk[s]; gk1[s] = 0.0;
     }
-    if (st.status0 != 0) {
+    if (TAIL != QTAIL_RESUME && st.status0 != 0) {
         if (st.status0 == TSF_ST_CONSTANT) {
 #pragma unroll
             for (int s = 0; s < PPL; ++s) if (lane + s * W == 2) xk[s] = -20.72326583694641;
@@ -1072,8 +1095,34 @@
         return bad;
     };
     bool first = true, do_resid = true;
+    if constexpr (TAIL == QTAIL_RESUME) {
+        const double *r = rec + lane;
+        xk[0] = r[QT_XK * W]; gk[0] = r[QT_GK * W]; xk1[0] = r[QT_XK1 * W]; gk1[0] = r[QT_GK1 * W]; pk[0] = r[QT_PK * W];
+        ref_w[lane] = r[QT_REF * W]; cvec_w[lane] = r[QT_CVEC * W];
+#pragma unroll
+        for (int h = 0; h < QH; ++h) {
+            histS[h * W + lane] = r[(QT_S + h) * W];
+            histY[h * W + lane] = r[(QT_Y + h) * W];
+        }
+        const double sc = r[QT_SCAL * W];
+#pragma unroll
+        for (int h = 0; h < QH; ++h) histR[h] = readlane_f64(sc, QTS_RHO + h);
+        fk = readlane_f64(sc, QTS_FK); fk1 = readlane_f64(sc, QTS_FK1); alpha = readlane_f64(sc, QTS_ALPHA);
+        s0 = readlane_f64(sc, QTS_S0); dfp = readlane_f64(sc, QTS_DFP);
+        itNum = (int)readlane_f64(sc, QTS_ITNUM); resetB = (int)readlane_f64(sc, QTS_RESETB);
+        hist_len = (int)readlane_f64(sc, QTS_HIST_LEN); since_rc = (int)readlane_f64(sc, QTS_SINCE_RC);
+        do_resid = readlane_f64(sc, QTS_DO_RESID) != 0.0;
+        sv.n_eval = (int)readlane_f64(sc, QTS_N_EVAL);
+        first = false;
+        wave_sync();
+    }
     for (;;) {
         QT_LAP(0);
+        int hand_over = 0;
+        if constexpr (TAIL == QTAIL_MAIN) {
+            if ((itNum & (TSF_QUAD_TAIL_POLL_EVERY - 1)) == 0)
+                hand_over = __hip_atomic_load(qa.counter + QTC_FLAG, __ATOMIC_RELAXED, __HIP_MEMORY_SCOPE_AGENT);
+        }
         if (do_resid) {
             double fe0;
             const bool bad0 = recenter(fe0);
@@ -1340,10 +1389,45 @@
         }
         since_rc++;
         do_resid = q2 > (CT ? qc(ct, QC_RC_RATIO) : qa.recenter_ratio) * s0 || since_rc >= qa.recenter_every;
+        if constexpr (TAIL == QTAIL_MAIN) {
+            if (__builtin_amdgcn_readfirstlane(hand_over) != 0) {
+                int slot = atomicAdd(qa.counter + QTC_LEN, lane == 0 ? 1 : 0);
+                slot = __builtin_amdgcn_readfirstlane(slot);
+                if (slot < qa.tail_cap) {
+                    double *r = qa.tail_rec + (size_t)slot * QT_REC + lane;
+                    r[QT_XK * W] = xk[0]; r[QT_GK * W] = gk[0]; r[QT_XK1 * W] = xk1[0]; r[QT_GK1 * W] = gk1[0]; r[QT_PK * W] = pk[0];
+                    r[QT_REF * W] = ref_w[lane]; r[QT_CVEC * W] = cvec_w[lane];
+                    double rho = 0.0;
+#pragma unroll
+                    for (int h = 0; h < QH; ++h) {
+                        int sl = h0 + h; if (sl >= QH) sl -= QH;
+                        r[(QT_S + h) * W] = histS[sl * W + lane];
+                        r[(QT_Y + h) * W] = histY[sl * W + lane];
+                        if (lane == QTS_RHO + h) rho = histR[sl];
+                    }
+                    double sc = rho;
+                    if (lane == QTS_FK) sc = fk;
+                    if (lane == QTS_FK1) sc = fk1;
+                    if (lane == QTS_ALPHA) sc = alpha;
+                    if (lane == QTS_S0) sc = s0;
+                    if (lane == QTS_DFP) sc = dfp;
+                    if (lane == QTS_ITNUM) sc = (double)itNum;
+                    if (lane == QTS_RESETB) sc = (double)resetB;
+                    if (lane == QTS_HIST_LEN) sc = (double)hist_len;
+                    if (lane == QTS_SINCE_RC) sc = (double)since_rc;
+                    if (lane == QTS_DO_RESID) sc = do_resid ? 1.0 : 0.0;
+                    if (lane == QTS_N_EVAL) sc = (double)sv.n_eval;
+                    r[QT_SCAL * W] = sc;
+                    qa.tail_list[slot] = (int)n;
+                    QT_FLUSH();
+                    return true;
+                }
+            }
+        }
     }
     store_theta<PPL>(a, sv, n, xk, a.theta);
     if (lane == 0) { a.status[n] = ret; a.n_iter[n] = itNum; a.n_eval[n] = sv.n_eval; a.fval[n] = fk; }
-    QT_FLUSH();
+    if (TAIL != QTAIL_RESUME) QT_FLUSH();
     return false;
 }
 
@@ -1352,9 +1436,18 @@
 template <int PPL>
 constexpr size_t quad_hist_bytes(bool hlds) { return hlds ? sizeof(double) * (2 * QH * PPL * W + 8) : 0; }
 
-template <int KP, int PPL, int NW, int MMODE, int PQ, bool RLDS, bool HLDS = false, int NTR = 0, bool RPOOL = false>
+template <int KP, int PPL, int NW, int MMODE, int PQ, bool RLDS, bool HLDS = false, int NTR = 0, bool RPOOL = false, int TAIL = QTAIL_NONE>
 __global__ __launch_bounds__(NW * 64, quad_waves_per_simd(quad_three_waves(MMODE, PPL, HLDS), NW)) void fit_quad_kernel(QuadArgs qa, int pool_slots, int pool_slot_bytes)
 {
+    static_assert(TAIL != QTAIL_MAIN || (MMODE == QM_LDS && PPL == 1 && HLDS && !RPOOL), "the kernel that hands over: shared M in LDS, 12 waves");
+    static_assert(TAIL != QTAIL_RESUME || (MMODE == QM_GLOBAL_REG && PPL == 1 && HLDS && RLDS), "the kernel that resumes: shared M in registers");
+    int tail_len = 0;
+    if constexpr (TAIL == QTAIL_RESUME) {
+        tail_len = __hip_atomic_load(qa.counter + QTC_LEN, __ATOMIC_RELAXED, __HIP_MEMORY_SCOPE_AGENT);
+        tail_len = __builtin_amdgcn_readfirstlane(tail_len);
+        if (tail_len > qa.tail_cap) tail_len = qa.tail_cap;
+        if (tail_len <= 0) return;
+    }
     static_assert(NTR == 0 || (!RLDS && MMODE == QM_LDS), "register-resident weights: the shared-M kernel without LDS staging");
     static_assert(!RPOOL || (MMODE == QM_LDS && !RLDS && PPL == 1 && PQ > 0 && HLDS), "pooled trend tables: the shared-M one-slot kernel");
     extern __shared__ __align__(16) unsigned char smem[];
@@ -1414,13 +1507,39 @@
     wave_sync();
 
     for (;;) {
+        constexpr int MBATCH = (quad_three_waves(MMODE, PPL, HLDS) || MMODE == QM_RAGGED_REG || MMODE == QM_GLOBAL_REG) ? 8 : 16;
+        constexpr bool MREG = MMODE == QM_RAGGED_REG || MMODE == QM_GLOBAL_REG;
+        if constexpr (TAIL == QTAIL_RESUME) {
+            int i = atomicAdd(qa.counter + QTC_TAIL_HEAD, lane == 0 ? 1 : 0);
+            i = __builtin_amdgcn_readfirstlane(i);
+            if (i >= tail_len) break;
+            const int64_t n = (int64_t)__builtin_amdgcn_readfirstlane(qa.tail_list[i]);
+            fit_one_quad<KP, PPL, PQ, RAGGED_K, MRS, HLDS, MBATCH, MREG, NTR, RPOOL, TAIL>(qa, wlp, rb, Mp, Mown, n, lanec, hist, gx, qw, &pool,
+                                                                                        qa.tail_rec + (size_t)i * QT_REC);
+            atomicAdd(qa.counter + QTC_RESUMED, lane == 0 ? 1 : 0);
+            continue;
+        }
         int n32 = atomicAdd(qa.counter, lane == 0 ? 1 : 0);
         n32 = __builtin_amdgcn_readfirstlane(n32);
-        if (n32 >= a.N) break;
+        if (n32 >= a.N) {
+            if constexpr (TAIL == QTAIL_MAIN) {
+                if (qa.tail_at > 0 && __builtin_amdgcn_readfirstlane(__hip_atomic_load(qa.counter + QTC_FLAG, __ATOMIC_RELAXED, __HIP_MEMORY_SCOPE_AGENT)) == 0) {
+                    const int done = __hip_atomic_load(qa.counter + QTC_DONE, __ATOMIC_RELAXED, __HIP_MEMORY_SCOPE_AGENT);
+                    const int alive = (int)a.N - __builtin_amdgcn_readfirstlane(done);
+                    if (alive <= qa.tail_at) {
+                        atomicCAS(qa.counter + QTC_ALIVE, 0, alive + 1);
+                        __hip_atomic_store(qa.counter + QTC_FLAG, 1, __ATOMIC_RELAXED, __HIP_MEMORY_SCOPE_AGENT);
+                    }
+                }
+            }
+            break;
+        }
         const int64_t n = a.order ? (int64_t)a.order[n32] : (int64_t)n32;
-        fit_one_quad<KP, PPL, PQ, RAGGED_K, MRS, HLDS,
-                     ((quad_three_waves(MMODE, PPL, HLDS) || MMODE == QM_RAGGED_REG || MMODE == QM_GLOBAL_REG) ? 8 : 16),
-                     MMODE == QM_RAGGED_REG || MMODE == QM_GLOBAL_REG, NTR, RPOOL>(qa, wlp, rb, Mp, Mown, n, lanec, hist, gx, qw, &pool);
+        const bool moved = fit_one_quad<KP, PPL, PQ, RAGGED_K, MRS, HLDS, MBATCH, MREG, NTR, RPOOL, TAIL>(qa, wlp, rb, Mp, Mown, n, lanec, hist, gx, qw, &pool);
+        if constexpr (TAIL == QTAIL_MAIN) {
+            if (moved) break;
+            atomicAdd(qa.counter + QTC_DONE, lane == 0 ? 1 : 0);
+        }
     }
 }
 
diff --git a/time_series_spark_amd/csrc/tsf_quad_launch.h b/time_series_spark_amd/csrc/tsf_quad_launch.h
--- a/time_series_spark_amd/csrc/tsf_quad_launch.h
+++ b/time_series_spark_amd/csrc/tsf_quad_launch.h
@@ -39,6 +39,8 @@
 
 namespace tsf {
 
+static_assert(TSF_QUAD_NW3 <= QT_MAIN_WAVES, "the checkpoint records are sized for the 12-wave kernel");
+
 template <int PPL, int MMODE>
 struct QuadShape {
     static constexpr bool HL = true;
@@ -52,7 +54,30 @@
            (sizeof(QuadWave<PPL>) + quad_hist_bytes<PPL>(true)) * (size_t)nw + QUAD_POOL_LOCK_BYTES;
 }
 
-template <int KP, int PPL, int MMODE, int PQ, bool RLDS, int NTR = 0, bool RPOOL = false>
+template <int KP>
+static size_t quad_reg_lds_bytes(int NTmax)
+{
+    return quad_lanec_bytes<1>() + (sizeof(QuadLds<KP, 1>) + quad_hist_bytes<1>(true) + sizeof(double) * (size_t)NTmax * W) * TSF_QUAD_NW;
+}
+
+template <int KP, int PQ>
+static int launch_quad_resume(const QuadPlan &qp, const QuadArgs &qa_in, hipStream_t st)
+{
+    constexpr int NW = TSF_QUAD_NW;
+    QuadArgs qa = qa_in;
+    qa.dbg = nullptr;
+    int64_t blocks = qp.n_cu;
+    const int64_t cap_blocks = ((int64_t)qa.tail_cap + NW - 1) / NW;
+    if (blocks > cap_blocks) blocks = cap_blocks;
+    if (blocks < 1) blocks = 1;
+    hipFuncSetAttribute((const void *)fit_quad_kernel<KP, 1, NW, QM_GLOBAL_REG, PQ, true, true, 0, false, QTAIL_RESUME>,
+                        hipFuncAttributeMaxDynamicSharedMemorySize, 160 * 1024);
+    hipLaunchKernelGGL((fit_quad_kernel<KP, 1, NW, QM_GLOBAL_REG, PQ, true, true, 0, false, QTAIL_RESUME>), dim3((unsigned)blocks), dim3(NW * 64),
+                       quad_reg_lds_bytes<KP>(qa.f.NTmax), st, qa, 0, 0);
+    return (int)hipGetLastError();
+}
+
+template <int KP, int PPL, int MMODE, int PQ, bool RLDS, int NTR = 0, bool RPOOL = false, int TAIL = QTAIL_NONE>
 static int launch_quad_rl(const QuadPlan &qp, const QuadArgs &qa_in, double *Mg, hipStream_t st, int pool_slots = 0, int pool_slot_bytes = 0)
 {
     constexpr int NW = RPOOL ? TSF_QUAD_NW4 : QuadShape<PPL, MMODE>::NW;
@@ -71,7 +96,7 @@
                      : (MLDS ? sizeof(double) * (size_t)qp.P4 * PPL * W : 0) + quad_lanec_bytes<PPL>() * ((MMODE == QM_RAGGED || MMODE == QM_RAGGED_REG) ? NW : 1) +
                        (sizeof(QuadLds<KP, PPL>) + quad_hist_bytes<PPL>(HL)) * NW +
                        (RLDS ? sizeof(double) * (size_t)NW * qa.f.NTmax * W : 0);
-    hipFuncSetAttribute((const void *)fit_quad_kernel<KP, PPL, NW, MMODE, PQ, RLDS, HL, NTR, RPOOL>,
+    hipFuncSetAttribute((const void *)fit_quad_kernel<KP, PPL, NW, MMODE, PQ, RLDS, HL, NTR, RPOOL, TAIL>,
                             hipFuncAttributeMaxDynamicSharedMemorySize, 160 * 1024);
 #ifdef TSF_QUAD_TIMING
     {
@@ -79,7 +104,7 @@
         const size_t nb = sizeof(long long) * 8 * (size_t)qa.f.N;
         hipMalloc((void **)&qb.dbg, nb);
         hipMemsetAsync(qb.dbg, 0, nb, st);
-        hipLaunchKernelGGL((fit_quad_kernel<KP, PPL, NW, MMODE, PQ, RLDS, HL, NTR, RPOOL>), dim3((unsigned)blocks), dim3(NW * 64), lds, st, qb, pool_slots, pool_slot_bytes);
+        hipLaunchKernelGGL((fit_quad_kernel<KP, PPL, NW, MMODE, PQ, RLDS, HL, NTR, RPOOL, TAIL>), dim3((unsigned)blocks), dim3(NW * 64), lds, st, qb, pool_slots, pool_slot_bytes);
         hipStreamSynchronize(st);
         std::vector<long long> h(8 * (size_t)qa.f.N);
         hipMemcpy(h.data(), qb.dbg, nb, hipMemcpyDeviceToHost);
@@ -92,8 +117,24 @@
         return (int)hipGetLastError();
     }
 #endif
-    hipLaunchKernelGGL((fit_quad_kernel<KP, PPL, NW, MMODE, PQ, RLDS, HL, NTR, RPOOL>), dim3((unsigned)blocks), dim3(NW * 64), lds, st, qa, pool_slots, pool_slot_bytes);
+    hipLaunchKernelGGL((fit_quad_kernel<KP, PPL, NW, MMODE, PQ, RLDS, HL, NTR, RPOOL, TAIL>), dim3((unsigned)blocks), dim3(NW * 64), lds, st, qa, pool_slots, pool_slot_bytes);
     return (int)hipGetLastError();
+}
+
+#ifndef TSF_QUAD_TAIL_DEFAULT
+#define TSF_QUAD_TAIL_DEFAULT 800
+#endif
+template <int KP, int PQ>
+static int quad_tail_at(const QuadPlan &qp, const QuadArgs &qa)
+{
+    if (PQ != 40 && PQ != 56) return 0;
+    if (!qa.tail_rec || !qa.tail_list || qa.tail_cap < 1) return 0;
+    if (quad_reg_lds_bytes<KP>(qa.f.NTmax) > 160 * 1024) return 0;
+    const int e = qp.opt ? qp.opt[TSF_OPT_QUAD_TAIL] : -1;
+    const int pct = e >= 0 ? e : TSF_QUAD_TAIL_DEFAULT;
+    const int64_t at = (int64_t)qp.n_cu * pct / 100;
+    if (pct > 0 && at < 1) return 1;
+    return (int)(at > qa.tail_cap ? qa.tail_cap : at);
 }
 
 template <int KP, int PPL, int MMODE, int PQ>
@@ -120,8 +161,18 @@
     const size_t rbytes = sizeof(double) * (size_t)NW * qa.f.NTmax * W;
     if (base + rbytes <= 160 * 1024) return launch_quad_rl<KP, PPL, MMODE, PQ, true>(qp, qa, Mg, st);
     if constexpr (MMODE == QM_LDS && PPL == 1 && PQ > 0) {
-        if (!(qp.opt && qp.opt[TSF_OPT_QUAD_RREG] == 0))
+        if (!(qp.opt && qp.opt[TSF_OPT_QUAD_RREG] == 0)) {
+            if constexpr (PQ == 40 || PQ == 56) {
+                QuadArgs qt = qa;
+                qt.tail_at = quad_tail_at<KP, PQ>(qp, qa);
+                if (qt.tail_at > 0) {
+                    const int rc = launch_quad_rl<KP, PPL, MMODE, PQ, false, TSF_QUAD_NTR, false, QTAIL_MAIN>(qp, qt, Mg, st);
+                    if (rc != 0) return rc;
+                    return launch_quad_tail(KP, qp, qt, st);
+                }
+            }
             return launch_quad_rl<KP, PPL, MMODE, PQ, false, TSF_QUAD_NTR>(qp, qa, Mg, st);
+        }
     }
     return launch_quad_rl<KP, PPL, MMODE, PQ, false>(qp, qa, Mg, st);
 }
diff --git a/time_series_spark_amd/forecaster.py b/time_series_spark_amd/forecaster.py
--- a/time_series_spark_amd/forecaster.py
+++ b/time_series_spark_amd/forecaster.py
@@ -840,6 +840,13 @@
     g, n = ctypes.c_int64(), ctypes.c_int32()
     ctx.check(_lib.load().tsf_last_cv_grids(ctx.handle, ctypes.byref(g), ctypes.byref(n)))
     return int(g.value), int(n.value)
+
+
+def last_quad_tail(ctx=None):
+    ctx = ctx or get_context()
+    h, r, a = ctypes.c_int32(), ctypes.c_int32(), ctypes.c_int32()
+    ctx.check(_lib.load().tsf_last_quad_tail(ctx.handle, ctypes.byref(h), ctypes.byref(r), ctypes.byref(a)))
+    return int(h.value), int(r.value), int(a.value)
 
 
 
```
